# HaydenFaulkner/Tennis

Measured on AMD Instinct MI355X. Metric: frames/sec DenseNet-121 224x224 feature-extract, higher is better.
Workload: dtype f16

## Files before the change

### include/tennis_hip_debug.h

```cpp
#ifndef TENNIS_HIP_DEBUG_H
#define TENNIS_HIP_DEBUG_H
#include "tennis_hip.h"
#ifdef __cplusplus
extern "C" {
#endif

typedef struct {
  char name[32];
  int launches;
  double ms;
  double flops;
  double bytes;
} tn_kernel_stat;


int tn_densenet121_profile(tn_encoder *enc, const void *x, tn_layout layout, int batch, float *feat,
                           tn_kernel_stat *stats, int max_stats, int *n_stats);

int tn_dbg_profile_class_maps(tn_encoder *enc, const void *x, tn_layout layout, int batch, float *feat, const tn_dense *classes,
                              float *maps, tn_kernel_stat *stats, int max_stats, int *n_stats);
int tn_dbg_class_maps(tn_ctx *ctx, const void *x_f16, const float *x32, int B, int H, int W, int C, const float *scale, const float *shift,
                      const float *wd, int PH, int PW, int classes, float *maps, int *n_seq, int *depth);

int tn_densenet121_read_tap(tn_encoder *enc, const char *tap, int batch, float *out_host,
                            size_t capacity, size_t *numel);

int tn_jpeg_sync_passes(const tn_jpeg *j);

int tn_dbg_conv1x1(tn_ctx *ctx, const void *x_f16, int ldx, int K, const float *scale_host,
                   const float *shift_host, const float *w_host, int N, void *y_f16, int ldy, int yoff,
                   int M, int pool, int H, int W);
int tn_dbg_conv3x3(tn_ctx *ctx, const void *x_f16, const float *scale_host, const float *shift_host,
                   const float *w_host, void *y_f16, int ldy, int yoff, int B, int H, int W);
int tn_dbg_pack_conv3x3(const float *w_host, uint16_t *out_host);
int tn_dbg_conv1x1_dev(tn_ctx *ctx, const void *x_f16, int ldx, int K, const float *scale, const float *shift,
                       const void *w_f16, int N, void *y_f16, int ldy, int yoff, int M, int pool, int H, int W,
                       int variant);
int tn_dbg_conv3x3_dev(tn_ctx *ctx, const void *x_f16, const float *scale, const float *shift,
                       const void *wp_f16, void *y_f16, int ldy, int yoff, int B, int H, int W, int variant);
int tn_dbg_conv1x1_ex(tn_ctx *ctx, const void *x_f16, int ldx, int K, const float *scale, const float *shift, const void *w_f16, int N,
                      void *y_f16, int ldy, int yoff, int M, int pool, int H, int W, int variant, const float *bias, int clamp,
                      float *y32, int ld32, const void *wfrag);
int tn_dbg_pack_trans_frags(const uint16_t *w_f16_host, int N, int K, uint16_t *out_host);
int tn_dbg_pack_trans_frags_dev(tn_ctx *ctx, const void *w_f16, int N, int K, void *out_f16);
int tn_dbg_dense_layer_dev(tn_ctx *ctx, void *buf_f16, int ldc, int K, const float *s1, const float *t1,
                           const void *w1_f16, const float *s2, const float *t2, const void *w3p_f16, int B,
                           int H, int W, unsigned long long *ts , int variant );
int tn_dbg_dense_chain_dev(tn_ctx *ctx, void *buf_f16, int ldc, int K0, int nchain, const float *const *s1, const float *const *t1,
                           const void *const *w1_f16, const float *const *s2, const float *const *t2, const void *const *w3p_f16,
                           int B, int H, int W, int variant);
int tn_dbg_linear(tn_ctx *ctx, const float *x, const float *w, const float *bias, float *y, int M, int N,
                  int K);
int tn_dbg_channel_mean(tn_ctx *ctx, const void *x_f16, int ld, int K, const float *scale, const float *shift, int64_t rows,
                        void *scratch, size_t scratch_bytes, float *out, int clamp);
int tn_dbg_stem(tn_ctx *ctx, const float *w0_host, const float *gamma_host, const float *beta_host, const float *mean_host,
                const float *var_host, const float *centre_host, int exact, int fused, int layout, int B, int H, int W,
                const void *x, void *y_f16, int ldy);
int tn_dbg_maxpool(tn_ctx *ctx, const void *x_f16, int B, int H, int W, int C, void *y_f16, int ldy, int Ho, int Wo);
int tn_dbg_head(tn_ctx *ctx, const void *x_f16, const float *x32, int B, int H, int W, int C, const float *scale, const float *shift,
                float *feat, int PH, int PW);
int tn_dbg_pack_strip(const float *w1_host, int K, const float *s2_host, const float *t2_host, uint16_t *w1s_out,
                      const float *w3_host, uint16_t *w3s_out);
int tn_dbg_dense_strip_dev(tn_ctx *ctx, void *buf_f16, int ldc, int K, const float *s1, const float *t1,
                           const void *w1s_f16, const void *w3s_f16, int B, int H, int W,
                           unsigned long long *ts );
int tn_dbg_dense_strip_pair_dev(tn_ctx *ctx, void *buf_f16, int ldc, int K, const float *s1, const float *t1,
                                const void *w1s_f16, const void *w3s_f16, int B, int H, int W, unsigned long long *ts);
int tn_dbg_dense_strip_pair_chain_dev(tn_ctx *ctx, void *buf_f16, int ldc, int K0, int nl, const float *const *s1,
                                      const float *const *t1, const void *const *w1s_f16, const void *const *w3s_f16, int B, int H,
                                      int W);
int tn_dbg_strip_pair_launches(int64_t *count);

int tn_dbg_block7_create(tn_ctx *ctx, int K0, int nl, const float *w1_all, const float *s1_all, const float *t1_all,
                         const float *s2_all, const float *t2_all, const float *w3_all, void **out);
int tn_dbg_block7_run(void *handle, void *buf_f16, int ldc, int B);
int tn_dbg_block7_run_ts(void *handle, void *buf_f16, int ldc, int B,
                         unsigned long long *ts );
void tn_dbg_block7_destroy(void *handle);

int tn_dbg_block14_create(tn_ctx *ctx, int K0, int nl, const float *w1_all, const float *s1_all, const float *t1_all,
                          const float *s2_all, const float *t2_all, const float *w3_all, void **out);
int tn_dbg_block14_run(void *handle, void *buf_f16, int ldc, int B);
int tn_dbg_block14_run_ts(void *handle, void *buf_f16, int ldc, int B,
                          unsigned long long *ts );
void tn_dbg_block14_destroy(void *handle);
int tn_dbg_block28_create(tn_ctx *ctx, int K0, int nl, const float *w1_all, const float *s1_all, const float *t1_all,
                          const float *s2_all, const float *t2_all, const float *w3_all, void **out);
int tn_dbg_block28_run(void *handle, void *buf_f16, int ldc, int B);
int tn_dbg_block28_run_ts(void *handle, void *buf_f16, int ldc, int B, unsigned long long *ts);
void tn_dbg_block28_destroy(void *handle);

int tn_dbg_gemm_tn(tn_ctx *ctx, const float *A, int lda, const float *B, int ldb, const float *bsc, const float *bsh, float *Cm, int ldc,
                   int M, int N, int K, float *workspace, int64_t workspace_floats);
int tn_dbg_linear_bnrelu(tn_ctx *ctx, const float *X, int ldx, const float *asc, const float *ash, const float *W, int ldw,
                         const float *bias, float *Y, int ldy, int M, int N, int K, int accumulate);
int tn_dbg_linear_fp32x3(tn_ctx *ctx, const float *X, int ldx, const float *asc, const float *ash, const float *W, int ldw,
                         const float *bias, float *Y, int ldy, int M, int N, int K, int accumulate);
int tn_dbg_gemm_tn_fp32x3(tn_ctx *ctx, const float *A, int lda, const float *B, int ldb, const float *bsc, const float *bsh, float *Cm,
                          int ldc, int M, int N, int K, float *workspace, int64_t workspace_floats);
int tn_dbg_gemm_nn(tn_ctx *ctx, const float *A, int lda, const float *B, int ldb, float *Cm, int ldc, int M, int N, int K);
int tn_dbg_bn_train(tn_ctx *ctx, const float *x, int ld, int64_t M, int C, const float *gamma, const float *beta, float *mean, float *var,
                    float *y, const float *dy, float *dgamma, float *dbeta, float *dx, int ldd, int accumulate);
int tn_dbg_gnmt_trainer_src_grad(tn_gnmt_trainer *t, const float *src, const int32_t *src_valid_len, const int32_t *tgt, int ld,
                                 const int32_t *tgt_valid_len, int batch, int steps, int tgt_len, float *loss, float *logits_out,
                                 float *dsrc, int ldd);
int tn_dbg_rows_pad_skip(int on);

int tn_dbg_rnn_route(int gates, int B, int H, int dirs, int *nb, int *kr, int *big);

int tn_dbg_rnn_wide_route(int gates, int B, int H, int dirs, int *threads, int *rows, int *nb, int64_t *lds_fwd, int64_t *lds_bwd);
int tn_dbg_rnn_force_wide(int on);
int tn_dbg_rnn_wide_launches(int64_t *count);

int tn_dbg_encoder_plan(int height, int width, int flags, int batch, int calibrate, tn_kernel_stat *stats, int max_stats, int *n_stats);
int tn_dbg_encoder_plan_shared(int height, int width, int flags, int batch, tn_kernel_stat *stats, int max_stats, int *n_stats,
                               int *paired_out);

enum { TN_TRAINER_HEAD = 0, TN_TRAINER_GNMT = 1, TN_TRAINER_BACKBONE = 2 };
typedef struct tn_param_row {
  char name[96];
  int where;
  int64_t offset, count;
} tn_param_row;
int tn_dbg_trainer_params(int which, const int *dims, int n_dims, const char *prefix_a, const char *prefix_b, tn_param_row *rows,
                          int max_rows, int *n_rows, int64_t *numel, int64_t *state_numel);

int tn_dbg_conv_fp32x3(tn_ctx *ctx, int which, int kind, int tile, int layout, const void *x, int ldx, int K, const float *s, const float *t,
                       const float *w_host, int N, const float *es, const float *et, float *y, int ldy, int yoff, int64_t M, int H, int W,
                       int Ho, int Wo);

int tn_dbg_window_head_rows_per_group(struct tn_window_head *h, int nb);

#define TN_GRAD_SUMSQ_BLOCK 256
#define TN_GRAD_SUMSQ_CHUNK 4096
#define TN_GRAD_SUMSQ_GRID 1024
int tn_dbg_grad_sumsq(tn_ctx *ctx, const float *dev, int64_t n, const float *dev2, int64_t n2, double *sumsq_host);

int tn_dbg_gnmt_attention_fwd(tn_ctx *ctx, const float *g0, const float *hprev, int ldh, const float *cprev, int lstm, const float *keyproj,
                              const float *mem, const int32_t *valid_len, int B, int T, int H, int beam, int split_cap, float *hn, float *cn,
                              float *x1, int ldx1, float *ctx_out, float *w_out);
int tn_dbg_gnmt_attention_bwd(tn_ctx *ctx, const float *aw, const float *mem, const float *keyproj, const float *c0, int lc0, const float *c1,
                              int lc1, const int32_t *valid_len, int B, int T, int H, float *ds, float *dctx, float *dh0);
int tn_dbg_gnmt_attention_outer(tn_ctx *ctx, const float *aw, const float *ds, const float *dctx, const float *h0, int ldh, int steps, int B,
                                int T, int H, float *dmem, float *dkp);
int tn_dbg_gnmt_ce(tn_ctx *ctx, const float *logits, const int32_t *labels, int ld, const int32_t *valid_len, int B, int L, int V,
                   float *dlogits, float *loss_rows, float *loss, float *masked_loss);
int tn_dbg_gnmt_emb_grad(tn_ctx *ctx, const float *dx0, int K0, const int32_t *tgt, int ld, int B, int L, int E, int V, float *demb);

#ifdef __cplusplus
}
#endif
#endif
```

### tennis_amd/_lib.py

```python
from __future__ import annotations

import ctypes as C
import os

import numpy as np
import torch

_HERE = os.path.dirname(os.path.abspath(__file__))
LIB_PATH = os.environ.get("TENNIS_HIP_LIB") or os.path.join(_HERE, "lib", "libtennis_hip.so")

LAYOUT_NCHW_F32, LAYOUT_NHWC_F16, LAYOUT_NHWC_U8 = 0, 1, 2
ENC_EXACT_WEIGHTS = 1
ENC_FP32 = 4
ENC_FP32X3 = 8
RNN_GRU, RNN_LSTM = 0, 1
POOL_MAX, POOL_MEAN = 0, 1
MATMUL_MODES = {"f32": 0, "fp32x3": 1}


def matmul_mode(name) -> int:
    if name not in MATMUL_MODES:
        raise ValueError(f"matmul must be 'f32' or 'fp32x3', got {name!r}")
    return MATMUL_MODES[name]

# ... 15 lines not shown
PARAM_FLAT, PARAM_STATE, PARAM_PTR = 0, 1, 2

_P = C.c_void_p
_SIGS = {
    "tn_version": (C.c_int, []),
    "tn_last_error": (C.c_char_p, []),
    "tn_ctx_create": (C.c_int, [C.c_int, _P, C.c_int, C.POINTER(_P)]),
    "tn_ctx_stream": (_P, [_P]),
    "tn_ctx_sync": (C.c_int, [_P]),
    "tn_ctx_destroy": (C.c_int, [_P]),
    "tn_densenet121_create": (C.c_int, [_P, C.POINTER(TnParam), C.c_int, C.c_char_p, C.c_int, C.c_int, C.c_int,
                                        C.POINTER(_P)]),
    "tn_densenet121_create_ex": (C.c_int, [_P, C.POINTER(TnParam), C.c_int, C.c_char_p, C.c_int, C.c_int, C.c_int, C.c_int,
                                           C.POINTER(_P)]),
    "tn_densenet121_feature_dim": (C.c_int, [_P]),
    "tn_densenet121_workspace_bytes": (C.c_size_t, [_P]),
    "tn_densenet121_forward": (C.c_int, [_P, _P, C.c_int, C.c_int, _P]),
    "tn_densenet121_forward_class_maps": (C.c_int, [_P, _P, C.c_int, C.c_int, _P, _P, _P]),
    "tn_densenet121_class_map_dims": (C.c_int, [_P, C.POINTER(C.c_int), C.POINTER(C.c_int)]),
    "tn_dbg_profile_class_maps": (C.c_int, [_P, _P, C.c_int, C.c_int, _P, _P, _P, C.POINTER(TnKernelStat), C.c_int, C.POINTER(C.c_int)]),
    "tn_dbg_class_maps": (C.c_int, [_P, _P, _P, C.c_int, C.c_int, C.c_int, C.c_int, _P, _P, _P, C.c_int, C.c_int, C.c_int, _P,
                                    C.POINTER(C.c_int), C.POINTER(C.c_int)]),
    "tn_densenet121_set_pipelined": (C.c_int, [_P, C.c_int]),
    "tn_densenet121_join": (C.c_int, [_P, C.c_int]),
    "tn_densenet121_profile": (C.c_int, [_P, _P, C.c_int, C.c_int, _P, C.POINTER(TnKernelStat), C.c_int,
                                         C.POINTER(C.c_int)]),
    "tn_densenet121_read_tap": (C.c_int, [_P, C.c_char_p, C.c_int, _P, C.c_size_t, C.POINTER(C.c_size_t)]),
    "tn_densenet121_destroy": (C.c_int, [_P]),
    "tn_dense_create": (C.c_int, [_P, _P, _P, C.c_int, C.c_int, C.POINTER(_P)]),
    "tn_dense_forward": (C.c_int, [_P, _P, C.c_int, _P]),
    "tn_dense_destroy": (C.c_int, [_P]),
    "tn_birnn_create": (C.c_int, [_P, C.c_int, C.c_int, C.c_int, C.POINTER(TnParam), C.c_int, C.c_char_p, C.c_int,
                                  C.c_int, C.POINTER(_P)]),
    "tn_birnn_forward": (C.c_int, [_P, _P, C.c_int, C.c_int, _P, _P, _P, _P]),
    "tn_birnn_destroy": (C.c_int, [_P]),
    "tn_preproc_create": (C.c_int, [_P, C.c_int, C.c_int, C.c_int, C.c_int, C.POINTER(_P)]),
    "tn_preproc_forward": (C.c_int, [_P, _P, C.c_int, _P]),
    "tn_preproc_destroy": (C.c_int, [_P]),
    "tn_augment_forward": (C.c_int, [_P, _P, C.c_int, C.c_int, C.c_int, _P, _P, C.c_int, _P, _P, _P]),
    "tn_to_tensor_normalize": (C.c_int, [_P, _P, C.c_long, C.POINTER(C.c_float), C.POINTER(C.c_float), _P]),
    "tn_jpeg_create": (C.c_int, [_P, C.POINTER(_P)]),
    "tn_jpeg_info": (C.c_int, [_P, C.c_size_t, C.POINTER(C.c_int), C.POINTER(C.c_int), C.POINTER(C.c_int), C.POINTER(C.c_int),
                               C.POINTER(C.c_int)]),
    "tn_jpeg_decode": (C.c_int, [_P, C.POINTER(_P), C.POINTER(C.c_size_t), C.c_int, _P, C.POINTER(C.c_int), C.POINTER(C.c_int)]),
    "tn_jpeg_sync_passes": (C.c_int, [_P]),
    "tn_jpeg_destroy": (C.c_int, [_P]),
    "tn_temporal_pool": (C.c_int, [_P, _P, C.c_int, C.c_int, C.c_int, C.c_int, _P]),
    "tn_window_head_create": (C.c_int, [_P, C.c_int, C.c_int, C.c_int, C.c_int, C.POINTER(TnParam), C.c_int, C.c_char_p, C.c_char_p,
                                        C.c_int, C.c_int, C.POINTER(_P)]),
    "tn_window_head_project": (C.c_int, [_P, _P, C.c_int]),
    "tn_window_head_forward": (C.c_int, [_P, _P, _P, _P, C.c_int, C.c_int, C.c_int, _P, _P]),
    "tn_window_head_forward_rows": (C.c_int, [_P, _P, C.c_int, C.c_int, _P, _P]),
    "tn_window_head_destroy": (C.c_int, [_P]),
    "tn_temporal_pool_windows": (C.c_int, [_P, _P, C.c_int, C.c_int, _P, _P, _P, C.c_int, C.c_int, C.c_int, C.c_int, _P]),
    "tn_temporal_pool_rows": (C.c_int, [_P, _P, C.c_int, C.c_int, _P, C.c_int, C.c_int, C.c_int, _P]),
    "tn_dbg_window_head_rows_per_group": (C.c_int, [_P, C.c_int]),
    "tn_prf1_update": (C.c_int, [_P, _P, _P, C.c_int, C.c_int, _P]),
    "tn_head_create": (C.c_int, [_P, C.c_int, C.c_int, C.c_int, C.c_int, C.POINTER(TnParam), C.c_int, C.c_char_p, C.c_char_p, C.c_int,
                                 C.c_int, C.POINTER(_P)]),
    "tn_head_forward_backward": (C.c_int, [_P, _P, _P, C.c_int, C.c_int, _P, _P]),
    "tn_head_set_features": (C.c_int, [_P, _P, C.c_int, C.c_int]),
    "tn_head_forward_backward_rows": (C.c_int, [_P, _P, _P, C.c_int, C.c_int, _P, _P]),
    "tn_head_forward_rows": (C.c_int, [_P, _P, C.c_int, C.c_int, _P]),
    "tn_head_buffers": (C.c_int, [_P, C.POINTER(_P), C.POINTER(_P), C.POINTER(C.c_int64)]),
    "tn_head_sgd_step": (C.c_int, [_P, C.c_float, C.c_float, C.c_float, C.c_float]),
    "tn_head_read_param": (C.c_int, [_P, C.c_char_p, C.c_int, C.POINTER(C.c_float), C.c_int64, C.POINTER(C.c_int64)]),
    "tn_head_destroy": (C.c_int, [_P]),
    "tn_finetune_create": (C.c_int, [_P, C.POINTER(TnParam), C.c_int, C.c_char_p, C.c_char_p, C.c_int, C.c_int, C.c_int, C.c_int,
                                     C.POINTER(_P)]),
    "tn_finetune_forward_backward": (C.c_int, [_P, _P, _P, C.c_int, C.c_int, C.c_int, _P, _P]),
    "tn_finetune_buffers": (C.c_int, [_P, C.POINTER(_P), C.POINTER(_P), C.POINTER(C.c_int64)]),
    "tn_finetune_sgd_step": (C.c_int, [_P, C.c_float, C.c_float, C.c_float, C.c_float]),
    "tn_finetune_read_param": (C.c_int, [_P, C.c_char_p, C.c_int, C.POINTER(C.c_float), C.c_int64, C.POINTER(C.c_int64)]),
    "tn_finetune_destroy": (C.c_int, [_P]),
    "tn_finetune_set_matmul": (C.c_int, [_P, C.c_int]),
    "tn_finetune_matmul_stats": (C.c_int, [_P, C.POINTER(C.c_int64), C.POINTER(C.c_int64)]),
    "tn_cnnrnn_trainer_set_matmul": (C.c_int, [_P, C.c_int]),
    "tn_cnnrnn_trainer_matmul_stats": (C.c_int, [_P, C.POINTER(C.c_int64), C.POINTER(C.c_int64)]),
    "tn_gnmt_frames_trainer_set_matmul": (C.c_int, [_P, C.c_int]),
    "tn_gnmt_frames_trainer_matmul_stats": (C.c_int, [_P, C.POINTER(C.c_int64), C.POINTER(C.c_int64)]),
    "tn_cnnrnn_trainer_create": (C.c_int, [_P, C.c_int, C.POINTER(TnParam), C.c_int, C.c_char_p, C.c_char_p, C.c_char_p, C.c_int, C.c_int,
                                           C.c_int, C.c_int, C.c_int, C.c_int, C.POINTER(_P)]),
    "tn_cnnrnn_trainer_forward_backward": (C.c_int, [_P, _P, _P, C.c_int, C.c_int, C.c_int, C.c_int, _P, _P]),
    "tn_cnnrnn_trainer_buffers": (C.c_int, [_P, C.POINTER(_P), C.POINTER(_P), C.POINTER(C.c_int64), C.POINTER(_P), C.POINTER(_P),
                                            C.POINTER(C.c_int64)]),
    "tn_cnnrnn_trainer_sgd_step": (C.c_int, [_P, C.c_float, C.c_float, C.c_float, C.c_float]),
    "tn_cnnrnn_trainer_read_param": (C.c_int, [_P, C.c_char_p, C.c_int, C.POINTER(C.c_float), C.c_int64, C.POINTER(C.c_int64)]),
    "tn_cnnrnn_trainer_destroy": (C.c_int, [_P]),
    "tn_gnmt_frames_trainer_create": (C.c_int, [_P, C.POINTER(TnParam), C.c_int, C.c_char_p, C.c_char_p, C.c_int, C.c_int, C.c_int, C.c_int,
                                                C.c_int, C.c_int, C.c_int, C.c_int, C.c_int, C.c_int, C.c_int, C.c_int, C.c_int,
                                                C.POINTER(_P)]),
    "tn_gnmt_frames_trainer_forward_backward": (C.c_int, [_P, _P, _P, _P, C.c_int, _P, C.c_int, C.c_int, C.c_int, _P, _P]),
    "tn_gnmt_frames_trainer_buffers": (C.c_int, [_P, C.POINTER(_P), C.POINTER(_P), C.POINTER(C.c_int64), C.POINTER(_P), C.POINTER(_P),
                                                 C.POINTER(C.c_int64)]),
    "tn_gnmt_frames_trainer_set_dropout": (C.c_int, [_P, C.c_float, C.c_uint64]),
    "tn_gnmt_frames_trainer_adam_step": (C.c_int, [_P, C.c_float, C.c_float, C.c_float, C.c_float]),
    "tn_gnmt_frames_trainer_read_param": (C.c_int, [_P, C.c_char_p, C.c_int, C.POINTER(C.c_float), C.c_int64, C.POINTER(C.c_int64)]),
    "tn_gnmt_frames_trainer_destroy": (C.c_int, [_P]),
    "tn_head_set_clip": (C.c_int, [_P, C.c_float]),
    "tn_head_clip_stats": (C.c_int, [_P, C.POINTER(C.c_float), C.POINTER(C.c_float), C.POINTER(C.c_int64)]),
    "tn_finetune_set_clip": (C.c_int, [_P, C.c_float]),
    "tn_finetune_clip_stats": (C.c_int, [_P, C.POINTER(C.c_float), C.POINTER(C.c_float), C.POINTER(C.c_int64)]),
    "tn_cnnrnn_trainer_set_clip": (C.c_int, [_P, C.c_float]),
    "tn_cnnrnn_trainer_clip_stats": (C.c_int, [_P, C.POINTER(C.c_float), C.POINTER(C.c_float), C.POINTER(C.c_int64)]),
    "tn_gnmt_trainer_set_clip": (C.c_int, [_P, C.c_float]),
    "tn_gnmt_trainer_clip_stats": (C.c_int, [_P, C.POINTER(C.c_float), C.POINTER(C.c_float), C.POINTER(C.c_int64)]),
    "tn_gnmt_frames_trainer_set_clip": (C.c_int, [_P, C.c_float]),
    "tn_gnmt_frames_trainer_clip_stats": (C.c_int, [_P, C.POINTER(C.c_float), C.POINTER(C.c_float), C.POINTER(C.c_int64)]),
    "tn_dbg_grad_sumsq": (C.c_int, [_P, _P, C.c_int64, _P, C.c_int64, C.POINTER(C.c_double)]),
    "tn_dbg_rows_pad_skip": (C.c_int, [C.c_int]),
    "tn_dbg_gnmt_trainer_src_grad": (C.c_int, [_P, _P, _P, _P, C.c_int, _P, C.c_int, C.c_int, C.c_int, _P, _P, _P, C.c_int]),
    "tn_dbg_gnmt_attention_fwd": (C.c_int, [_P, _P, _P, C.c_int, _P, C.c_int, _P, _P, _P, C.c_int, C.c_int, C.c_int, C.c_int, C.c_int,
                                            _P, _P, _P, C.c_int, _P, _P]),
    "tn_dbg_gnmt_attention_bwd": (C.c_int, [_P, _P, _P, _P, _P, C.c_int, _P, C.c_int, _P, C.c_int, C.c_int, C.c_int, _P, _P, _P]),
    "tn_dbg_gnmt_attention_outer": (C.c_int, [_P, _P, _P, _P, _P, C.c_int, C.c_int, C.c_int, C.c_int, C.c_int, _P, _P]),
    "tn_dbg_gnmt_ce": (C.c_int, [_P, _P, _P, C.c_int, _P, C.c_int, C.c_int, C.c_int, _P, _P, _P, _P]),
    "tn_dbg_gnmt_emb_grad": (C.c_int, [_P, _P, C.c_int, _P, C.c_int, C.c_int, C.c_int, C.c_int, C.c_int, _P]),
    "tn_gnmt_trainer_create": (C.c_int, [_P, C.POINTER(TnParam), C.c_int, C.c_char_p, C.c_int, C.c_int, C.c_int, C.c_int, C.c_int,
                                         C.c_int, C.c_int, C.c_int, C.POINTER(_P)]),
    "tn_gnmt_trainer_create_ex": (C.c_int, [_P, C.POINTER(TnParam), C.c_int, C.c_char_p, C.c_int, C.c_int, C.c_int, C.c_int, C.c_int,
                                            C.c_int, C.c_int, C.c_int, C.c_int, C.c_int, C.c_int, C.POINTER(_P)]),
    "tn_gnmt_trainer_dropout_mask": (C.c_int, [_P, C.c_int, C.POINTER(_P)]),
    "tn_gnmt_trainer_forward_backward": (C.c_int, [_P, _P, _P, _P, C.c_int, _P, C.c_int, C.c_int, C.c_int, _P, _P]),
    "tn_gnmt_trainer_forward_backward_rows": (C.c_int, [_P, _P, C.c_int, C.c_int, _P, _P, _P, C.c_int, _P, C.c_int, C.c_int, C.c_int, _P, _P]),
    "tn_gnmt_trainer_buffers": (C.c_int, [_P, C.POINTER(_P), C.POINTER(_P), C.POINTER(C.c_int64)]),
    "tn_gnmt_trainer_set_dropout": (C.c_int, [_P, C.c_float, C.c_uint64]),
    "tn_gnmt_trainer_dropout_masks": (C.c_int, [_P, C.POINTER(_P), C.POINTER(_P), C.POINTER(_P)]),
    "tn_gnmt_trainer_adam_step": (C.c_int, [_P, C.c_float, C.c_float, C.c_float, C.c_float]),
    "tn_gnmt_trainer_read_param": (C.c_int, [_P, C.c_char_p, C.c_int, C.POINTER(C.c_float), C.c_int64, C.POINTER(C.c_int64)]),
    "tn_gnmt_trainer_destroy": (C.c_int, [_P]),
    "tn_gnmt_create": (C.c_int, [_P, C.POINTER(TnParam), C.c_int, C.c_char_p, C.c_int, C.c_int, C.c_int, C.c_int, C.c_int,
                                 C.c_int, C.c_int, C.c_int, C.c_int, C.c_int, C.c_int, C.POINTER(_P)]),
    "tn_gnmt_create_ex": (C.c_int, [_P, C.POINTER(TnParam), C.c_int, C.c_char_p, C.c_int, C.c_int, C.c_int, C.c_int, C.c_int,
                                    C.c_int, C.c_int, C.c_int, C.c_int, C.c_int, C.c_int, C.c_int, C.POINTER(_P)]),
    "tn_gnmt_encode": (C.c_int, [_P, _P, _P, C.c_int, C.c_int, _P]),
    "tn_gnmt_encode_rows": (C.c_int, [_P, _P, C.c_int, C.c_int, _P, _P, C.c_int, C.c_int, _P]),
    "tn_gnmt_beam_search": (C.c_int, [_P, C.c_int, C.c_int, C.c_float, C.c_float, C.c_int, _P, _P, _P,
                                      C.POINTER(C.c_int)]),
    "tn_gnmt_decode_seq": (C.c_int, [_P, _P, C.c_int, C.c_int, _P]),
    "tn_gnmt_decode_seq_attention": (C.c_int, [_P, _P, C.c_int, C.c_int, _P, _P]),
    "tn_gnmt_beam_search_attention": (C.c_int, [_P, C.c_int, C.c_int, C.c_float, C.c_float, C.c_int, _P, _P, _P,
                                                C.POINTER(C.c_int), _P]),
    "tn_masked_softmax_ce": (C.c_int, [_P, _P, _P, C.c_int, _P, C.c_int, C.c_int, C.c_int, _P]),
    "tn_gnmt_destroy": (C.c_int, [_P]),
    "tn_dbg_conv1x1": (C.c_int, [_P, _P, C.c_int, C.c_int, _P, _P, _P, C.c_int, _P, C.c_int, C.c_int, C.c_int,
                                 C.c_int, C.c_int, C.c_int]),
    "tn_dbg_conv3x3": (C.c_int, [_P, _P, _P, _P, _P, _P, C.c_int, C.c_int, C.c_int, C.c_int, C.c_int]),
    "tn_dbg_pack_conv3x3": (C.c_int, [_P, _P]),
    "tn_dbg_conv1x1_dev": (C.c_int, [_P, _P, C.c_int, C.c_int, _P, _P, _P, C.c_int, _P, C.c_int, C.c_int, C.c_int,
                                     C.c_int, C.c_int, C.c_int, C.c_int]),
    "tn_dbg_conv3x3_dev": (C.c_int, [_P, _P, _P, _P, _P, _P, C.c_int, C.c_int, C.c_int, C.c_int, C.c_int, C.c_int]),
    "tn_dbg_conv1x1_ex": (C.c_int, [_P, _P, C.c_int, C.c_int, _P, _P, _P, C.c_int, _P, C.c_int, C.c_int, C.c_int,
                                    C.c_int, C.c_int, C.c_int, C.c_int, _P, C.c_int, _P, C.c_int, _P]),
    "tn_dbg_pack_trans_frags": (C.c_int, [_P, C.c_int, C.c_int, _P]),
    "tn_dbg_pack_trans_frags_dev": (C.c_int, [_P, _P, C.c_int, C.c_int, _P]),
    "tn_dbg_dense_layer_dev": (C.c_int, [_P, _P, C.c_int, C.c_int, _P, _P, _P, _P, _P, _P, C.c_int, C.c_int, C.c_int,
                                         _P, C.c_int]),
    "tn_dbg_dense_chain_dev": (C.c_int, [_P, _P, C.c_int, C.c_int, C.c_int, _P, _P, _P, _P, _P, _P, C.c_int, C.c_int, C.c_int, C.c_int]),
    "tn_dbg_linear": (C.c_int, [_P, _P, _P, _P, _P, C.c_int, C.c_int, C.c_int]),
    "tn_dbg_channel_mean": (C.c_int, [_P, _P, C.c_int, C.c_int, _P, _P, C.c_int64, _P, C.c_size_t, _P, C.c_int]),
    "tn_dbg_stem": (C.c_int, [_P, _P, _P, _P, _P, _P, _P, C.c_int, C.c_int, C.c_int, C.c_int, C.c_int, C.c_int, _P, _P, C.c_int]),
    "tn_dbg_maxpool": (C.c_int, [_P, _P, C.c_int, C.c_int, C.c_int, C.c_int, _P, C.c_int, C.c_int, C.c_int]),
    "tn_dbg_head": (C.c_int, [_P, _P, _P, C.c_int, C.c_int, C.c_int, C.c_int, _P, _P, _P, C.c_int, C.c_int]),
    "tn_dbg_conv_fp32x3": (C.c_int, [_P, C.c_int, C.c_int, C.c_int, C.c_int, _P, C.c_int, C.c_int, _P, _P, _P, C.c_int, _P, _P, _P, C.c_int,
                                     C.c_int, C.c_int64, C.c_int, C.c_int, C.c_int, C.c_int]),
    "tn_dbg_gemm_tn": (C.c_int, [_P, _P, C.c_int, _P, C.c_int, _P, _P, _P, C.c_int, C.c_int, C.c_int, C.c_int, _P, C.c_int64]),
    "tn_dbg_gemm_nn": (C.c_int, [_P, _P, C.c_int, _P, C.c_int, _P, C.c_int, C.c_int, C.c_int, C.c_int]),
    "tn_dbg_rnn_wide_route": (C.c_int, [C.c_int, C.c_int, C.c_int, C.c_int, C.POINTER(C.c_int), C.POINTER(C.c_int), C.POINTER(C.c_int),
                                        C.POINTER(C.c_int64), C.POINTER(C.c_int64)]),
    "tn_dbg_rnn_force_wide": (C.c_int, [C.c_int]),
    "tn_dbg_rnn_wide_launches": (C.c_int, [C.POINTER(C.c_int64)]),
    "tn_dbg_rnn_route": (C.c_int, [C.c_int, C.c_int, C.c_int, C.c_int, C.POINTER(C.c_int), C.POINTER(C.c_int), C.POINTER(C.c_int)]),
    "tn_dbg_encoder_plan": (C.c_int, [C.c_int, C.c_int, C.c_int, C.c_int, C.c_int, C.POINTER(TnKernelStat), C.c_int, C.POINTER(C.c_int)]),
    "tn_dbg_encoder_plan_shared": (C.c_int, [C.c_int, C.c_int, C.c_int, C.c_int, C.POINTER(TnKernelStat), C.c_int, C.POINTER(C.c_int),
                                             C.POINTER(C.c_int)]),
    "tn_dbg_trainer_params": (C.c_int, [C.c_int, C.POINTER(C.c_int), C.c_int, C.c_char_p, C.c_char_p, C.POINTER(TnParamRow), C.c_int,
                                        C.POINTER(C.c_int), C.POINTER(C.c_int64), C.POINTER(C.c_int64)]),
    "tn_dbg_linear_bnrelu": (C.c_int, [_P, _P, C.c_int, _P, _P, _P, C.c_int, _P, _P, C.c_int, C.c_int, C.c_int, C.c_int, C.c_int]),
    "tn_dbg_linear_fp32x3": (C.c_int, [_P, _P, C.c_int, _P, _P, _P, C.c_int, _P, _P, C.c_int, C.c_int, C.c_int, C.c_int, C.c_int]),
    "tn_dbg_gemm_tn_fp32x3": (C.c_int, [_P, _P, C.c_int, _P, C.c_int, _P, _P, _P, C.c_int, C.c_int, C.c_int, C.c_int, _P, C.c_int64]),
    "tn_dbg_bn_train": (C.c_int, [_P, _P, C.c_int, C.c_int64, C.c_int, _P, _P, _P, _P, _P, _P, _P, _P, _P, C.c_int, C.c_int]),
    "tn_comm_unique_id": (C.c_int, [_P]),
    "tn_comm_create": (C.c_int, [_P, C.c_int, C.c_int, _P, C.c_int, C.POINTER(_P)]),
    "tn_comm_rank": (C.c_int, [_P]),
    "tn_comm_world": (C.c_int, [_P]),
    "tn_comm_device": (C.c_int, [_P]),
    "tn_comm_uses_rccl": (C.c_int, [_P]),
    "tn_allgather_features": (C.c_int, [_P, _P, C.c_int, C.c_int, _P]),
    "tn_allreduce_f32": (C.c_int, [_P, _P, C.c_size_t, C.c_int]),
    "tn_allreduce_i64": (C.c_int, [_P, _P, C.c_size_t]),
    "tn_comm_destroy": (C.c_int, [_P]),
    "tn_dbg_pack_strip": (C.c_int, [_P, C.c_int, _P, _P, _P, _P, _P]),
    "tn_dbg_dense_strip_dev": (C.c_int, [_P, _P, C.c_int, C.c_int, _P, _P, _P, _P, C.c_int, C.c_int, C.c_int, _P]),
    "tn_dbg_dense_strip_pair_dev": (C.c_int, [_P, _P, C.c_int, C.c_int, _P, _P, _P, _P, C.c_int, C.c_int, C.c_int, _P]),
    "tn_dbg_dense_strip_pair_chain_dev": (C.c_int, [_P, _P, C.c_int, C.c_int, C.c_int, _P, _P, _P, _P, C.c_int, C.c_int, C.c_int]),
    "tn_dbg_strip_pair_launches": (C.c_int, [C.POINTER(C.c_int64)]),
    "tn_densenet121_input_means": (C.c_int, [_P, _P, C.c_int, C.c_int, _P, C.c_int64, C.POINTER(C.c_int64)]),
    "tn_npy_writer_create": (C.c_int, [C.c_int, C.POINTER(_P)]),
    "tn_npy_writer_submit": (C.c_int, [_P, _P, C.c_int, C.c_int, C.POINTER(C.c_char_p), C.c_int]),
    "tn_npy_writer_drain": (C.c_int, [_P, C.POINTER(C.c_int64), C.POINTER(C.c_int64)]),
    "tn_npy_writer_destroy": (C.c_int, [_P]),
    "tn_bn_relu_clamp_fold": (C.c_int, [_P, _P, _P, _P, C.c_int, _P, _P, _P, _P]),
    "tn_fp32x3_split": (C.c_int, [_P, C.c_int64, _P, _P, _P]),
    "tn_round_fp16_calibrated": (C.c_int, [_P, C.c_int, C.c_int, _P, C.c_int, C.c_int, C.c_double, _P]),
    "tn_dbg_block7_create": (C.c_int, [_P, C.c_int, C.c_int, _P, _P, _P, _P, _P, _P, C.POINTER(C.c_void_p)]),
    "tn_dbg_block7_run": (C.c_int, [_P, _P, C.c_int, C.c_int]),
    "tn_dbg_block7_run_ts": (C.c_int, [_P, _P, C.c_int, C.c_int, _P]),
    "tn_dbg_block7_destroy": (None, [_P]),
    "tn_dbg_block14_create": (C.c_int, [_P, C.c_int, C.c_int, _P, _P, _P, _P, _P, _P, C.POINTER(C.c_void_p)]),
    "tn_dbg_block14_run": (C.c_int, [_P, _P, C.c_int, C.c_int]),
    "tn_dbg_block14_run_ts": (C.c_int, [_P, _P, C.c_int, C.c_int, _P]),
    "tn_dbg_block14_destroy": (None, [_P]),
    "tn_dbg_block28_create": (C.c_int, [_P, C.c_int, C.c_int, _P, _P, _P, _P, _P, _P, C.POINTER(C.c_void_p)]),
    "tn_dbg_block28_run": (C.c_int, [_P, _P, C.c_int, C.c_int]),
    "tn_dbg_block28_run_ts": (C.c_int, [_P, _P, C.c_int, C.c_int, _P]),
    "tn_dbg_block28_destroy": (None, [_P]),
}

_lib = None


def declared_symbols():
    return sorted(_SIGS)


def load():
    global _lib
    if _lib is None:
        if not os.path.exists(LIB_PATH):
            raise RuntimeError(
                f"{LIB_PATH} is missing: build it with `make` (or __graft_entry__.build()). "
                "tennis_amd has no CPU fallback.")
        lib = C.CDLL(LIB_PATH)
        for name, (res, args) in _SIGS.items():
            fn = getattr(lib, name)
            fn.restype, fn.argtypes = res, args
        _lib = lib
    return _lib


def check(rc: int, what: str = ""):
    if rc != 0:
        msg = load().tn_last_error().decode("utf-8", "replace")
        raise RuntimeError(f"libtennis_hip {what} failed ({rc}): {msg}")


def trainer_params(which: int, dims, prefix_a: str, prefix_b: str | None = None):
    lib = load()
    d = (C.c_int * len(dims))(*[int(v) for v in dims])
    b = None if prefix_b is None else prefix_b.encode()
    n, numel, ns = C.c_int(), C.c_int64(), C.c_int64()
    check(lib.tn_dbg_trainer_params(which, d, len(dims), prefix_a.encode(), b, None, 0, C.byref(n), None, None), "tn_dbg_trainer_params")
    rows = (TnParamRow * n.value)()
    check(lib.tn_dbg_trainer_params(which, d, len(dims), prefix_a.encode(), b, rows, n.value, C.byref(n), C.byref(numel), C.byref(ns)),
          "tn_dbg_trainer_params")
    return [(r.name.decode(), r.where, r.offset, r.count) for r in rows], numel.value, ns.value


def make_params(params: dict):
    keep = []
    arr = (TnParam * len(params))()
    for i, (k, v) in enumerate(params.items()):
        a = np.ascontiguousarray(v, dtype=np.float32)
        name = k.encode()
        keep += [a, name]
        arr[i].name = name
        arr[i].data_host = a.ctypes.data_as(C.POINTER(C.c_float))
        arr[i].numel = a.size
    return arr, keep


class Context:

    def __init__(self, device: int | None = None, stream=None):
        if not torch.cuda.is_available():
            raise RuntimeError("tennis_amd needs a ROCm GPU: torch.cuda.is_available() is False and there is no "
                               "CPU fallback")
        self.lib = load()
        device = default_device() if device is None else int(device)
        self.device = device
        if stream is None:
            stream = torch.cuda.current_stream(device)
        self.torch_stream = stream
        h = _P()
        check(self.lib.tn_ctx_create(device, _P(stream.cuda_stream), 0, C.byref(h)), "tn_ctx_create")
        self.handle = h

    def sync(self):
        check(self.lib.tn_ctx_sync(self.handle), "tn_ctx_sync")

    def __del__(self):
        try:
            if getattr(self, "handle", None):
                self.lib.tn_ctx_destroy(self.handle)
                self.handle = None
        except Exception:
            pass


_default_ctx = {}


def default_device() -> int:
    if torch.cuda.is_available():
        cur = torch.cuda.current_device()
        if cur != 0 or "LOCAL_RANK" not in os.environ:
            return cur
        lr = int(os.environ["LOCAL_RANK"])
        return lr if lr < torch.cuda.device_count() else cur
    return 0


def default_context(device: int | None = None) -> Context:
    device = default_device() if device is None else int(device)
    if device not in _default_ctx:
        _default_ctx[device] = Context(device)
    return _default_ctx[device]


def ptr(t) -> _P:
    return _P(t.data_ptr()) if t is not None else _P(None)
```

### tennis_amd/csrc/common.h

```cpp
#pragma once
#include <atomic>
#include <hip/hip_runtime.h>
#include <hip/hip_fp16.h>
#include <stdint.h>
#include <string>
#include <vector>

#include "../../include/tennis_hip.h"
#include "../../include/tennis_hip_debug.h"

typedef _Float16 f16;
typedef _Float16 f16x4 __attribute__((ext_vector_type(4)));
typedef _Float16 f16x8 __attribute__((ext_vector_type(8)));
typedef float f32x4 __attribute__((ext_vector_type(4)));
typedef float f32x16 __attribute__((ext_vector_type(16)));

void tn_set_error(const std::string &msg);
#define TN_HIP_CHECK(expr)                                                             \
  do {                                                                                 \
    hipError_t _e = (expr);                                                            \
    if (_e != hipSuccess) {                                                            \
      tn_set_error(std::string(#expr) + ": " + hipGetErrorString(_e));                 \
      return TN_ERR_HIP;                                                               \
    }                                                                                  \
  } while (0)
#define TN_REQUIRE(cond, msg)                                                          \
  do {                                                                                 \
    if (!(cond)) {                                                                     \
      tn_set_error(std::string("invalid argument: ") + (msg));                         \
      return TN_ERR_INVALID;                                                           \
    }                                                                                  \
  } while (0)

struct TnDeviceGuard {
  int prev = -1;
  bool ok = true;
  explicit TnDeviceGuard(int dev) {
    if (hipGetDevice(&prev) != hipSuccess) prev = -1;
    if (prev == dev) prev = -1;
    else ok = hipSetDevice(dev) == hipSuccess;
  }
  ~TnDeviceGuard() {
    if (prev >= 0) (void)hipSetDevice(prev);
  }
  TnDeviceGuard(const TnDeviceGuard &) = delete;
  TnDeviceGuard &operator=(const TnDeviceGuard &) = delete;
};
#define TN_DG_CAT2(a, b) a##b
#define TN_DG_CAT(a, b) TN_DG_CAT2(a, b)
#define TN_ON_DEVICE(dev)                                                              \
  TnDeviceGuard TN_DG_CAT(tn_dg_, __LINE__)(dev);                                      \
  if (!TN_DG_CAT(tn_dg_, __LINE__).ok) {                                               \
    tn_set_error("hipSetDevice failed");                                               \
    return TN_ERR_HIP;                                                                 \
  }

struct tn_ctx {
  int device;
  hipStream_t stream;
  bool own_stream;
};

__device__ __forceinline__ f16x8 bn_relu8(f16x8 v, const float *__restrict__ s, const float *__restrict__ t) {
  f16x8 r;
#pragma unroll
  for (int j = 0; j < 8; ++j) {
    float f = fmaf((float)v[j], s[j], t[j]);
    r[j] = (f16)fmaxf(f, 0.0f);
  }
  return r;
}

__device__ __forceinline__ f16x8 clamp8(f16x8 v, const float *__restrict__ lo, const float *__restrict__ hi) {
  f16x8 r;
#pragma unroll
  for (int j = 0; j < 8; ++j) r[j] = (f16)fminf(fmaxf((float)v[j], lo[j]), hi[j]);
  return r;
}
__device__ __forceinline__ unsigned clamp2_pk(unsigned in, float lo0, float lo1, float hi0, float hi1) {
  unsigned l, h, o;
  asm("v_cvt_pk_f16_f32 %1, %4, %5\n\tv_cvt_pk_f16_f32 %2, %6, %7\n\tv_pk_max_f16 %0, %3, %1\n\tv_pk_min_f16 %0, %0, %2\n\ts_nop 0"
      : "=&v"(o), "=&v"(l), "=&v"(h) : "v"(in), "v"(lo0), "v"(lo1), "v"(hi0), "v"(hi1));
  return o;
}
__device__ __forceinline__ f16x8 clamp8_pk(f16x8 v, const float *__restrict__ lo, const float *__restrict__ hi) {
  typedef unsigned u32x4 __attribute__((ext_vector_type(4)));
  const u32x4 in = __builtin_bit_cast(u32x4, v);
  u32x4 out;
#pragma unroll
  for (int j = 0; j < 4; ++j) out[j] = clamp2_pk(in[j], lo[2 * j], lo[2 * j + 1], hi[2 * j], hi[2 * j + 1]);
  return __builtin_bit_cast(f16x8, out);
}

__device__ __forceinline__ f16x4 bn_relu4_from_f32(f32x4 v, float4 s, float4 t) {
  typedef unsigned u32x2 __attribute__((ext_vector_type(2)));
  float a0, a1, a2, a3;
  unsigned d0, d1;
  asm("s_nop 11\n\t"
      "v_fma_f32 %2, %6, %10, %14\n\tv_fma_f32 %3, %7, %11, %15\n\tv_fma_f32 %4, %8, %12, %16\n\tv_fma_f32 %5, %9, %13, %17\n\t"
      "v_cvt_pk_f16_f32 %0, %2, %3\n\tv_cvt_pk_f16_f32 %1, %4, %5\n\tv_pk_max_f16 %0, %0, 0\n\tv_pk_max_f16 %1, %1, 0"
      : "=&v"(d0), "=&v"(d1), "=&v"(a0), "=&v"(a1), "=&v"(a2), "=&v"(a3)
      : "v"(v[0]), "v"(v[1]), "v"(v[2]), "v"(v[3]), "v"(s.x), "v"(s.y), "v"(s.z), "v"(s.w), "v"(t.x), "v"(t.y), "v"(t.z), "v"(t.w));
  const u32x2 o = {d0, d1};
  return __builtin_bit_cast(f16x4, o);
}

template <int ROWB>
__device__ __forceinline__ int swz(int row, int chunk) {
  constexpr int NCH = ROWB / 16;
  return row * ROWB + ((chunk ^ (row & (NCH - 1))) << 4);
}

struct Conv1x1Args {
  const f16 *x;
  int ldx;
  int K;
  const float *scale;
  const float *shift;
  const f16 *w;
  int N;
  f16 *y;
  int ldy, yoff;
  int M;
  int pool;
  int H, W;
  int variant = 0;
  int exact = 0;
  const float *bias = nullptr;
  int clamp = 0;
  float *y32 = nullptr;
  int ld32 = 0;
  const f16 *wfrag = nullptr;
};
int launch_conv1x1(const Conv1x1Args &a, hipStream_t s);
bool trans_ws_supported(const Conv1x1Args &a);
int launch_trans_ws(const Conv1x1Args &a, hipStream_t s);
std::vector<f16> pack_trans_frags(const f16 *w, int N, int K);
int launch_pack_trans_frags(const f16 *w, int N, int K, f16 *out, hipStream_t s);

struct Conv3x3Args {
  const f16 *x;
  const float *scale;
  const float *shift;
  const f16 *wp;
  f16 *y;
  int ldy, yoff;
  int M, H, W;
  int variant = 0;
  int exact = 0;
};
int launch_conv3x3(const Conv3x3Args &a, hipStream_t s);
size_t conv3x3_lds_bytes(int W);

struct DenseLayerDev {
  const float *s1, *t1;
  const f16 *w1;
  const float *s2, *t2;
  const f16 *w3p;
};
struct DenseLayerArgs {
  f16 *buf;
  int ldc, K;
  const float *s1, *t1;
  const f16 *w1;
  const float *s2, *t2;
  const f16 *w3p;
  int B, H, W;
  unsigned long long *ts = nullptr;
  int variant = 0;
  const DenseLayerDev *chain = nullptr;
  int nchain = 0;
  int exact = 0;
};
bool dense_layer_supported(int H, int W);
int dense_layer_kmax(int W);
int launch_dense_layer(const DenseLayerArgs &a, hipStream_t s);

struct DenseStripArgs {
  f16 *buf;
  int ldc, K;
  const float *s1, *t1;
  const f16 *w1s;
  const f16 *w3s;
  int B, H, W;
  unsigned long long *ts = nullptr;
};
bool dense_strip_supported(int H, int W, int K);
int launch_dense_strip(const DenseStripArgs &a, hipStream_t s);
struct DenseStripLayerDev {
  const float *s1, *t1;
  const f16 *w1s, *w3s;
};
struct DenseStripChainArgs {
  f16 *buf;
  int ldc, K0, nl;
  const DenseStripLayerDev *layers;
  int B, H, W;
};
bool dense_strip_chain_supported(int H, int W, int K0, int nl);
int dense_strip_chain_layers(int H, int W, int K0);
int launch_dense_strip_chain(const DenseStripChainArgs &a, hipStream_t s);
int launch_dense_strip_pair(const DenseStripArgs &a, hipStream_t s);
int launch_dense_strip_pair_chain(const DenseStripChainArgs &a, hipStream_t s);
long strip_pair_launches();
std::vector<f16> pack_w1_strip(const float *w , int K, const float *shift );
std::vector<f16> pack_w3_strip(const float *w );

struct DenseBlock7Args {
  f16 *buf;
  int ldc, K0, nl, B;
  const f16 *wa, *wb;
  const float *tab;
  unsigned a_off[4], b_off[4];
  unsigned long long *ts = nullptr;
  float *side = nullptr;
};
struct Block7Layer { const float *w1f , *w3 , *s1, *t1 , *t2 ; };
struct Block7Image {
  std::vector<f16> wa, wb;
  std::vector<float> tab;
  unsigned a_off[4], b_off[4];
};
bool dense_block7_supported(int H, int W, int K0, int nl);
inline constexpr const char *kDenseBlock7Range = "7 x 7, K0 = 448 ... 992 in steps of 32, nl >= 1, K0 + 32 nl <= 1024";
Block7Image pack_block7(const std::vector<Block7Layer> &layers, int K0);
int launch_dense_block7(const DenseBlock7Args &a, hipStream_t s);

struct DenseStreamArgs {
  f16 *buf;
  int ldc, K0, nl, B;
  const unsigned char *stream;
  int total_units;
  f16 *scratch = nullptr;
  unsigned long long *ts = nullptr;
};
struct Block14Layer { const float *w1f , *w3 , *s1, *t1 , *t2 ; };
bool dense_block14_supported(int H, int W, int K0, int nl);
int dense_block14_units(int K0, int nl);
size_t dense_block14_scratch_halfs();
std::vector<unsigned char> pack_block14(const std::vector<Block14Layer> &layers, int K0);
int launch_dense_block14(const DenseStreamArgs &a, hipStream_t s);
bool dense_block28_supported(int H, int W, int K0, int nl);
int dense_block28_units(int K0, int nl);
size_t dense_block28_scratch_halfs();
std::vector<unsigned char> pack_block28(const std::vector<Block14Layer> &layers, int K0);
int launch_dense_block28(const DenseStreamArgs &a, hipStream_t s);
inline constexpr const char *kDenseBlock14Range = "14 x 14, K0 = 256 ... 992 in steps of 32, nl >= 1, K0 + 32 nl <= 1024";
inline constexpr const char *kDenseBlock28Range = "28 x 28, K0 = 128 ... 512 in steps of 32, nl >= 1, K0 + 32 (nl - 1) <= 512";
struct DenseStreamKernel {
  int H;
  const char *family;
  bool (*supported)(int H, int W, int K0, int nl);
  int (*units)(int K0, int nl);
  size_t (*scratch_halfs)();
  std::vector<unsigned char> (*pack)(const std::vector<Block14Layer> &layers, int K0);
  int (*launch)(const DenseStreamArgs &a, hipStream_t s);
  const char *range;
};
inline constexpr DenseStreamKernel kDenseStreamKernels[2] = {
    {14, "dense_block_stream_14x14", dense_block14_supported, dense_block14_units, dense_block14_scratch_halfs, pack_block14, launch_dense_block14, kDenseBlock14Range},
    {28, "dense_block_stream_28x28", dense_block28_supported, dense_block28_units, dense_block28_scratch_halfs, pack_block28, launch_dense_block28, kDenseBlock28Range},
};

constexpr double kStemMean[3] = {0.485, 0.456, 0.406}, kStemStd[3] = {0.229, 0.224, 0.225};
constexpr float kStemQ[3] = {124.f, 116.f, 104.f};
constexpr double kStemWScale = 64.0;
constexpr float stem_unscale(int c) { return (float)(255.0 * kStemStd[c]); }
constexpr float stem_wfactor(int c) { return (float)(kStemWScale / (255.0 * kStemStd[c])); }
constexpr double stem_pad(int c) { return 255.0 * kStemMean[c] - (double)kStemQ[c]; }

struct StemArgs {
  const void *x;
  int layout;
  int B, H, W;
  const f16 *wp;
  const f16 *wp_zf;
  const float *scale;
  const float *shift;
  f16 *y;
  int Ho, Wo;
  const float *shift_u8 = nullptr;
  const f16 *wp_zf_lo = nullptr;
  const float *floor = nullptr;
};
struct StemFold {
  std::vector<f16> wp, wp_zf, wp_zf_lo;
  std::vector<float> scale, shift, shift_u8;
  std::vector<float> floor;
};
StemFold fold_stem(const float *w0, const float *bn_scale, const float *bn_shift, const float *centre, bool exact);
StemFold fold_stem_bn(const float *w0, const float *gamma, const float *beta, const float *mean, const float *var, const float *centre, bool exact);
int launch_stem(const StemArgs &a, hipStream_t s);
int launch_stem_pool(const StemArgs &a, f16 *out, int ldy, int Hp, int Wp, hipStream_t s);

int launch_maxpool3x3s2(const f16 *x, int B, int H, int W, int C, f16 *y, int ldy, int Ho, int Wo, hipStream_t s);
struct PerDeviceFlag {
  std::atomic<unsigned long long> done{0};
  bool is_set(int *dev_out) {
    int d = 0;
    (void)hipGetDevice(&d);
    *dev_out = d;
    return (done.load(std::memory_order_acquire) >> (d & 63)) & 1ull;
  }
  void set(int d) { done.fetch_or(1ull << (d & 63), std::memory_order_release); }
};
#define TN_SET_ATTR_ONCE_PER_DEVICE(...)                    \
  do {                                                      \
    static PerDeviceFlag tn_flag_;                          \
    int tn_dev_;                                            \
    if (!tn_flag_.is_set(&tn_dev_)) {                       \
      __VA_ARGS__;                                          \
      tn_flag_.set(tn_dev_);                                \
    }                                                       \
  } while (0)

void bn_scale_shift(const float *gamma, const float *beta, const float *mean, const float *var, int n, float eps, float *scale, float *shift);
void bn_relu_clamp_fold(const float *scale, const float *shift, int n, float *lo, float *hi, float *sw, float *tc);
int launch_channel_mean(const f16 *x, int ld, int K, const float *scale, const float *shift, long rows, double *scratch ,
                        float *out, hipStream_t s, int clamp = 0 );
int launch_head(const f16 *x, int B, int H, int W, int C, const float *scale, const float *shift,
                float *feat, int PH, int PW, hipStream_t s, const float *x32 = nullptr );
int launch_class_maps(const f16 *x, const float *x32, int B, int H, int W, int C, const float *scale, const float *shift, const float *wd,
                      int PH, int PW, int classes, float *out, hipStream_t s);
int class_maps_seq(int C);
int class_maps_depth();

enum { FP32_STEM = 0, FP32_1X1 = 1, FP32_3X3 = 2, FP32_TRANS = 3 };
struct Fp32ConvArgs {
  int kind;
  const void *x;
  int layout;
  int ldx;
  int K;
  const float *s, *t;
  const float *w;
  const uint16_t *wx = nullptr;
  int N;
  const float *es, *et;
  float *y;
  int ldy, yoff;
  long M;
  int H, W;
  int Ho, Wo;
};
int launch_conv_fp32(const Fp32ConvArgs &a, hipStream_t s);
int launch_conv_fp32x3(const Fp32ConvArgs &a, hipStream_t s, int tile = 0);
void fp32x3_split(const float *w, int64_t n, uint16_t *t1, uint16_t *t2, uint16_t *t3);
std::vector<uint16_t> fp32x3_pack_weights(const float *wk, int kp, int N);
int launch_maxpool_fp32(const float *x, int B, int H, int W, float *y, int ldy, int Ho, int Wo, hipStream_t s);
```

### tennis_amd/csrc/conv1x1.hip

```cpp
#include <cstdlib>

#include "common.h"

namespace {

constexpr int BN_TILE = 128;
constexpr int BK = 64;

template <int MI, int NB, bool POOL = false>
constexpr int smem_bytes() {
  constexpr int tiles = (POOL ? 2 : 1) * 32 * MI * 128 + NB * 128;
  constexpr int epi = 32 * MI * (NB * 2 + 16);
  return tiles > epi ? tiles : epi;
}

template <int MI, bool POOL, int NB, bool EX = false, bool ONCE = false>
__global__ __launch_bounds__(256) void conv1x1_kernel(Conv1x1Args a) {
  constexpr int BM = 32 * MI;
  constexpr int NSRC = POOL ? 4 : 1;
  constexpr int NI = NB / 32;
  constexpr int CPITCH = NB * 2 + 16;
  __shared__ __attribute__((aligned(16))) unsigned char smem[smem_bytes<MI, NB, POOL>()];
  unsigned char *Xs = smem;
  unsigned char *Xl = smem + BM * 128;
// ... 42 lines not shown
  const int WLD = EX ? 2 * nkc * BK : K;
  const f16 *wsrc = a.w + (long)(n0 + r0) * WLD;

  f16x8 xr[MI][NSRC];
  f16x8 wr[NI];
  float sc[8], sh[8];

  auto load_tile = [&](int kt) {
    const int kc = ((EX && kt >= nkc) ? kt - nkc : kt) * BK + c * 8;
    const int kw = kt * BK + c * 8;
    if (kc < K) {
      const float4 s0 = *(const float4 *)(a.scale + kc);
      const float4 s1 = *(const float4 *)(a.scale + kc + 4);
      const float4 t0 = *(const float4 *)(a.shift + kc);
      const float4 t1 = *(const float4 *)(a.shift + kc + 4);
      sc[0] = s0.x; sc[1] = s0.y; sc[2] = s0.z; sc[3] = s0.w;
      sc[4] = s1.x; sc[5] = s1.y; sc[6] = s1.z; sc[7] = s1.w;
      sh[0] = t0.x; sh[1] = t0.y; sh[2] = t0.z; sh[3] = t0.w;
      sh[4] = t1.x; sh[5] = t1.y; sh[6] = t1.z; sh[7] = t1.w;
#pragma unroll
      for (int i = 0; i < MI; ++i)
#pragma unroll
        for (int s = 0; s < NSRC; ++s) {
          if constexpr (ONCE) xr[i][s] = __builtin_nontemporal_load((const f16x8 *)(xsrc[i][s] + kc));
          else xr[i][s] = *(const f16x8 *)(xsrc[i][s] + kc);
        }
#pragma unroll
      for (int i = 0; i < NI; ++i) wr[i] = *(const f16x8 *)(wsrc + (long)(32 * i) * WLD + kw);
    }
  };

  auto store_tile = [&](int kt) {
    const int kc = ((EX && kt >= nkc) ? kt - nkc : kt) * BK + c * 8;
    const bool kv = kc < K;
#pragma unroll
    for (int i = 0; i < MI; ++i) {
      f16x8 v;
      [[maybe_unused]] f16x8 vl;
      if (kv) {
        if constexpr (POOL) {
#pragma unroll
          for (int j = 0; j < 8; ++j) {
            float acc = 0.f;
#pragma unroll
            for (int s = 0; s < 4; ++s) acc += fmaxf(fmaf((float)xr[i][s][j], sc[j], sh[j]), 0.f);
            const float m = 0.25f * acc;
            v[j] = (f16)m;
            vl[j] = (f16)(m - (float)v[j]);
          }
        } else {
          v = a.clamp ? clamp8(xr[i][0], sc, sh) : bn_relu8(xr[i][0], sc, sh);
        }
      } else {
#pragma unroll
        for (int j = 0; j < 8; ++j) { v[j] = (f16)0.f; vl[j] = (f16)0.f; }
      }
      *(f16x8 *)(Xs + swz<128>(r0 + 32 * i, c)) = v;
      if constexpr (POOL) *(f16x8 *)(Xl + swz<128>(r0 + 32 * i, c)) = vl;
    }
#pragma unroll
    for (int i = 0; i < NI; ++i) {
      f16x8 v = wr[i];
      if (!kv) {
#pragma unroll
        for (int j = 0; j < 8; ++j) v[j] = (f16)0.f;
      }
      *(f16x8 *)(Ws + swz<128>(r0 + 32 * i, c)) = v;
    }
  };

  f32x4 acc[NI][MI];
#pragma unroll
  for (int ni = 0; ni < NI; ++ni)
#pragma unroll
    for (int mi = 0; mi < MI; ++mi) acc[ni][mi] = (f32x4){0.f, 0.f, 0.f, 0.f};

  const int nk = EX ? 2 * nkc : nkc;
  const int frow = lane & 15;
  const int fch = lane >> 4;

  load_tile(0);
  for (int kt = 0; kt < nk; ++kt) {
    store_tile(kt);
    __syncthreads();
    if (kt + 1 < nk) load_tile(kt + 1);
#pragma unroll
    for (int ks = 0; ks < 2; ++ks) {
      if (((EX && kt >= nkc) ? kt - nkc : kt) * BK + ks * 32 < K) {
        f16x8 xb[MI], wa[NI];
        [[maybe_unused]] f16x8 xl[MI];
#pragma unroll
        for (int mi = 0; mi < MI; ++mi) {
          xb[mi] = *(const f16x8 *)(Xs + swz<128>(wm * 16 * MI + mi * 16 + frow, ks * 4 + fch));
          if constexpr (POOL) xl[mi] = *(const f16x8 *)(Xl + swz<128>(wm * 16 * MI + mi * 16 + frow, ks * 4 + fch));
        }
#pragma unroll
        for (int ni = 0; ni < NI; ++ni)
          wa[ni] = *(const f16x8 *)(Ws + swz<128>(wn * (NB / 2) + ni * 16 + frow, ks * 4 + fch));
#pragma unroll
        for (int ni = 0; ni < NI; ++ni)
#pragma unroll
          for (int mi = 0; mi < MI; ++mi)
            acc[ni][mi] = __builtin_amdgcn_mfma_f32_16x16x32_f16(wa[ni], xb[mi], acc[ni][mi], 0, 0, 0);
        if constexpr (POOL) {
#pragma unroll
          for (int ni = 0; ni < NI; ++ni)
#pragma unroll
            for (int mi = 0; mi < MI; ++mi)
              acc[ni][mi] = __builtin_amdgcn_mfma_f32_16x16x32_f16(wa[ni], xl[mi], acc[ni][mi], 0, 0, 0);
        }
      }
    }
    __syncthreads();
  }

#pragma unroll
  for (int ni = 0; ni < NI; ++ni)
#pragma unroll
    for (int mi = 0; mi < MI; ++mi) {
      const int m = wm * 16 * MI + mi * 16 + frow;
      const int n = wn * (NB / 2) + ni * 16 + fch * 4;
      f16x4 h;
      float4 bv = make_float4(0.f, 0.f, 0.f, 0.f);
      if (a.bias) bv = *(const float4 *)(a.bias + n0 + n);
      const float b4[4] = {bv.x, bv.y, bv.z, bv.w};
#pragma unroll
      for (int r = 0; r < 4; ++r) h[r] = (f16)(acc[ni][mi][r] + b4[r]);
      *(f16x4 *)(smem + m * CPITCH + n * 2) = h;
      if (a.y32 && m0 + m < a.M)
        *(float4 *)(a.y32 + (long)(m0 + m) * a.ld32 + n0 + n) =
            make_float4(acc[ni][mi][0] + b4[0], acc[ni][mi][1] + b4[1], acc[ni][mi][2] + b4[2], acc[ni][mi][3] + b4[3]);
    }
  __syncthreads();
#pragma unroll
  for (int i = 0; i < MI * NB / 64; ++i) {
    const int id = t + 256 * i;
    const int row = id / (NB / 8), ch = id % (NB / 8);
    const int m = m0 + row;
    if (m < a.M) {
      const uint4 v = *(const uint4 *)(smem + row * CPITCH + ch * 16);
      *(uint4 *)(a.y + (long)m * a.ldy + a.yoff + n0 + ch * 8) = v;
    }
  }
}

}

int launch_conv1x1(const Conv1x1Args &a, hipStream_t s) {
  TN_REQUIRE(a.K % 32 == 0 && a.N % BN_TILE == 0, "conv1x1: K%32 or N%128");
  TN_REQUIRE(a.ldx % 8 == 0 && a.ldy % 8 == 0 && a.yoff % 8 == 0, "conv1x1: strides must be multiples of 8");
  const dim3 block(256);
  static const bool no_ws = getenv("TN_NO_TRANS_WS") != nullptr;
  if (a.wfrag && !no_ws && trans_ws_supported(a)) return launch_trans_ws(a, s);
  if (a.pool) {
    static const bool narrow = getenv("TN_TRANS_NARROW") != nullptr;
    const bool wide = a.N % 256 == 0 && !narrow;
    const int mtiles = (a.M + 63) / 64, NT = a.N / (wide ? 256 : BN_TILE);
    const dim3 grid(((mtiles + 7) / 8) * 8 * NT);
    if (a.exact) {
      TN_REQUIRE(a.K % 64 == 0, "conv1x1: the exact-weights mode needs K % 64 == 0");
      if (wide) hipLaunchKernelGGL((conv1x1_kernel<2, true, 256, true>), grid, block, 0, s, a);
      else hipLaunchKernelGGL((conv1x1_kernel<2, true, 128, true>), grid, block, 0, s, a);
    } else {
      static const bool no_nt = getenv("TN_TRANS_NO_NT") != nullptr;
      static const size_t nt_mb = getenv("TN_TRANS_NT_MB") ? (size_t)atoi(getenv("TN_TRANS_NT_MB")) : 128;
      const bool stream = NT == 1 && !no_nt && (size_t)a.M * 4 * a.ldx * sizeof(f16) > (nt_mb << 20);
      if (wide && stream) hipLaunchKernelGGL((conv1x1_kernel<2, true, 256, false, true>), grid, block, 0, s, a);
      else if (wide) hipLaunchKernelGGL((conv1x1_kernel<2, true, 256>), grid, block, 0, s, a);
      else if (stream) hipLaunchKernelGGL((conv1x1_kernel<2, true, 128, false, true>), grid, block, 0, s, a);
      else hipLaunchKernelGGL((conv1x1_kernel<2, true, 128>), grid, block, 0, s, a);
    }
  } else if (a.M >= 128 * 512) {
    const dim3 grid((a.M + 127) / 128, a.N / BN_TILE);
    if (a.exact) hipLaunchKernelGGL((conv1x1_kernel<4, false, 128, true>), grid, block, 0, s, a);
    else hipLaunchKernelGGL((conv1x1_kernel<4, false, 128>), grid, block, 0, s, a);
  } else if (a.M >= 64 * 512) {
    const dim3 grid((a.M + 63) / 64, a.N / BN_TILE);
    if (a.exact) hipLaunchKernelGGL((conv1x1_kernel<2, false, 128, true>), grid, block, 0, s, a);
    else hipLaunchKernelGGL((conv1x1_kernel<2, false, 128>), grid, block, 0, s, a);
  } else {
    const dim3 grid((a.M + 31) / 32, a.N / BN_TILE);
    if (a.exact) hipLaunchKernelGGL((conv1x1_kernel<1, false, 128, true>), grid, block, 0, s, a);
    else hipLaunchKernelGGL((conv1x1_kernel<1, false, 128>), grid, block, 0, s, a);
  }
  TN_HIP_CHECK(hipGetLastError());
  return TN_OK;
}
```

### tennis_amd/csrc/dbg.hip

```cpp
#include <cstring>
#include <vector>

#include "common.h"
#include "encoder_plan.h"
#include "gemm_fp32x3.h"
#include "linear.h"
#include "param_table.h"
#include "rnn.h"
#include "train.h"

namespace {
template <typename T>
T *up(const std::vector<T> &h) {
  T *d = nullptr;
  if (hipMalloc(&d, h.size() * sizeof(T)) != hipSuccess) return nullptr;
  if (hipMemcpy(d, h.data(), h.size() * sizeof(T), hipMemcpyHostToDevice) != hipSuccess) return nullptr;
  return d;
}
}

std::vector<f16> pack_conv3x3(const float *w);

extern "C" int tn_dbg_pack_conv3x3(const float *w_host, uint16_t *out_host) {
  TN_REQUIRE(w_host && out_host, "tn_dbg_pack_conv3x3: null argument");
  const std::vector<f16> p = pack_conv3x3(w_host);
  memcpy(out_host, p.data(), p.size() * sizeof(f16));
  return TN_OK;
}

extern "C" int tn_dbg_conv1x1_dev(tn_ctx *ctx, const void *x_f16, int ldx, int K, const float *scale,
                                  const float *shift, const void *w_f16, int N, void *y_f16, int ldy, int yoff, int M,
                                  int pool, int H, int W, int variant) {
  TN_REQUIRE(ctx && x_f16 && y_f16 && scale && shift && w_f16, "tn_dbg_conv1x1_dev: null argument");
  Conv1x1Args a{(const f16 *)x_f16, ldx, K, scale, shift, (const f16 *)w_f16, N, (f16 *)y_f16, ldy, yoff, M, pool, H, W};
  a.variant = variant & 0xffff;
  a.exact = (variant >> 17) & 1;
  if ((variant >> 18) & 1) {
    TN_REQUIRE(trans_ws_supported(a), "tn_dbg_conv1x1_dev: geometry not supported by trans_ws");
    TN_ON_DEVICE(ctx->device);
    static f16 *frags[64] = {};
    static size_t frag_halves[64] = {};
    TN_REQUIRE(ctx->device >= 0 && ctx->device < 64, "tn_dbg_conv1x1_dev: device index out of range");
    f16 *&frag = frags[ctx->device];
    if (frag_halves[ctx->device] < (size_t)N * K) {
      if (frag) (void)hipFree(frag);
      frag = nullptr; frag_halves[ctx->device] = 0;
      TN_HIP_CHECK(hipMalloc((void **)&frag, (size_t)N * K * sizeof(f16)));
      frag_halves[ctx->device] = (size_t)N * K;
    }
    const int rc = launch_pack_trans_frags(a.w, N, K, frag, ctx->stream);
    if (rc) return rc;
    a.wfrag = frag;
  }
  return launch_conv1x1(a, ctx->stream);
}

extern "C" int tn_dbg_conv1x1_ex(tn_ctx *ctx, const void *x_f16, int ldx, int K, const float *scale, const float *shift, const void *w_f16,
                                 int N, void *y_f16, int ldy, int yoff, int M, int pool, int H, int W, int variant, const float *bias,
                                 int clamp, float *y32, int ld32, const void *wfrag) {
  TN_REQUIRE(ctx && x_f16 && y_f16 && scale && shift && w_f16, "tn_dbg_conv1x1_ex: null argument");
  TN_REQUIRE(M > 0 && K > 0 && N > 0 && ldx >= K && ldy >= yoff + N && yoff >= 0, "tn_dbg_conv1x1_ex: bad shape (M, K, N positive, ldx >= K, ldy >= yoff + N)");
  TN_REQUIRE(!pool || (H >= 2 && W >= 2 && M % ((H / 2) * (W / 2)) == 0), "tn_dbg_conv1x1_ex: pooling needs H, W >= 2 and M = B (H / 2) (W / 2)");
  TN_REQUIRE(!y32 || (ld32 >= N && ld32 % 4 == 0 && ((uintptr_t)y32 & 15) == 0), "tn_dbg_conv1x1_ex: y32 needs ld32 >= N, a multiple of 4, and 16-byte alignment");
  Conv1x1Args a{(const f16 *)x_f16, ldx, K, scale, shift, (const f16 *)w_f16, N, (f16 *)y_f16, ldy, yoff, M, pool, H, W};
  a.variant = variant & 0xffff;
  a.exact = (variant >> 17) & 1;
  a.bias = bias;
  a.clamp = clamp != 0;
  a.y32 = y32;
  a.ld32 = ld32;
  a.wfrag = (const f16 *)wfrag;
  TN_REQUIRE(!wfrag || trans_ws_supported(a), "tn_dbg_conv1x1_ex: wfrag with a geometry trans_ws does not support (pooling, fp16 weights, no bias, N = 512 | 256, K % 128 == 0, even H and W)");
  TN_ON_DEVICE(ctx->device);
  return launch_conv1x1(a, ctx->stream);
}

extern "C" int tn_dbg_pack_trans_frags(const uint16_t *w_f16_host, int N, int K, uint16_t *out_host) {
  TN_REQUIRE(w_f16_host && out_host, "tn_dbg_pack_trans_frags: null argument");
  TN_REQUIRE(N > 0 && K > 0 && N % 32 == 0 && K % 16 == 0, "tn_dbg_pack_trans_frags: N % 32 or K % 16");
  const std::vector<f16> p = pack_trans_frags((const f16 *)w_f16_host, N, K);
  memcpy(out_host, p.data(), p.size() * sizeof(f16));
  return TN_OK;
}
extern "C" int tn_dbg_pack_trans_frags_dev(tn_ctx *ctx, const void *w_f16, int N, int K, void *out_f16) {
  TN_REQUIRE(ctx && w_f16 && out_f16, "tn_dbg_pack_trans_frags_dev: null argument");
  TN_REQUIRE(N > 0 && K > 0, "tn_dbg_pack_trans_frags_dev: N and K must be positive");
  TN_ON_DEVICE(ctx->device);
  return launch_pack_trans_frags((const f16 *)w_f16, N, K, (f16 *)out_f16, ctx->stream);
}

extern "C" int tn_dbg_conv3x3_dev(tn_ctx *ctx, const void *x_f16, const float *scale, const float *shift,
                                  const void *wp_f16, void *y_f16, int ldy, int yoff, int B, int H, int W,
                                  int variant) {
  TN_REQUIRE(ctx && x_f16 && y_f16 && scale && shift && wp_f16, "tn_dbg_conv3x3_dev: null argument");
  Conv3x3Args a{(const f16 *)x_f16, scale, shift, (const f16 *)wp_f16, (f16 *)y_f16, ldy, yoff, B * H * W, H, W};
  a.variant = variant & 0xffff;
  a.exact = (variant >> 17) & 1;
  return launch_conv3x3(a, ctx->stream);
}

extern "C" int tn_dbg_conv1x1(tn_ctx *ctx, const void *x_f16, int ldx, int K, const float *scale_host,
                              const float *shift_host, const float *w_host , int N, void *y_f16, int ldy,
                              int yoff, int M, int pool, int H, int W) {
  TN_REQUIRE(ctx && x_f16 && y_f16 && scale_host && shift_host && w_host, "tn_dbg_conv1x1: null argument");
  TN_ON_DEVICE(ctx->device);
  std::vector<f16> wh((size_t)N * K);
  for (size_t i = 0; i < wh.size(); ++i) wh[i] = (f16)w_host[i];
  f16 *w = up(wh);
  float *s = up(std::vector<float>(scale_host, scale_host + K));
  float *t = up(std::vector<float>(shift_host, shift_host + K));
  TN_REQUIRE(w && s && t, "tn_dbg_conv1x1: device allocation failed");
  const int rc = tn_dbg_conv1x1_dev(ctx, x_f16, ldx, K, s, t, w, N, y_f16, ldy, yoff, M, pool, H, W, 0);
  hipError_t e = hipStreamSynchronize(ctx->stream);
  (void)hipFree(w); (void)hipFree(s); (void)hipFree(t);
  if (rc) return rc;
  TN_HIP_CHECK(e);
  return TN_OK;
}

extern "C" int tn_dbg_conv3x3(tn_ctx *ctx, const void *x_f16, const float *scale_host, const float *shift_host,
                              const float *w_host, void *y_f16, int ldy, int yoff, int B, int H, int W) {
  TN_REQUIRE(ctx && x_f16 && y_f16 && scale_host && shift_host && w_host, "tn_dbg_conv3x3: null argument");
  TN_ON_DEVICE(ctx->device);
  f16 *w = up(pack_conv3x3(w_host));
  float *s = up(std::vector<float>(scale_host, scale_host + 128));
  float *t = up(std::vector<float>(shift_host, shift_host + 128));
  TN_REQUIRE(w && s && t, "tn_dbg_conv3x3: device allocation failed");
  const int rc = tn_dbg_conv3x3_dev(ctx, x_f16, s, t, w, y_f16, ldy, yoff, B, H, W, 0);
  hipError_t e = hipStreamSynchronize(ctx->stream);
  (void)hipFree(w); (void)hipFree(s); (void)hipFree(t);
  if (rc) return rc;
  TN_HIP_CHECK(e);
  return TN_OK;
}

extern "C" int tn_dbg_dense_layer_dev(tn_ctx *ctx, void *buf_f16, int ldc, int K, const float *s1, const float *t1,
                                      const void *w1_f16, const float *s2, const float *t2, const void *w3p_f16,
                                      int B, int H, int W, unsigned long long *ts, int variant) {
  TN_REQUIRE(ctx && buf_f16 && s1 && t1 && w1_f16 && s2 && t2 && w3p_f16, "tn_dbg_dense_layer_dev: null argument");
  DenseLayerArgs a{(f16 *)buf_f16, ldc, K, s1, t1, (const f16 *)w1_f16, s2, t2, (const f16 *)w3p_f16, B, H, W};
  a.ts = ts;
  a.variant = variant & 0xffff;
  a.exact = (variant >> 17) & 1;
  return launch_dense_layer(a, ctx->stream);
}

extern "C" int tn_dbg_dense_chain_dev(tn_ctx *ctx, void *buf_f16, int ldc, int K0, int nchain, const float *const *s1, const float *const *t1,
                                      const void *const *w1_f16, const float *const *s2, const float *const *t2, const void *const *w3p_f16,
                                      int B, int H, int W, int variant) {
  TN_REQUIRE(ctx && buf_f16 && s1 && t1 && w1_f16 && s2 && t2 && w3p_f16, "tn_dbg_dense_chain_dev: null argument");
  TN_REQUIRE(nchain > 0 && nchain <= 64, "tn_dbg_dense_chain_dev: nchain must be 1 ... 64");
  std::vector<DenseLayerDev> cd(nchain);
  for (int l = 0; l < nchain; ++l) {
    TN_REQUIRE(s1[l] && t1[l] && w1_f16[l] && s2[l] && t2[l] && w3p_f16[l], "tn_dbg_dense_chain_dev: null layer operand");
    cd[l] = DenseLayerDev{s1[l], t1[l], (const f16 *)w1_f16[l], s2[l], t2[l], (const f16 *)w3p_f16[l]};
  }
  TN_ON_DEVICE(ctx->device);
  DenseLayerDev *chain = up(cd);
  TN_REQUIRE(chain, "tn_dbg_dense_chain_dev: device allocation failed");
  DenseLayerArgs a{(f16 *)buf_f16, ldc, K0, cd[0].s1, cd[0].t1, cd[0].w1, cd[0].s2, cd[0].t2, cd[0].w3p, B, H, W};
  a.variant = variant & 0xffff;
  a.exact = (variant >> 17) & 1;
  a.chain = ((variant >> 19) & 1) ? nullptr : chain;
  a.nchain = nchain;
  const int rc = launch_dense_layer(a, ctx->stream);
  const hipError_t e = hipStreamSynchronize(ctx->stream);
  (void)hipFree(chain);
  if (rc) return rc;
  TN_HIP_CHECK(e);
  return TN_OK;
}

extern "C" int tn_dbg_channel_mean(tn_ctx *ctx, const void *x_f16, int ld, int K, const float *scale, const float *shift, int64_t rows,
                                   void *scratch, size_t scratch_bytes, float *out, int clamp) {
  TN_REQUIRE(ctx && x_f16 && scale && shift && scratch && out, "tn_dbg_channel_mean: null argument");
  TN_REQUIRE(K > 0 && ld >= K && rows > 0, "tn_dbg_channel_mean: bad shape");
  TN_REQUIRE(scratch_bytes >= (size_t)32 * K * sizeof(double), "tn_dbg_channel_mean: scratch smaller than 32 K doubles");
  TN_ON_DEVICE(ctx->device);
  const int rc = launch_channel_mean((const f16 *)x_f16, ld, K, scale, shift, (long)rows, (double *)scratch, out, ctx->stream, clamp != 0);
  if (rc) return rc;
  TN_HIP_CHECK(hipStreamSynchronize(ctx->stream));
  return TN_OK;
}

extern "C" int tn_dbg_stem(tn_ctx *ctx, const float *w0_host, const float *gamma_host, const float *beta_host, const float *mean_host,
                           const float *var_host, const float *centre_host, int exact, int fused, int layout, int B, int H, int W,
                           const void *x, void *y_f16, int ldy) {
  TN_REQUIRE(ctx && w0_host && gamma_host && beta_host && mean_host && var_host && x && y_f16, "tn_dbg_stem: null argument");
  TN_REQUIRE(layout >= 0 && layout <= 2, "tn_dbg_stem: unknown input layout");
  TN_REQUIRE(B > 0 && H >= 16 && W >= 16 && H <= 1024 && W <= 1024, "tn_dbg_stem: bad shape (frames of 16 .. 1024 pixels a side)");
  TN_REQUIRE(ldy >= 64 && ldy % 8 == 0, "tn_dbg_stem: the output stride must be a multiple of 8, at least 64");
  TN_REQUIRE(((uintptr_t)x & 15) == 0 && ((uintptr_t)y_f16 & 15) == 0, "tn_dbg_stem: x and y must be 16-byte aligned");
  TN_REQUIRE(fused || !exact, "tn_dbg_stem: the exact-weights mode has the fused kernel only");
  TN_ON_DEVICE(ctx->device);
  const StemFold f = fold_stem_bn(w0_host, gamma_host, beta_host, mean_host, var_host, centre_host, exact != 0);
  const int Ho = (H + 6 - 7) / 2 + 1, Wo = (W + 6 - 7) / 2 + 1, Hp = (Ho + 2 - 3) / 2 + 1, Wp = (Wo + 2 - 3) / 2 + 1;
  f16 *wp = up(f.wp), *wp_zf = up(f.wp_zf), *wp_lo = exact ? up(f.wp_zf_lo) : nullptr, *map = nullptr;
  float *sc = up(f.scale), *sh = up(f.shift), *shu = up(f.shift_u8), *fl = centre_host ? up(f.floor) : nullptr;
  bool ok = wp && wp_zf && sc && sh && shu && (!exact || wp_lo) && (!centre_host || fl);
  if (ok && !fused) ok = hipMalloc((void **)&map, (size_t)B * Ho * Wo * 64 * sizeof(f16)) == hipSuccess;
  int rc = TN_OK;
  if (ok) {
    StemArgs a{x, layout, B, H, W, wp, wp_zf, sc, sh, map, Ho, Wo};
    a.shift_u8 = shu;
    a.wp_zf_lo = wp_lo;
    a.floor = fl;
    if (fused) rc = launch_stem_pool(a, (f16 *)y_f16, ldy, Hp, Wp, ctx->stream);
    else {
      rc = launch_stem(a, ctx->stream);
      if (!rc) rc = launch_maxpool3x3s2(map, B, Ho, Wo, 64, (f16 *)y_f16, ldy, Hp, Wp, ctx->stream);
    }
  }
  const hipError_t e = hipStreamSynchronize(ctx->stream);
  (void)hipFree(wp); (void)hipFree(wp_zf); (void)hipFree(wp_lo); (void)hipFree(map);
  (void)hipFree(sc); (void)hipFree(sh); (void)hipFree(shu); (void)hipFree(fl);
  TN_REQUIRE(ok, "tn_dbg_stem: device allocation failed");
  if (rc) return rc;
  TN_HIP_CHECK(e);
  return TN_OK;
}

extern "C" int tn_dbg_maxpool(tn_ctx *ctx, const void *x_f16, int B, int H, int W, int C, void *y_f16, int ldy, int Ho, int Wo) {
  TN_REQUIRE(ctx && x_f16 && y_f16, "tn_dbg_maxpool: null argument");
  TN_REQUIRE(B > 0 && H > 0 && W > 0 && C > 0 && ldy >= C, "tn_dbg_maxpool: bad shape");
  TN_REQUIRE(Ho == (H - 1) / 2 + 1 && Wo == (W - 1) / 2 + 1, "tn_dbg_maxpool: the output is ((H - 1) / 2 + 1) x ((W - 1) / 2 + 1)");
  TN_REQUIRE(((uintptr_t)x_f16 & 15) == 0 && ((uintptr_t)y_f16 & 15) == 0, "tn_dbg_maxpool: x and y must be 16-byte aligned");
  TN_ON_DEVICE(ctx->device);
  const int rc = launch_maxpool3x3s2((const f16 *)x_f16, B, H, W, C, (f16 *)y_f16, ldy, Ho, Wo, ctx->stream);
  if (rc) return rc;
  TN_HIP_CHECK(hipStreamSynchronize(ctx->stream));
  return TN_OK;
}

extern "C" int tn_dbg_head(tn_ctx *ctx, const void *x_f16, const float *x32, int B, int H, int W, int C, const float *scale, const float *shift,
                           float *feat, int PH, int PW) {
  TN_REQUIRE(ctx && (x_f16 || x32) && scale && shift && feat, "tn_dbg_head: null argument");
  TN_REQUIRE(B > 0 && C > 0 && PH > 0 && PW > 0 && 7 * PH <= H && 7 * PW <= W, "tn_dbg_head: bad shape (PH x PW windows of 7 x 7 inside H x W)");
  TN_REQUIRE((((uintptr_t)x_f16 | (uintptr_t)x32) & 15) == 0, "tn_dbg_head: the map must be 16-byte aligned");
  TN_ON_DEVICE(ctx->device);
  const int rc = launch_head((const f16 *)x_f16, B, H, W, C, scale, shift, feat, PH, PW, ctx->stream, x32);
  if (rc) return rc;
  TN_HIP_CHECK(hipStreamSynchronize(ctx->stream));
  return TN_OK;
}

extern "C" int tn_dbg_class_maps(tn_ctx *ctx, const void *x_f16, const float *x32, int B, int H, int W, int C, const float *scale,
                                 const float *shift, const float *wd, int PH, int PW, int classes, float *maps, int *n_seq, int *depth) {
  TN_REQUIRE(ctx && (x_f16 || x32) && scale && shift && wd && maps, "tn_dbg_class_maps: null argument");
  TN_REQUIRE((((uintptr_t)x_f16 | (uintptr_t)x32 | (uintptr_t)wd) & 15) == 0, "tn_dbg_class_maps: the map and the weights must be 16-byte aligned");
  TN_ON_DEVICE(ctx->device);
  const int rc = launch_class_maps((const f16 *)x_f16, x32, B, H, W, C, scale, shift, wd, PH, PW, classes, maps, ctx->stream);
  if (rc) return rc;
  TN_HIP_CHECK(hipStreamSynchronize(ctx->stream));
  if (n_seq) *n_seq = class_maps_seq(C);
  if (depth) *depth = class_maps_depth();
  return TN_OK;
}

extern "C" int tn_dbg_linear(tn_ctx *ctx, const float *x, const float *w, const float *bias, float *y, int M, int N,
                             int K) {
  TN_REQUIRE(ctx && x && w && y, "tn_dbg_linear: null argument");
  TN_ON_DEVICE(ctx->device);
  return launch_linear_f32(x, K, w, K, bias, y, N, M, N, K, 0, ctx->stream);
}

extern "C" int tn_dbg_pack_strip(const float *w1_host, int K, const float *s2_host, const float *t2_host, uint16_t *w1s_out,
                                 const float *w3_host, uint16_t *w3s_out) {
  TN_REQUIRE(K > 0 && K % 32 == 0, "tn_dbg_pack_strip: K must be a multiple of 32");
  if (w1_host && w1s_out) {
    TN_REQUIRE(s2_host && t2_host, "tn_dbg_pack_strip: the 1x1 image needs BN2's scale and shift");
    std::vector<float> wf((size_t)128 * K);
    for (int n = 0; n < 128; ++n)
      for (int k = 0; k < K; ++k) wf[(size_t)n * K + k] = w1_host[(size_t)n * K + k] * s2_host[n];
    const std::vector<f16> p = pack_w1_strip(wf.data(), K, t2_host);
    memcpy(w1s_out, p.data(), p.size() * sizeof(f16));
  }
  if (w3_host && w3s_out) {
    const std::vector<f16> p = pack_w3_strip(w3_host);
    memcpy(w3s_out, p.data(), p.size() * sizeof(f16));
  }
  return TN_OK;
}

extern "C" int tn_dbg_dense_strip_dev(tn_ctx *ctx, void *buf_f16, int ldc, int K, const float *s1, const float *t1,
                                      const void *w1s_f16, const void *w3s_f16, int B, int H, int W, unsigned long long *ts) {
  TN_REQUIRE(ctx && buf_f16 && s1 && t1 && w1s_f16 && w3s_f16, "tn_dbg_dense_strip_dev: null argument");
  DenseStripArgs a{(f16 *)buf_f16, ldc, K, s1, t1, (const f16 *)w1s_f16, (const f16 *)w3s_f16, B, H, W};
  a.ts = ts;
  return launch_dense_strip(a, ctx->stream);
}

extern "C" int tn_dbg_dense_strip_pair_dev(tn_ctx *ctx, void *buf_f16, int ldc, int K, const float *s1, const float *t1,
                                           const void *w1s_f16, const void *w3s_f16, int B, int H, int W, unsigned long long *ts) {
  TN_REQUIRE(ctx && buf_f16 && s1 && t1 && w1s_f16 && w3s_f16, "tn_dbg_dense_strip_pair_dev: null argument");
  DenseStripArgs a{(f16 *)buf_f16, ldc, K, s1, t1, (const f16 *)w1s_f16, (const f16 *)w3s_f16, B, H, W};
  a.ts = ts;
  return launch_dense_strip_pair(a, ctx->stream);
}

extern "C" int tn_dbg_dense_strip_pair_chain_dev(tn_ctx *ctx, void *buf_f16, int ldc, int K0, int nl, const float *const *s1,
                                                 const float *const *t1, const void *const *w1s_f16, const void *const *w3s_f16, int B,
                                                 int H, int W) {
  TN_REQUIRE(ctx && buf_f16 && s1 && t1 && w1s_f16 && w3s_f16, "tn_dbg_dense_strip_pair_chain_dev: null argument");
  TN_REQUIRE(nl > 0 && nl <= 16, "tn_dbg_dense_strip_pair_chain_dev: bad layer count");
  TN_ON_DEVICE(ctx->device);
  std::vector<DenseStripLayerDev> tab(nl);
  for (int l = 0; l < nl; ++l) {
    TN_REQUIRE(s1[l] && t1[l] && w1s_f16[l] && w3s_f16[l], "tn_dbg_dense_strip_pair_chain_dev: null operand");
    tab[l] = DenseStripLayerDev{s1[l], t1[l], (const f16 *)w1s_f16[l], (const f16 *)w3s_f16[l]};
  }
  DenseStripLayerDev *dev = nullptr;
  TN_HIP_CHECK(hipMalloc((void **)&dev, sizeof(DenseStripLayerDev) * nl));
  int rc = TN_OK;
  if (hipMemcpy(dev, tab.data(), sizeof(DenseStripLayerDev) * nl, hipMemcpyHostToDevice) != hipSuccess) {
    tn_set_error("tn_dbg_dense_strip_pair_chain_dev: upload failed");
    rc = TN_ERR_HIP;
  }
  if (rc == TN_OK) {
    const DenseStripChainArgs c{(f16 *)buf_f16, ldc, K0, nl, dev, B, H, W};
    rc = launch_dense_strip_pair_chain(c, ctx->stream);
  }
  const hipError_t he = hipStreamSynchronize(ctx->stream);
  (void)hipFree(dev);
  if (rc == TN_OK && he != hipSuccess) {
    tn_set_error("tn_dbg_dense_strip_pair_chain_dev: the launch failed");
    rc = TN_ERR_HIP;
  }
  return rc;
}


struct tn_dbg_block7 {
  tn_ctx *ctx;
  void *wa = nullptr, *wb = nullptr, *tab = nullptr;
  DenseBlock7Args args;
};

extern "C" int tn_dbg_block7_create(tn_ctx *ctx, int K0, int nl, const float *w1_all, const float *s1_all, const float *t1_all,
                                    const float *s2_all, const float *t2_all, const float *w3_all, void **out) {
  TN_REQUIRE(ctx && w1_all && s1_all && t1_all && s2_all && t2_all && w3_all && out, "tn_dbg_block7_create: null argument");
  TN_REQUIRE(dense_block7_supported(7, 7, K0, nl), std::string("tn_dbg_block7_create: unsupported geometry (dense_block7 runs ") + kDenseBlock7Range + "): 7 x 7, K0 = " + std::to_string(K0) +
                                                       ", nl = " + std::to_string(nl));
  TN_ON_DEVICE(ctx->device);
  std::vector<std::vector<float>> folded(nl);
  std::vector<Block7Layer> layers(nl);
  size_t o1 = 0, ok = 0;
  for (int l = 0; l < nl; ++l) {
    const int K = K0 + 32 * l;
    folded[l].resize((size_t)128 * K);
    for (int n = 0; n < 128; ++n)
      for (int k = 0; k < K; ++k) folded[l][(size_t)n * K + k] = w1_all[o1 + (size_t)n * K + k] * s2_all[(size_t)l * 128 + n];
    layers[l] = Block7Layer{folded[l].data(), w3_all + (size_t)l * 32 * 128 * 9, s1_all + ok, t1_all + ok, t2_all + (size_t)l * 128};
    o1 += (size_t)128 * K;
    ok += K;
  }
  const Block7Image img = pack_block7(layers, K0);
  tn_dbg_block7 *b = new tn_dbg_block7();
  b->ctx = ctx;
  auto up = [&](void **dst, const void *src, size_t bytes) {
    if (hipMalloc(dst, bytes) != hipSuccess) return false;
    return hipMemcpy(*dst, src, bytes, hipMemcpyHostToDevice) == hipSuccess;
  };
  if (!up(&b->wa, img.wa.data(), img.wa.size() * sizeof(f16)) || !up(&b->wb, img.wb.data(), img.wb.size() * sizeof(f16)) ||
      !up(&b->tab, img.tab.data(), img.tab.size() * sizeof(float))) {
    tn_set_error("tn_dbg_block7_create: device allocation failed");
    return TN_ERR_NOMEM;
  }
  b->args = DenseBlock7Args{nullptr, 0, K0, nl, 0, (const f16 *)b->wa, (const f16 *)b->wb, (const float *)b->tab};
  for (int w = 0; w < 4; ++w) { b->args.a_off[w] = img.a_off[w]; b->args.b_off[w] = img.b_off[w]; }
  *out = b;
  return TN_OK;
}

extern "C" int tn_dbg_block7_run_ts(void *handle, void *buf_f16, int ldc, int B, unsigned long long *ts);
extern "C" int tn_dbg_block7_run(void *handle, void *buf_f16, int ldc, int B) { return tn_dbg_block7_run_ts(handle, buf_f16, ldc, B, nullptr); }
extern "C" int tn_dbg_block7_run_ts(void *handle, void *buf_f16, int ldc, int B, unsigned long long *ts) {
  tn_dbg_block7 *b = (tn_dbg_block7 *)handle;
  TN_REQUIRE(b && buf_f16, "tn_dbg_block7_run: null argument");
  TN_ON_DEVICE(b->ctx->device);
  DenseBlock7Args a = b->args;
  a.buf = (f16 *)buf_f16; a.ldc = ldc; a.B = B; a.ts = ts;
  return launch_dense_block7(a, b->ctx->stream);
}

extern "C" void tn_dbg_block7_destroy(void *handle) {
  tn_dbg_block7 *b = (tn_dbg_block7 *)handle;
  if (!b) return;
  (void)hipFree(b->wa); (void)hipFree(b->wb); (void)hipFree(b->tab);
  delete b;
}


struct tn_dbg_stream_block {
  tn_ctx *ctx;
  const DenseStreamKernel *kernel;
  void *stream = nullptr, *scratch = nullptr;
  int scratch_frames = 0;
  DenseStreamArgs args;
};

static_assert(sizeof(kDenseStreamKernels) / sizeof(kDenseStreamKernels[0]) == 2 && kDenseStreamKernels[0].H == 14 && kDenseStreamKernels[1].H == 28,
              "tn_dbg_block14_* / tn_dbg_block28_* index the table");
static int dbg_stream_create(const DenseStreamKernel &sk, tn_ctx *ctx, int K0, int nl, const float *w1_all, const float *s1_all, const float *t1_all,
                             const float *s2_all, const float *t2_all, const float *w3_all, void **out) {
  const std::string who = "tn_dbg_block" + std::to_string(sk.H) + "_create";
  TN_REQUIRE(ctx && w1_all && s1_all && t1_all && s2_all && t2_all && w3_all && out, who + ": null argument");
  TN_REQUIRE(sk.supported(sk.H, sk.H, K0, nl), who + ": unsupported geometry (dense_block" + std::to_string(sk.H) + " runs " + sk.range + "): " + std::to_string(sk.H) + " x " + std::to_string(sk.H) +
                                                   ", K0 = " + std::to_string(K0) + ", nl = " + std::to_string(nl));
  TN_ON_DEVICE(ctx->device);
  std::vector<std::vector<float>> folded(nl);
  std::vector<Block14Layer> layers(nl);
  size_t o1 = 0, ok = 0;
  for (int l = 0; l < nl; ++l) {
    const int K = K0 + 32 * l;
    folded[l].resize((size_t)128 * K);
    for (int n = 0; n < 128; ++n)
      for (int k = 0; k < K; ++k) folded[l][(size_t)n * K + k] = w1_all[o1 + (size_t)n * K + k] * s2_all[(size_t)l * 128 + n];
    layers[l] = Block14Layer{folded[l].data(), w3_all + (size_t)l * 32 * 128 * 9, s1_all + ok, t1_all + ok, t2_all + (size_t)l * 128};
    o1 += (size_t)128 * K;
    ok += K;
  }
  const std::vector<unsigned char> img = sk.pack(layers, K0);
  tn_dbg_stream_block *b = new tn_dbg_stream_block();
  b->ctx = ctx;
  b->kernel = &sk;
  if (hipMalloc(&b->stream, img.size()) != hipSuccess || hipMemcpy(b->stream, img.data(), img.size(), hipMemcpyHostToDevice) != hipSuccess) {
    tn_set_error(who + ": device allocation failed");
    delete b;
    return TN_ERR_NOMEM;
  }
  b->args = DenseStreamArgs{nullptr, 0, K0, nl, 0, (const unsigned char *)b->stream, sk.units(K0, nl)};
  *out = b;
  return TN_OK;
}

static int dbg_stream_run(void *handle, void *buf_f16, int ldc, int B, unsigned long long *ts) {
  tn_dbg_stream_block *b = (tn_dbg_stream_block *)handle;
  TN_REQUIRE(b && buf_f16, "tn_dbg_block14_run / tn_dbg_block28_run: null argument");
  const std::string who = "tn_dbg_block" + std::to_string(b->kernel->H) + "_run";
  TN_REQUIRE(B > 0, who + ": the batch must be positive: " + std::to_string(b->kernel->H) + " x " + std::to_string(b->kernel->H) + ", K0 = " + std::to_string(b->args.K0) +
                        ", nl = " + std::to_string(b->args.nl) + ", ldc = " + std::to_string(ldc) + ", B = " + std::to_string(B));
  TN_ON_DEVICE(b->ctx->device);
  const size_t scratch_bytes = (size_t)B * b->kernel->scratch_halfs() * sizeof(f16);
  if (b->scratch_frames < B) {
    (void)hipFree(b->scratch);
    b->scratch = nullptr; b->scratch_frames = 0;
    if (hipMalloc(&b->scratch, scratch_bytes) != hipSuccess) {
      tn_set_error(who + ": device allocation failed");
      return TN_ERR_NOMEM;
    }
    b->scratch_frames = B;
    TN_HIP_CHECK(hipMemset(b->scratch, 0, scratch_bytes));
  }
  DenseStreamArgs a = b->args;
  a.buf = (f16 *)buf_f16; a.ldc = ldc; a.B = B; a.ts = ts; a.scratch = (f16 *)b->scratch;
  return b->kernel->launch(a, b->ctx->stream);
}

static void dbg_stream_destroy(void *handle) {
  tn_dbg_stream_block *b = (tn_dbg_stream_block *)handle;
  if (!b) return;
  (void)hipFree(b->stream);
  (void)hipFree(b->scratch);
  delete b;
}

extern "C" int tn_dbg_block14_create(tn_ctx *ctx, int K0, int nl, const float *w1_all, const float *s1_all, const float *t1_all,
                                     const float *s2_all, const float *t2_all, const float *w3_all, void **out) {
  return dbg_stream_create(kDenseStreamKernels[0], ctx, K0, nl, w1_all, s1_all, t1_all, s2_all, t2_all, w3_all, out);
}
extern "C" int tn_dbg_block14_run_ts(void *handle, void *buf_f16, int ldc, int B, unsigned long long *ts) { return dbg_stream_run(handle, buf_f16, ldc, B, ts); }
extern "C" int tn_dbg_block14_run(void *handle, void *buf_f16, int ldc, int B) { return dbg_stream_run(handle, buf_f16, ldc, B, nullptr); }
extern "C" void tn_dbg_block14_destroy(void *handle) { dbg_stream_destroy(handle); }

extern "C" int tn_dbg_block28_create(tn_ctx *ctx, int K0, int nl, const float *w1_all, const float *s1_all, const float *t1_all,
                                     const float *s2_all, const float *t2_all, const float *w3_all, void **out) {
  return dbg_stream_create(kDenseStreamKernels[1], ctx, K0, nl, w1_all, s1_all, t1_all, s2_all, t2_all, w3_all, out);
}
extern "C" int tn_dbg_block28_run_ts(void *handle, void *buf_f16, int ldc, int B, unsigned long long *ts) { return dbg_stream_run(handle, buf_f16, ldc, B, ts); }
extern "C" int tn_dbg_block28_run(void *handle, void *buf_f16, int ldc, int B) { return dbg_stream_run(handle, buf_f16, ldc, B, nullptr); }
extern "C" void tn_dbg_block28_destroy(void *handle) { dbg_stream_destroy(handle); }

extern "C" int tn_dbg_gemm_tn(tn_ctx *ctx, const float *A, int lda, const float *B, int ldb, const float *bsc, const float *bsh, float *Cm,
                              int ldc, int M, int N, int K, float *workspace, int64_t workspace_floats) {
  TN_REQUIRE(ctx && A && B && Cm && (bsc == nullptr) == (bsh == nullptr), "tn_dbg_gemm_tn: null argument");
  TN_REQUIRE(M > 0 && N > 0 && K > 0 && lda >= M && ldb >= N && ldc >= N && workspace_floats >= 0, "tn_dbg_gemm_tn: bad shape");
  TN_ON_DEVICE(ctx->device);
  const int rc = bsc ? launch_gemm_tn_f32_bnrelu(A, lda, B, ldb, bsc, bsh, Cm, ldc, M, N, K, ctx->stream, workspace, workspace_floats)
                     : launch_gemm_tn_f32(A, lda, B, ldb, Cm, ldc, M, N, K, ctx->stream, workspace, workspace_floats);
  if (rc) return rc;
  TN_HIP_CHECK(hipStreamSynchronize(ctx->stream));
  return TN_OK;
}

extern "C" int tn_dbg_gemm_nn(tn_ctx *ctx, const float *A, int lda, const float *B, int ldb, float *Cm, int ldc, int M, int N, int K) {
  TN_REQUIRE(ctx && A && B && Cm, "tn_dbg_gemm_nn: null argument");
  TN_REQUIRE(M > 0 && N > 0 && K > 0 && lda >= K && ldb >= N && ldc >= N, "tn_dbg_gemm_nn: bad shape");
  TN_ON_DEVICE(ctx->device);
  const int rc = launch_gemm_nn_f32(A, lda, B, ldb, Cm, ldc, M, N, K, 0, ctx->stream);
  if (rc) return rc;
  TN_HIP_CHECK(hipStreamSynchronize(ctx->stream));
  return TN_OK;
}

extern "C" int tn_dbg_grad_sumsq(tn_ctx *ctx, const float *dev, int64_t n, const float *dev2, int64_t n2, double *sumsq_host) {
  TN_REQUIRE(ctx && sumsq_host, "tn_dbg_grad_sumsq: null argument");
  TN_REQUIRE(n >= 0 && n2 >= 0 && (dev || !n) && (dev2 || !n2), "tn_dbg_grad_sumsq: a non-empty segment needs a pointer, counts >= 0");
  TN_ON_DEVICE(ctx->device);
  void *ws = nullptr;
  const size_t part_bytes = sizeof(float) * TN_GRAD_SUMSQ_GRID;
  TN_HIP_CHECK(hipMalloc(&ws, part_bytes + sizeof(tn_clip_record)));
  tn_clip_record *rec = (tn_clip_record *)((char *)ws + part_bytes), r;
  int rc = launch_grad_sumsq(dev, n, dev2, n2, 1.f, 0.f, (float *)ws, rec, ctx->stream);
  hipError_t e = hipSuccess;
  if (!rc) e = hipMemcpyAsync(&r, rec, sizeof(r), hipMemcpyDeviceToHost, ctx->stream);
  if (!rc && e == hipSuccess) e = hipStreamSynchronize(ctx->stream);
  (void)hipFree(ws);
  if (rc) return rc;
  TN_HIP_CHECK(e);
  *sumsq_host = r.sumsq;
  return TN_OK;
}

extern "C" int tn_dbg_rnn_route(int gates, int B, int H, int dirs, int *nb, int *kr, int *big) {
  TN_REQUIRE(nb && kr && big, "tn_dbg_rnn_route: null argument");
  TN_REQUIRE(gates == 3 || gates == 4, "tn_dbg_rnn_route: gates must be 3 or 4");
  TN_REQUIRE(B > 0 && (dirs == 1 || dirs == 2) && H > 0 && gates * H <= 1024 && H % 4 == 0,
             "tn_dbg_rnn_route: gates*hidden must be <= 1024, hidden % 4 == 0, batch > 0, dirs 1 or 2");
  const tn_rnn_route r = rnn_route(gates, B, H, dirs);
  *nb = r.nb; *kr = r.kr; *big = r.big;
  return TN_OK;
}

extern "C" int tn_dbg_rnn_wide_route(int gates, int B, int H, int dirs, int *threads, int *rows, int *nb, int64_t *lds_fwd, int64_t *lds_bwd) {
  TN_REQUIRE(threads && rows && nb && lds_fwd && lds_bwd, "tn_dbg_rnn_wide_route: null argument");
  TN_REQUIRE(gates == 3 || gates == 4, "tn_dbg_rnn_wide_route: gates must be 3 or 4");
  TN_REQUIRE(B > 0 && (dirs == 1 || dirs == 2) && H > 0 && gates * H > 1024 && gates * H <= 2048 && H % 4 == 0,
             "tn_dbg_rnn_wide_route: gates*hidden must be in (1024, 2048], hidden % 4 == 0, batch > 0, dirs 1 or 2");
  const tn_rnn_wide_route r = rnn_wide_route(gates, B, H, dirs);
  *threads = r.threads; *rows = r.rows; *nb = r.nb; *lds_fwd = (int64_t)r.lds_fwd; *lds_bwd = (int64_t)r.lds_bwd;
  return TN_OK;
}

extern "C" int tn_dbg_rnn_force_wide(int on) {
  rnn_set_force_wide(on != 0);
  return TN_OK;
}

extern "C" int tn_dbg_rnn_wide_launches(int64_t *count) {
  TN_REQUIRE(count, "tn_dbg_rnn_wide_launches: null argument");
  *count = (int64_t)rnn_wide_launches();
  return TN_OK;
}

extern "C" int tn_dbg_trainer_params(int which, const int *dims, int n_dims, const char *prefix_a, const char *prefix_b, tn_param_row *rows,
                                     int max_rows, int *n_rows, int64_t *numel, int64_t *state_numel) {
  TN_REQUIRE(dims && prefix_a && n_rows && (rows || max_rows == 0), "tn_dbg_trainer_params: null argument");
  ParamTable t;
  if (which == TN_TRAINER_HEAD) {
    TN_REQUIRE(n_dims == 4 && prefix_b, "tn_dbg_trainer_params: the head takes (gates, input, hidden, classes) and two prefixes");
    HeadOffsets o;
    t = head_param_table(dims[0], dims[1], dims[2], dims[3], prefix_a, prefix_b, &o);
  } else if (which == TN_TRAINER_GNMT) {
    TN_REQUIRE(n_dims == 7 && dims[5] >= 2 && dims[6] >= 0 && dims[6] < dims[5],
               "tn_dbg_trainer_params: the captioner takes (gates, input, hidden, embed, vocab, num_layers, num_bi_layers < num_layers)");
    GnmtOffsets o;
    t = gnmt_param_table(dims[0], dims[1], dims[2], dims[3], dims[4], dims[5], dims[6], prefix_a, &o);
  } else if (which == TN_TRAINER_BACKBONE) {
    TN_REQUIRE(n_dims == 1 && (dims[0] > 0) == (prefix_b != nullptr),
               "tn_dbg_trainer_params: the backbone takes (classes) and the classifier's prefix, or (0) and none");
    FtNet net;
    t = ft_param_table(prefix_a, prefix_b, dims[0], &net);
  } else {
    TN_REQUIRE(false, "tn_dbg_trainer_params: which must be TN_TRAINER_HEAD, TN_TRAINER_GNMT or TN_TRAINER_BACKBONE");
  }
  for (size_t i = 0; i < t.rows.size() && (int)i < max_rows; ++i) {
    const ParamTable::Row &r = t.rows[i];
    TN_REQUIRE(r.name.size() < sizeof(rows[i].name), "tn_dbg_trainer_params: a name does not fit tn_param_row");
    memset(&rows[i], 0, sizeof(rows[i]));
    memcpy(rows[i].name, r.name.data(), r.name.size());
    rows[i].where = (int)r.where; rows[i].offset = r.off; rows[i].count = r.count;
  }
  *n_rows = (int)t.rows.size();
  if (numel) *numel = t.n;
  if (state_numel) *state_numel = t.ns;
  return TN_OK;
}

static int encoder_plan_stats(int height, int width, int flags, int batch, int calibrate, bool shared_chip, tn_kernel_stat *stats, int max_stats,
                              int *n_stats, int *paired_out) {
  TN_REQUIRE(stats && n_stats && max_stats > 0, "tn_dbg_encoder_plan: null argument");
  TN_REQUIRE((flags & ~TN_ENC_EXACT_WEIGHTS) == 0, "tn_dbg_encoder_plan: unknown flag, or a mode that is not planned (TN_ENC_FP32, TN_ENC_FP32X3)");
  TN_REQUIRE(batch > 0, "tn_dbg_encoder_plan: batch must be positive");
  TN_REQUIRE(height >= 224 && width >= 224 && height <= 1024 && width <= 1024, "tn_dbg_encoder_plan: input size must be in [224,1024]");
  const EncPolicy p = enc_policy(flags);
  const EncGeom g = enc_geom(height, width);
  if (const char *why = enc_refusal(p, g)) { tn_set_error(why); return TN_ERR_INVALID; }
  std::vector<tn_kernel_stat> fams;
  auto add = [&](const std::string &name, const EncCost &c) {
    size_t i = 0;
    while (i < fams.size() && name != fams[i].name) ++i;
    if (i == fams.size()) {
      tn_kernel_stat st;
      memset(&st, 0, sizeof(st));
      strncpy(st.name, name.c_str(), sizeof(st.name) - 1);
      fams.push_back(st);
    }
    fams[i].launches += 1;
    fams[i].flops += c.flops;
    fams[i].bytes += c.bytes;
  };
  const double fB = (double)batch;
  int paired = 0;
  if (p.fuse) {
    add("stem_conv_bn_relu_maxpool", stem_pool_cost(g, fB));
  } else {
    add("stem_conv7x7_bn_relu", stem_cost(g, fB));
    add("maxpool3x3s2", maxpool_cost(g, fB));
  }
  for (int b = 0; b < 4; ++b) {
    const int M = batch * g.Hb[b] * g.Wb[b];
    for (const EncStep &st : enc_block_plan(p, g, b, batch, calibrate != 0, shared_chip)) {
      if (st.paired) ++paired;
      if (st.route == ENC_LAYERWISE) {
        add(family_name(st, g, b), conv1x1_cost(M, enc_layer_cin(g, b, st.l0)));
        add("conv3x3_bnrelu", conv3x3_cost(M));
      } else {
        add(family_name(st, g, b), step_cost(st, g, b, M));
      }
    }
    if (b < 3) add("transition_conv1x1_avgpool", transition_cost(M, batch * g.Hb[b + 1] * g.Wb[b + 1], g.Cb[b], g.Cb[b] / 2));
  }
  add("head_bnrelu_avgpool7", head_cost(g, fB));
  const int n = (int)fams.size() < max_stats ? (int)fams.size() : max_stats;
  for (int i = 0; i < n; ++i) stats[i] = fams[i];
  *n_stats = n;
  if (paired_out) *paired_out = paired;
  return TN_OK;
}

extern "C" int tn_dbg_encoder_plan(int height, int width, int flags, int batch, int calibrate, tn_kernel_stat *stats, int max_stats,
                                   int *n_stats) {
  return encoder_plan_stats(height, width, flags, batch, calibrate, false, stats, max_stats, n_stats, nullptr);
}

extern "C" int tn_dbg_encoder_plan_shared(int height, int width, int flags, int batch, tn_kernel_stat *stats, int max_stats, int *n_stats,
                                          int *paired_out) {
  TN_REQUIRE(paired_out, "tn_dbg_encoder_plan_shared: null argument");
  return encoder_plan_stats(height, width, flags, batch, 0, true, stats, max_stats, n_stats, paired_out);
}

extern "C" int tn_dbg_strip_pair_launches(int64_t *count) {
  TN_REQUIRE(count, "tn_dbg_strip_pair_launches: null argument");
  *count = (int64_t)strip_pair_launches();
  return TN_OK;
}

extern "C" int tn_dbg_gnmt_trainer_src_grad(tn_gnmt_trainer *t, const float *src, const int32_t *src_valid_len, const int32_t *tgt, int ld,
                                            const int32_t *tgt_valid_len, int batch, int steps, int tgt_len, float *loss,
                                            float *logits_out, float *dsrc, int ldd) {
  TN_REQUIRE(t && dsrc, "tn_dbg_gnmt_trainer_src_grad: null argument");
  return gnmt_trainer_step(t, src, src_valid_len, tgt, ld, tgt_valid_len, batch, steps, tgt_len, loss, logits_out, dsrc, ldd);
}

extern "C" int tn_dbg_rows_pad_skip(int on) {
  linear_rows_set_pad_skip(on != 0);
  return TN_OK;
}

extern "C" int tn_dbg_linear_bnrelu(tn_ctx *ctx, const float *X, int ldx, const float *asc, const float *ash, const float *W, int ldw,
                                    const float *bias, float *Y, int ldy, int M, int N, int K, int accumulate) {
  TN_REQUIRE(ctx && X && asc && ash && W && Y, "tn_dbg_linear_bnrelu: null argument");
  TN_REQUIRE(M > 0 && N > 0 && K > 0 && ldx >= K && ldw >= K && ldy >= N, "tn_dbg_linear_bnrelu: bad shape");
  TN_ON_DEVICE(ctx->device);
  const int rc = launch_linear_f32_bnrelu(X, ldx, asc, ash, W, ldw, bias, Y, ldy, M, N, K, accumulate, ctx->stream);
  if (rc) return rc;
  TN_HIP_CHECK(hipStreamSynchronize(ctx->stream));
  return TN_OK;
}

extern "C" int tn_dbg_linear_fp32x3(tn_ctx *ctx, const float *X, int ldx, const float *asc, const float *ash, const float *W, int ldw,
                                    const float *bias, float *Y, int ldy, int M, int N, int K, int accumulate) {
  TN_REQUIRE(ctx && X && W && Y && (asc == nullptr) == (ash == nullptr), "tn_dbg_linear_fp32x3: null argument");
  TN_REQUIRE(M > 0 && N > 0 && K > 0 && ldx >= K && ldw >= K && ldy >= N, "tn_dbg_linear_fp32x3: bad shape");
  TN_ON_DEVICE(ctx->device);
  const int rc = launch_linear_fp32x3(X, ldx, asc, ash, W, ldw, bias, Y, ldy, M, N, K, accumulate, ctx->stream);
  if (rc) return rc;
  TN_HIP_CHECK(hipStreamSynchronize(ctx->stream));
  return TN_OK;
}
extern "C" int tn_dbg_gemm_tn_fp32x3(tn_ctx *ctx, const float *A, int lda, const float *B, int ldb, const float *bsc, const float *bsh,
                                     float *Cm, int ldc, int M, int N, int K, float *workspace, int64_t workspace_floats) {
  TN_REQUIRE(ctx && A && B && Cm && (bsc == nullptr) == (bsh == nullptr), "tn_dbg_gemm_tn_fp32x3: null argument");
  TN_REQUIRE(M > 0 && N > 0 && K > 0 && lda >= M && ldb >= N && ldc >= N && workspace_floats >= 0, "tn_dbg_gemm_tn_fp32x3: bad shape");
  TN_ON_DEVICE(ctx->device);
  const int rc = launch_gemm_tn_fp32x3(A, lda, B, ldb, bsc, bsh, Cm, ldc, M, N, K, ctx->stream, workspace, workspace_floats);
  if (rc) return rc;
  TN_HIP_CHECK(hipStreamSynchronize(ctx->stream));
  return TN_OK;
}

extern "C" int tn_dbg_bn_train(tn_ctx *ctx, const float *x, int ld, int64_t M, int C, const float *gamma, const float *beta, float *mean,
                               float *var, float *y, const float *dy, float *dgamma, float *dbeta, float *dx, int ldd, int accumulate) {
  TN_REQUIRE(ctx && x && gamma && beta && mean && var && y, "tn_dbg_bn_train: null argument");
  TN_REQUIRE(!dy || (dgamma && dbeta && dx), "tn_dbg_bn_train: dy needs dgamma, dbeta and dx");
  TN_REQUIRE(M > 0 && C > 0 && ld >= C && (!dy || ldd >= C), "tn_dbg_bn_train: bad shape");
  TN_ON_DEVICE(ctx->device);
  float *ws = nullptr;
  TN_HIP_CHECK(hipMalloc((void **)&ws, sizeof(float) * ft_bn_ws_floats((long)M, C)));
  int rc = launch_ft_bn_stats(x, ld, (long)M, C, ws, mean, var, ctx->stream);
  if (!rc) rc = launch_ft_bn_relu(x, ld, (long)M, C, mean, var, gamma, beta, y, ctx->stream);
  if (!rc && dy) rc = launch_ft_bn_backward(dy, x, ld, (long)M, C, mean, var, gamma, beta, ws, dgamma, dbeta, dx, ldd, accumulate, ctx->stream);
  const hipError_t e = hipStreamSynchronize(ctx->stream);
  (void)hipFree(ws);
  if (rc) return rc;
  TN_HIP_CHECK(e);
  TN_HIP_CHECK(hipGetLastError());
  return TN_OK;
}

extern "C" int tn_dbg_conv_fp32x3(tn_ctx *ctx, int which, int kind, int tile, int layout, const void *x, int ldx, int K, const float *s,
                                  const float *t, const float *w_host, int N, const float *es, const float *et, float *y, int ldy, int yoff,
                                  int64_t M, int H, int W, int Ho, int Wo) {
  TN_REQUIRE(ctx && x && w_host && y, "tn_dbg_conv_fp32x3: null argument");
  TN_REQUIRE(which == 0 || which == 1, "tn_dbg_conv_fp32x3: which must be 0 (fp32x3) or 1 (fp32)");
  TN_REQUIRE(which == 0 || tile == 0, "tn_dbg_conv_fp32x3: the fp32 kernel takes its launcher's tile");
  TN_REQUIRE(kind >= FP32_STEM && kind <= FP32_TRANS, "tn_dbg_conv_fp32x3: unknown kind");
  TN_REQUIRE(layout >= 0 && layout <= 2, "tn_dbg_conv_fp32x3: unknown input layout");
  TN_REQUIRE(M > 0 && K > 0 && N > 0 && N % 32 == 0 && H > 0 && W > 0 && Ho > 0 && Wo > 0 && M % ((int64_t)Ho * Wo) == 0,
             "tn_dbg_conv_fp32x3: bad shape (M = B Ho Wo, N a multiple of 32)");
  if (kind == FP32_STEM) {
    TN_REQUIRE(K == 147 && es && et && Ho == (H - 1) / 2 + 1 && Wo == (W - 1) / 2 + 1, "tn_dbg_conv_fp32x3: the stem has K = 147, an epilogue and a ((H - 1) / 2 + 1) x ((W - 1) / 2 + 1) output");
  } else {
    TN_REQUIRE(s && t && !es && !et && K % 32 == 0 && ldx % 4 == 0, "tn_dbg_conv_fp32x3: s / t, no epilogue, K a multiple of 32");
    TN_REQUIRE(kind == FP32_3X3 ? (K == 1152 && ldx == 128) : ldx >= K, "tn_dbg_conv_fp32x3: K beyond the channel stride (3x3: K = 1152, ldx = 128)");
    TN_REQUIRE(kind == FP32_TRANS ? (2 * Ho <= H && 2 * Wo <= W) : (Ho == H && Wo == W), "tn_dbg_conv_fp32x3: output map size does not fit the input's");
  }
  TN_ON_DEVICE(ctx->device);
  const int kp = (K + 31) / 32 * 32;
  std::vector<float> wk((size_t)kp * N, 0.f);
  memcpy(wk.data(), w_host, (size_t)K * N * sizeof(float));
  float *wd = nullptr;
  uint16_t *wx = nullptr;
  if (which == 0) wx = up(fp32x3_pack_weights(wk.data(), kp, N));
  else wd = up(wk);
  TN_REQUIRE(wd || wx, "tn_dbg_conv_fp32x3: device allocation failed");
  Fp32ConvArgs a{};
  a.kind = kind; a.x = x; a.layout = layout; a.ldx = ldx; a.K = K; a.s = s; a.t = t; a.w = wd; a.wx = wx; a.N = N; a.es = es; a.et = et;
  a.y = y; a.ldy = ldy; a.yoff = yoff; a.M = (long)M; a.H = H; a.W = W; a.Ho = Ho; a.Wo = Wo;
  const int rc = which == 0 ? launch_conv_fp32x3(a, ctx->stream, tile) : launch_conv_fp32(a, ctx->stream);
  const hipError_t e = hipStreamSynchronize(ctx->stream);
  (void)hipFree(wd); (void)hipFree(wx);
  if (rc) return rc;
  TN_HIP_CHECK(e);
  return TN_OK;
}
```

### tennis_amd/csrc/dense_block7.hip

```cpp
#include <cstring>
#include <type_traits>
#include <utility>

#include "common.h"

#ifndef TN_B7_EXP
#define TN_B7_EXP 0
#endif

namespace {

typedef unsigned u32x4 __attribute__((ext_vector_type(4)));

#define TN_INL __attribute__((always_inline))
template <int N, typename F>
__device__ __forceinline__ void static_for(F &&f) {
  [&]<int... I>(std::integer_sequence<int, I...>) TN_INL { (f(std::integral_constant<int, I>{}), ...); }(std::make_integer_sequence<int, N>{});
}
template <int V>
using ic = std::integral_constant<int, V>;
#define TN_SB() __builtin_amdgcn_sched_barrier(0)

constexpr int kPix = 49;
constexpr int kChunkRow = kPix * 16;
constexpr int kActBytes = 128 * kChunkRow;
constexpr int kSlotPitch = 272;
constexpr int kZeroSlot = 49, kDumpSlot = 50;
constexpr int kTileOff = kActBytes, kTileBytes = 51 * kSlotPitch;
constexpr int kRedOff = kTileOff + kTileBytes, kRedBytes = 4 * 8192;
constexpr int kTabOff = kRedOff + kRedBytes;
constexpr int kTabFloats = 512 + 512 + 128;
constexpr int kLdsBytes = kTabOff + kTabFloats * 4;
static_assert(kLdsBytes <= 160 * 1024, "LDS");
constexpr int kStepUnits = 256;
constexpr int kW3Units = 18 * 64;

__device__ __forceinline__ f32x16 mfma32(const f16x8 a, const f16x8 b, const f32x16 c) {
  return __builtin_amdgcn_mfma_f32_32x32x16_f16(a, b, c, 0, 0, 0);
}

template <int D>
__global__ void __launch_bounds__(256) __attribute__((amdgpu_waves_per_eu(1, 1))) dense_block7_kernel(DenseBlock7Args a) {
  extern __shared__ __attribute__((aligned(16))) unsigned char smem[];
  const int tid = threadIdx.x, lane = tid & 63, n = lane & 31, h = lane >> 5;
  const int w = __builtin_amdgcn_readfirstlane(tid >> 6);
  f16 *xb = a.buf + (size_t)blockIdx.x * kPix * a.ldc;

  auto lds_h8 = [&](unsigned ad) TN_INL -> f16x8 { return *(const f16x8 *)(smem + ad); };
  auto lds_f4 = [&](unsigned ad) TN_INL -> f32x4 { return *(const f32x4 *)(smem + ad); };

  const f16x8 *wa = (const f16x8 *)a.wa + a.a_off[w];
  const f16x8 *wb = (const f16x8 *)a.wb + a.b_off[w];
  f16x8 ring[D][4];
  static_for<D>([&](auto i_tag) TN_INL {
    static_for<4>([&](auto m_tag) TN_INL { ring[i_tag.value][m_tag.value] = wa[i_tag.value * kStepUnits + m_tag.value * 64 + lane]; });
  });
  wa += D * kStepUnits;

  {
    const int c8 = a.K0 >> 3, total = c8 * kPix;
    for (int idx = tid; idx < total; idx += 256) {
      const int p = idx / c8, c = idx - p * c8;
      *(f16x8 *)(smem + c * kChunkRow + p * 16) = *(const f16x8 *)(xb + (size_t)p * a.ldc + c * 8);
    }
    if (tid < kSlotPitch / 16) *(u32x4 *)(smem + kTileOff + kZeroSlot * kSlotPitch + tid * 16) = (u32x4){0, 0, 0, 0};
    const f32x4 *tb = (const f32x4 *)a.tab;
    f32x4 *tl = (f32x4 *)(smem + kTabOff);
    tl[tid] = tb[tid];
    if (tid < 32) tl[256 + tid] = tb[256 + tid];
  }
  __syncthreads();

  const unsigned aaddr0 = (unsigned)(h * kPix + n) * 16;
  const unsigned caddr0 = kTabOff + h * 16;
  unsigned waddr[2], offb[9][2];
#pragma unroll
  for (int t = 0; t < 2; ++t) {
    const int p = 32 * t + n, y = p / 7, x = p - 7 * y;
    const unsigned cell = (unsigned)(4 * w + h) * 16;
    waddr[t] = kTileOff + (p < kPix ? p : kDumpSlot) * kSlotPitch + cell;
#pragma unroll
    for (int tap = 0; tap < 9; ++tap) {
      const int yy = y + tap / 3 - 1, xx = x + tap % 3 - 1;
      const bool ok = p < kPix && yy >= 0 && yy < 7 && xx >= 0 && xx < 7;
      offb[tap][t] = kTileOff + (ok ? yy * 7 + xx : kZeroSlot) * kSlotPitch + cell;
    }
  }

  f32x16 acc[4][2];

  u32x4 raw[2][2], x[2][2];
  u32x4 cs[2][2];
  auto read_step = [&](unsigned aad, unsigned cad, auto i_tag) TN_INL {
    constexpr int I = decltype(i_tag)::value, Bf = I & 1;
    raw[Bf][0] = __builtin_bit_cast(u32x4, lds_h8(aad + I * 2 * kChunkRow));
    raw[Bf][1] = __builtin_bit_cast(u32x4, lds_h8(aad + I * 2 * kChunkRow + 512));
    cs[Bf][0] = __builtin_bit_cast(u32x4, lds_h8(cad + I * 32));
    cs[Bf][1] = __builtin_bit_cast(u32x4, lds_h8(cad + I * 32 + 2048));
  };
  auto bn_pair = [&](auto u_tag, auto par_tag) TN_INL {
    constexpr int U = decltype(u_tag)::value, T = U >> 1, D0 = 2 * (U & 1), D1 = D0 + 1, PAR = decltype(par_tag)::value;
    const unsigned in0 = raw[PAR][T][D0], in1 = raw[PAR][T][D1];
    const unsigned l0 = cs[PAR][0][D0], l1 = cs[PAR][0][D1], h0 = cs[PAR][1][D0], h1 = cs[PAR][1][D1];
    unsigned o0, o1;
    asm("v_pk_max_f16 %0, %2, %4\n\tv_pk_max_f16 %1, %3, %5\n\tv_pk_min_f16 %0, %0, %6\n\tv_pk_min_f16 %1, %1, %7"
        : "=&v"(o0), "=&v"(o1) : "v"(in0), "v"(in1), "v"(l0), "v"(l1), "v"(h0), "v"(h1));
    x[PAR][T][D0] = o0;
    x[PAR][T][D1] = o1;
  };
  auto step = [&](auto p_tag, auto kind_tag, auto last_tag, unsigned aad, unsigned cad) TN_INL {
    constexpr int P = decltype(p_tag)::value, S = P % D, KIND = decltype(kind_tag)::value, PAR = P & 1;
    constexpr int LAST = decltype(last_tag)::value;
    constexpr bool NEXT = LAST == 0 || P + 1 <= LAST, NEXT2 = LAST == 0 || P + 2 <= LAST;
    static_for<8>([&](auto j_tag) TN_INL {
      constexpr int J = decltype(j_tag)::value, M = J >> 1, T = J & 1;
      if constexpr (J == 0 && NEXT2 && !(TN_B7_EXP & 4)) read_step(aad, cad, ic<P + 2>{});
      if constexpr (P == 0) {
        f32x16 z;
#pragma unroll
        for (int e = 0; e < 16; ++e) z[e] = 0.f;
        acc[M][T] = mfma32(ring[S][M], __builtin_bit_cast(f16x8, x[PAR][T]), z);
      } else {
        acc[M][T] = mfma32(ring[S][M], __builtin_bit_cast(f16x8, x[PAR][T]), acc[M][T]);
      }
      if constexpr (NEXT && !(TN_B7_EXP & 2) && (J & 1) == 0) bn_pair(ic<(J >> 1)>{}, ic<PAR ^ 1>{});
      if constexpr (T == 1 && KIND == 1 && !(TN_B7_EXP & 1)) ring[S][M] = wa[M * 64 + lane];
      if constexpr (T == 1 && KIND == 2 && !(TN_B7_EXP & 1)) ring[S][M] = wa[S * kStepUnits + M * 64 + lane];
      TN_SB();
    });
    if constexpr (KIND == 1) wa += kStepUnits;
  };

  int nstamp = 0;
  auto stamp = [&]() TN_INL {
    if (a.ts) {
      const unsigned long long tnow = __builtin_amdgcn_s_memtime();
      if (w == 0 && lane == 0 && nstamp < 126) a.ts[(size_t)blockIdx.x * 128 + nstamp] = tnow;
      ++nstamp;
    }
  };
  if (a.ts && w == 0 && lane == 0) a.ts[(size_t)blockIdx.x * 128 + 127] = __builtin_amdgcn_s_memrealtime();
  stamp();
  int K = a.K0;
  for (int l = 0; l < a.nl; ++l, K += 32) {
    const int G = K >> 4, gbase = G >> 2, grem = G & 3;
    const int nA = gbase + (w < grem ? 1 : 0);
    const int g0 = w * gbase + (w < grem ? w : grem);

    __builtin_amdgcn_s_waitcnt(0x0F70);

    unsigned aad = aaddr0 + (unsigned)g0 * (2 * kChunkRow), cad = caddr0 + (unsigned)g0 * 32;
    read_step(aad, cad, ic<0>{});
    read_step(aad, cad, ic<1>{});
    static_for<4>([&](auto u_tag) TN_INL { bn_pair(u_tag, ic<0>{}); });
    TN_SB();
    step(ic<0>{}, ic<1>{}, ic<0>{}, aad, cad);
#ifdef TN_B7_STAMPS_A
    stamp();
#endif
    int b = 0;
    while (b + 2 * D + 1 <= nA) {
      static_for<D>([&](auto i_tag) TN_INL { step(ic<decltype(i_tag)::value + 1>{}, ic<1>{}, ic<0>{}, aad, cad); });
      aad += D * 2 * kChunkRow;
      cad += D * 32;
      b += D;
    }
#ifdef TN_B7_STAMPS_A
    stamp();
#endif
    const int r = nA - 1 - b - D;
    static_for<D>([&](auto r_tag) TN_INL {
      constexpr int R = decltype(r_tag)::value;
      if (r == R) {
        static_for<D + R>([&](auto i_tag) TN_INL {
          constexpr int P = decltype(i_tag)::value + 1;
          step(ic<P>{}, ic<(P <= R ? 1 : 2)>{}, ic<D + R>{}, aad, cad);
        });
      }
    });
    wa += D * kStepUnits;
    f16x8 w3f[18];
    static_for<18>([&](auto u_tag) TN_INL { w3f[u_tag.value] = wb[u_tag.value * 64 + lane]; });
    wb += kW3Units;
    stamp();

    const float *tbn = a.tab + (size_t)(l + 1) * kTabFloats;
    f32x4 tv0, tv2;
    static_for<3>([&](auto rd_tag) TN_INL {
      constexpr int RD = decltype(rd_tag)::value + 1;
      {
        const unsigned base = kRedOff + (unsigned)((w + RD) & 3) * 8192 + lane * 16;
        static_for<8>([&](auto i_tag) TN_INL {
          constexpr int T = decltype(i_tag)::value >> 2, Q = decltype(i_tag)::value & 3;
          const f32x16 v = acc[RD][T];
          *(f32x4 *)(smem + base + T * 4096 + Q * 1024) = (f32x4){v[4 * Q], v[4 * Q + 1], v[4 * Q + 2], v[4 * Q + 3]};
        });
      }
      __syncthreads();
      if constexpr (RD == 1) {
        if (l + 1 < a.nl) {
          tv0 = ((const f32x4 *)tbn)[tid];
          if (tid < 32) tv2 = ((const f32x4 *)tbn)[256 + tid];
        }
      }
      {
        const unsigned base = kRedOff + (unsigned)w * 8192 + lane * 16;
        static_for<8>([&](auto i_tag) TN_INL {
          constexpr int T = decltype(i_tag)::value >> 2, Q = decltype(i_tag)::value & 3;
          const f32x4 v = lds_f4(base + T * 4096 + Q * 1024);
          acc[0][T][4 * Q] += v[0];
          acc[0][T][4 * Q + 1] += v[1];
          acc[0][T][4 * Q + 2] += v[2];
          acc[0][T][4 * Q + 3] += v[3];
        });
      }
      if constexpr (RD < 3) __syncthreads();
    });

    stamp();
    {
      const unsigned t2ad = kTabOff + 4096 + (unsigned)(32 * w + 4 * h) * 4;
      f32x4 sh[4];
      static_for<4>([&](auto g_tag) TN_INL { sh[g_tag.value] = lds_f4(t2ad + g_tag.value * 32); });
      static_for<2>([&](auto t_tag) TN_INL {
        constexpr int T = decltype(t_tag)::value;
        f16x8 lo, hi;
        static_for<8>([&](auto j_tag) TN_INL {
          constexpr int J = decltype(j_tag)::value;
          lo[J] = (f16)fmaxf(acc[0][T][J] + sh[J >> 2][J & 3], 0.f);
          hi[J] = (f16)fmaxf(acc[0][T][8 + J] + sh[2 + (J >> 2)][J & 3], 0.f);
        });
        *(f16x8 *)(smem + waddr[T]) = lo;
        *(f16x8 *)(smem + waddr[T] + 32) = hi;
      });
    }

    stamp();
    f32x16 q[2];
    f16x8 bq[2][2];
    bq[0][0] = lds_h8(offb[0][0]);
    bq[0][1] = lds_h8(offb[0][1]);
    static_for<36>([&](auto i_tag) TN_INL {
      constexpr int I = decltype(i_tag)::value, U = I >> 1, T = I & 1, TAP = U >> 1, SS = U & 1;
      if constexpr (U + 1 < 18) bq[(U + 1) & 1][T] = lds_h8(offb[(U + 1) >> 1][T] + ((U + 1) & 1) * 32);
      if constexpr (U == 0) {
        f32x16 z;
#pragma unroll
        for (int j = 0; j < 16; ++j) z[j] = 0.f;
        q[T] = mfma32(w3f[U], bq[U & 1][T], z);
      } else {
        q[T] = mfma32(w3f[U], bq[U & 1][T], q[T]);
      }
      (void)TAP; (void)SS;
      TN_SB();
    });

    stamp();
    {
      const unsigned base = kRedOff + (unsigned)w * 8192 + lane * 16;
      static_for<8>([&](auto i_tag) TN_INL {
        constexpr int T = decltype(i_tag)::value >> 2, Q = decltype(i_tag)::value & 3;
        *(f32x4 *)(smem + base + T * 4096 + Q * 1024) = (f32x4){q[T][4 * Q], q[T][4 * Q + 1], q[T][4 * Q + 2], q[T][4 * Q + 3]};
      });
    }
    __syncthreads();
    {
      const int tf = w & 1, sf = w >> 1;
      f32x4 o0 = {0.f, 0.f, 0.f, 0.f}, o1 = {0.f, 0.f, 0.f, 0.f};
      static_for<4>([&](auto x_tag) TN_INL {
        const unsigned base = kRedOff + decltype(x_tag)::value * 8192 + (unsigned)tf * 4096 + (unsigned)(2 * sf) * 1024 + lane * 16;
        o0 += lds_f4(base);
        o1 += lds_f4(base + 1024);
      });
      f16x8 ov;
#pragma unroll
      for (int j = 0; j < 4; ++j) {
        ov[j] = (f16)o0[j];
        ov[4 + j] = (f16)o1[j];
      }
      const int p = 32 * tf + n;
      if (p < kPix) {
        *(f16x8 *)(smem + (unsigned)((K >> 3) + 2 * sf + h) * kChunkRow + p * 16) = ov;
        *(f16x8 *)(xb + (size_t)p * a.ldc + K + 16 * sf + 8 * h) = ov;
        if (a.side) {
          float *sp = a.side + ((size_t)blockIdx.x * kPix + p) * a.ldc + K + 16 * sf + 8 * h;
          *(f32x4 *)sp = o0;
          *(f32x4 *)(sp + 4) = o1;
        }
      }
      if (l + 1 < a.nl) {
        f32x4 *tl = (f32x4 *)(smem + kTabOff);
        tl[tid] = tv0;
        if (tid < 32) tl[256 + tid] = tv2;
      }
    }
    __syncthreads();
    stamp();
  }
  if (a.ts && w == 0 && lane == 0) a.ts[(size_t)blockIdx.x * 128 + 126] = __builtin_amdgcn_s_memrealtime();
}

constexpr int kRingDepth = 6;

}

bool dense_block7_supported(int H, int W, int K0, int nl) {
  return H == 7 && W == 7 && K0 % 32 == 0 && K0 >= 64 * (kRingDepth + 1) && nl >= 1 && K0 + 32 * nl <= 1024;
}

Block7Image pack_block7(const std::vector<Block7Layer> &layers, int K0) {
  Block7Image img;
  const int nl = (int)layers.size();
  std::vector<f16> wave_a[4], wave_b[4];
  for (int l = 0; l < nl; ++l) {
    const Block7Layer &L = layers[l];
    const int K = K0 + 32 * l, G = K / 16, gbase = G / 4, grem = G % 4;
    for (int w = 0; w < 4; ++w) {
      const int nA = gbase + (w < grem ? 1 : 0), g0 = w * gbase + (w < grem ? w : grem);
      for (int sidx = 0; sidx < nA; ++sidx)
        for (int m = 0; m < 4; ++m) {
          const int M = (w + m) & 3, g = g0 + sidx;
          for (int lane = 0; lane < 64; ++lane)
            for (int i = 0; i < 8; ++i)
              wave_a[w].push_back((f16)L.w1f[(size_t)(32 * M + (lane & 31)) * K + 16 * g + 8 * (lane >> 5) + i]);
        }
      for (int tap = 0; tap < 9; ++tap)
        for (int s = 0; s < 2; ++s)
          for (int lane = 0; lane < 64; ++lane) {
            const int r = lane & 31, h = lane >> 5;
            const int co = 16 * (r >> 4) + 8 * ((r >> 2) & 1) + (r & 3) + 4 * ((r >> 3) & 1);
            for (int i = 0; i < 8; ++i) {
              const int cb = 32 * w + (i & 3) + 8 * (2 * s + (i >> 2)) + 4 * h;
              wave_b[w].push_back((f16)L.w3[((size_t)co * 128 + cb) * 9 + tap]);
            }
          }
    }
    img.tab.resize((size_t)(l + 1) * kTabFloats, 0.f);
    float *tb = img.tab.data() + (size_t)l * kTabFloats;
    f16 *th = (f16 *)tb;
    for (int k = 0; k < K; ++k) {
      th[k] = (f16)L.s1[k];
      th[1024 + k] = (f16)L.t1[k];
    }
    memcpy(tb + 1024, L.t2, sizeof(float) * 128);
  }
  for (int w = 0; w < 4; ++w) {
    wave_a[w].resize(wave_a[w].size() + (size_t)kRingDepth * kStepUnits * 8, (f16)0.f);
    img.a_off[w] = (unsigned)(img.wa.size() / 8);
    img.wa.insert(img.wa.end(), wave_a[w].begin(), wave_a[w].end());
    img.b_off[w] = (unsigned)(img.wb.size() / 8);
    img.wb.insert(img.wb.end(), wave_b[w].begin(), wave_b[w].end());
  }
  return img;
}

int launch_dense_block7(const DenseBlock7Args &a, hipStream_t s) {
  const std::string geom = "7 x 7, K0 = " + std::to_string(a.K0) + ", nl = " + std::to_string(a.nl) + ", ldc = " + std::to_string(a.ldc) + ", B = " + std::to_string(a.B);
  TN_REQUIRE(dense_block7_supported(7, 7, a.K0, a.nl), std::string("dense_block7: unsupported geometry (this kernel runs ") + kDenseBlock7Range + "): " + geom);
  TN_REQUIRE(a.ldc % 8 == 0, "dense_block7: the row pitch must be a multiple of 8: " + geom);
  TN_REQUIRE(a.K0 + 32 * a.nl <= a.ldc, "dense_block7: the row pitch does not hold the last layer's output: " + geom);
  TN_REQUIRE(a.B > 0, "dense_block7: the batch must be positive: " + geom);
  TN_SET_ATTR_ONCE_PER_DEVICE(TN_HIP_CHECK(hipFuncSetAttribute((const void *)dense_block7_kernel<kRingDepth>, hipFuncAttributeMaxDynamicSharedMemorySize, kLdsBytes)));
  hipLaunchKernelGGL((dense_block7_kernel<kRingDepth>), dim3(a.B), dim3(256), kLdsBytes, s, a);
  TN_HIP_CHECK(hipGetLastError());
  return TN_OK;
}
```

### tennis_amd/csrc/encoder.hip

```cpp
#include <cmath>
#include <cstdlib>
#include <cstring>
#include <string>
#include <vector>

#include "api_internal.h"
#include "encoder_plan.h"

namespace {

constexpr float kBnEps = 1e-5f;

bool fold_bn(const ParamMap &pm, const std::string &name, int c, std::vector<float> &scale, std::vector<float> &shift) {
  const float *g = pm.get(name + "_gamma", c), *b = pm.get(name + "_beta", c);
  const float *mu = pm.get(name + "_running_mean", c), *var = pm.get(name + "_running_var", c);
  if (!g || !b || !mu || !var) return false;
  scale.resize(c);
  shift.resize(c);
  bn_scale_shift(g, b, mu, var, c, kBnEps, scale.data(), shift.data());
  return true;
}

std::vector<f16> to_f16(const float *w, size_t n) {
  std::vector<f16> h(n + 64, (f16)0.f);
// ... 457 lines not shown
      L.cin = enc_layer_cin(g, b, l);
      const float *w1 = pm.get(sp + "conv" + std::to_string(2 * l) + "_weight", (int64_t)128 * L.cin);
      const float *w3 = pm.get(sp + "conv" + std::to_string(2 * l + 1) + "_weight", 32 * 128 * 9);
      if (!w1 || !w3) return fail(TN_ERR_MISSING);
      if (!fold_bn(pm, sp + "batchnorm" + std::to_string(2 * l), L.cin, s, t)) return fail(TN_ERR_MISSING);
      if (b == 0) centre_shift(s, t);
      std::vector<float> sw1(L.cin), tc1(L.cin);
      bn_relu_clamp_fold(std::vector<float>(s).data(), std::vector<float>(t).data(), L.cin, s.data(), t.data(), sw1.data(), tc1.data());
      L.s1 = e->pool.upload(s); L.t1 = e->pool.upload(t);
      if (b == 0)
        for (int c = 0; c < 64; ++c) e->calib_centre.push_back(s[c] != t[c] ? e->stem_centre[c] : 0.f);
      std::vector<float> x0(L.cin);
      for (int k = 0; k < L.cin; ++k) x0[k] = std::fmin(std::fmax(0.f, s[k]), t[k]);
      if (sk || block7) hl.push_back(BlockLayerHost{{}, s, t, {}, w3});
      if (!fold_bn(pm, sp + "batchnorm" + std::to_string(2 * l + 1), 128, s, t)) return fail(TN_ERR_MISSING);
      std::vector<float> w1f((size_t)128 * L.cin);
      bool in_range = true;
      for (int n = 0; n < 128; ++n) {
        double bias = 0.0, corr = 0.0;
        for (int k = 0; k < L.cin; ++k) {
          const float wf = s[n] * sw1[k] * w1[(size_t)n * L.cin + k];
          w1f[(size_t)n * L.cin + k] = wf;
          in_range = in_range && std::fabs(wf) <= 65504.0f;
          bias += (double)w1[(size_t)n * L.cin + k] * ((double)tc1[k] + (double)sw1[k] * (double)x0[k]);
          if (x0[k] != 0.f) {
            const float hi = (float)(f16)wf;
            const double weff = p.exact ? (double)hi + (double)(float)(f16)(wf - hi) : (double)hi;
            corr += weff * (double)x0[k];
          }
        }
        t[n] = (float)((double)t[n] + (double)s[n] * bias - corr);
      }
      if (!in_range) { tn_set_error("a 1x1 weight leaves the fp16 range once its BatchNorm scales are folded in (" + sp + "conv" + std::to_string(2 * l) + ")"); return fail(TN_ERR_INVALID); }
      if (p.exact) {
        const int bk = enc_exact_ktile(p, g, b, l);
        L.w1 = e->pool.upload(split_hi_lo_rows(w1f.data(), 128, L.cin, (L.cin + bk - 1) / bk * bk));
      } else {
        L.w1 = e->pool.upload(to_f16(w1f.data(), (size_t)128 * L.cin));
      }
      if (sk || block7) { hl.back().w1f = w1f; hl.back().t2 = t; }
      if (enc_layer_strip(p, g, b, l)) L.w1s = e->pool.upload(pack_w1_strip(w1f.data(), L.cin, t.data()));
      L.s2 = e->pool.upload(std::vector<float>(128, 1.0f)); L.t2 = e->pool.upload(t);
      if (p.exact) {
        std::vector<float> hi(32 * 128 * 9), lo(32 * 128 * 9);
        for (size_t i = 0; i < hi.size(); ++i) {
          hi[i] = (float)(f16)w3[i];
          lo[i] = w3[i] - hi[i];
        }
        std::vector<f16> img = pack_conv3x3(hi.data());
        const std::vector<f16> img_lo = pack_conv3x3(lo.data());
        img.insert(img.end(), img_lo.begin(), img_lo.end());
        L.w3p = e->pool.upload(img);
      } else {
        L.w3p = e->pool.upload(pack_conv3x3(w3));
      }
      if (L.w1s) L.w3s = e->pool.upload(pack_w3_strip(w3));
      e->layers[b].push_back(L);
    }
    if (sk) {
      DenseStreamArgs &as = e->b_stream[b];
      as.stream = e->pool.upload(sk->pack(block_layers<Block14Layer>(hl), g.Cin[b]));
      as.total_units = sk->units(g.Cin[b], kBlockCfg[b]);
      as.ldc = g.Cb[b]; as.K0 = g.Cin[b]; as.nl = kBlockCfg[b];
    } else if (block7) {
      const Block7Image img = pack_block7(block_layers<Block7Layer>(hl), g.Cin[b]);
      DenseBlock7Args &a7 = e->b7[b];
      a7.wa = e->pool.upload(img.wa); a7.wb = e->pool.upload(img.wb); a7.tab = e->pool.upload(img.tab);
      for (int w = 0; w < 4; ++w) { a7.a_off[w] = img.a_off[w]; a7.b_off[w] = img.b_off[w]; }
      a7.ldc = g.Cb[b]; a7.K0 = g.Cin[b]; a7.nl = kBlockCfg[b];
    }
    {
      std::vector<DenseLayerDev> cd;
      for (auto &L : e->layers[b]) cd.push_back(DenseLayerDev{L.s1, L.t1, L.w1, L.s2, L.t2, L.w3p});
      e->chain_dev[b] = e->pool.upload(cd);
    }
    if (const int nl = enc_strip_chain_layers(p, g, b)) {
      std::vector<DenseStripLayerDev> sd;
      for (int l = 0; l < nl; ++l) {
        const auto &L = e->layers[b][l];
        sd.push_back(DenseStripLayerDev{L.s1, L.t1, L.w1s, L.w3s});
      }
      e->strip_chain_dev[b] = e->pool.upload(sd);
    }
    if (b < 3) {
      auto &T = e->trans[b];
      T.cin = g.Cb[b]; T.cout = g.Cb[b] / 2;
      const float *wt = pm.get(pre + "conv" + std::to_string(outer) + "_weight", (int64_t)T.cout * T.cin);
      if (!wt || !fold_bn(pm, pre + "batchnorm" + std::to_string(outer), T.cin, s, t)) return fail(TN_ERR_MISSING);
      if (b == 0) centre_shift(s, t);
      T.s = e->pool.upload(s); T.t = e->pool.upload(t);
      T.w = p.exact ? e->pool.upload(split_hi_lo_rows(wt, T.cout, T.cin, T.cin))
                     : e->pool.upload(to_f16(wt, (size_t)T.cout * T.cin));
      if (!p.exact && (T.cout == 512 || T.cout == 256) && T.cin % 128 == 0) {
        const std::vector<f16> wh = to_f16(wt, (size_t)T.cout * T.cin);
        T.wfrag = e->pool.upload(pack_trans_frags(wh.data(), T.cout, T.cin));
      }
      ++outer;
    }
  }
  if (!fold_bn(pm, pre + "batchnorm" + std::to_string(outer), g.Cb[3], s, t)) return fail(TN_ERR_MISSING);
  e->head_s = e->pool.upload(s); e->head_t = e->pool.upload(t);

  const size_t weights_bytes = e->pool.bytes;
  e->interleave = getenv("TN_NO_INTERLEAVE") == nullptr && e->split && max_batch >= 64;
  const size_t B = (size_t)max_batch * (e->interleave ? 2 : 1);
  e->stem_out = (f16 *)e->pool.alloc(B * g.Hs * g.Ws * 64 * sizeof(f16));
  e->bott = (f16 *)e->pool.alloc(B * g.Hb[0] * g.Wb[0] * 128 * sizeof(f16));
  for (int b = 0; b < 4; ++b)
    e->blockbuf[b] = (f16 *)e->pool.alloc(B * g.Hb[b] * g.Wb[b] * g.Cb[b] * sizeof(f16));
  if (enc_block7(p, g, 3)) e->head32 = (float *)e->pool.alloc(B * g.Hb[3] * g.Wb[3] * g.Cb[3] * sizeof(float));
  for (int b = 0; b < 4; ++b)
    if (const DenseStreamKernel *sk = enc_stream_kernel(p, g, b)) e->b_stream_scratch[b] = (f16 *)e->pool.alloc(B * sk->scratch_halfs() * sizeof(f16));
  e->workspace_bytes = e->pool.bytes - weights_bytes;
  if (e->pool.failed) { tn_set_error("device allocation failed"); return fail(TN_ERR_NOMEM); }
  for (int b = 0; b < 4; ++b)
    if (const DenseStreamKernel *sk = enc_stream_kernel(p, g, b))
      if (hipMemset(e->blockbuf[b], 0, B * g.Hb[b] * g.Wb[b] * g.Cb[b] * sizeof(f16)) != hipSuccess ||
          hipMemset(e->b_stream_scratch[b], 0, B * sk->scratch_halfs() * sizeof(f16)) != hipSuccess) {
        tn_set_error("hipMemset failed");
        return fail(TN_ERR_HIP);
      }
  *out = e;
  return TN_OK;
}

extern "C" int tn_densenet121_feature_dim(const tn_encoder *enc) { return enc ? enc->geom.feat_dim : 0; }
extern "C" size_t tn_densenet121_workspace_bytes(const tn_encoder *enc) { return enc ? enc->workspace_bytes : 0; }

static int encoder_run_range(tn_encoder *e, const void *x0, tn_layout layout, int b0, int B, float *feat0,
                             hipStream_t s, EventTimer &tm, int ws0 = -1, bool shared_chip = false) {
  int rc;
  const EncGeom &g = e->geom;
  const EncPolicy &p = e->policy;
  const double fB = (double)B;
  const size_t frame_bytes = (size_t)g.H * g.W * 3 * (layout == TN_LAYOUT_NCHW_F32 ? 4 : layout == TN_LAYOUT_NHWC_F16 ? 2 : 1);
  const void *x = (const unsigned char *)x0 + (size_t)b0 * frame_bytes;
  float *feat = feat0 + (size_t)b0 * g.feat_dim;
  const int w0 = ws0 >= 0 ? ws0 : b0;
  float *cam = e->cam_w ? e->cam_out + (size_t)b0 * e->cam_units * 49 * g.PH * g.PW : nullptr;
  if (e->fp32) return encoder_run_range_fp32(e, x, layout, B, feat, s, tm, w0, cam);
  f16 *stem_out = e->stem_out + (size_t)w0 * g.Hs * g.Ws * 64;
  f16 *bott = e->bott + (size_t)w0 * g.Hb[0] * g.Wb[0] * 128;
  f16 *bbuf[4];
  for (int b = 0; b < 4; ++b) bbuf[b] = e->blockbuf[b] + (size_t)w0 * g.Hb[b] * g.Wb[b] * g.Cb[b];
  const bool cal = e->calib_dev != nullptr;
  float *cal_out = e->calib_dev;
  auto cal_mean = [&](const f16 *xin, int ld, int K, const float *sc, const float *sh, long rows, int clamp = 0) {
    const int rc2 = launch_channel_mean(xin, ld, K, sc, sh, rows, e->calib_scratch, cal_out, s, clamp);
    cal_out += K;
    return rc2;
  };
  std::vector<EncStep> plan[4];
  for (int b = 0; b < 4; ++b) plan[b] = enc_block_plan(p, g, b, B, cal, shared_chip);
  float *h32 = plan[3][0].route == ENC_BLOCK7 ? e->head32 + (size_t)w0 * g.Hb[3] * g.Wb[3] * g.Cb[3] : nullptr;
  auto begin = [&](const std::string &family, const EncCost &c) { tm.begin(family.c_str(), c.flops, c.bytes); };
  {
    StemArgs a{x, (int)layout, B, g.H, g.W, e->stem_wp, e->stem_wp_zf, e->stem_scale, e->stem_shift, stem_out, g.Hs, g.Ws};
    a.shift_u8 = e->stem_shift_u8;
    a.wp_zf_lo = e->stem_wp_zf_lo;
    a.floor = e->stem_floor;
    if (p.fuse) {
      begin("stem_conv_bn_relu_maxpool", stem_pool_cost(g, fB));
      rc = launch_stem_pool(a, bbuf[0], g.Cb[0], g.Hb[0], g.Wb[0], s);
      tm.end();
      if (rc) return rc;
    } else {
      begin("stem_conv7x7_bn_relu", stem_cost(g, fB));
      rc = launch_stem(a, s);
      tm.end();
      if (rc) return rc;
      begin("maxpool3x3s2", maxpool_cost(g, fB));
      rc = launch_maxpool3x3s2(stem_out, B, g.Hs, g.Ws, 64, bbuf[0], g.Cb[0], g.Hb[0], g.Wb[0], s);
      tm.end();
      if (rc) return rc;
    }
  }
  for (int b = 0; b < 4; ++b) {
    const int Hh = g.Hb[b], Ww = g.Wb[b];
    const int M = B * Hh * Ww;
    for (const EncStep &st : plan[b]) {
      auto &L = e->layers[b][st.l0];
      if (st.route != ENC_LAYERWISE) begin(family_name(st, g, b), step_cost(st, g, b, M));
      switch (st.route) {
        case ENC_STREAM14:
        case ENC_STREAM28: {
          const DenseStreamKernel &sk = kDenseStreamKernels[st.route];
          DenseStreamArgs as = e->b_stream[b];
          as.buf = bbuf[b]; as.B = B;
          as.scratch = e->b_stream_scratch[b] + (size_t)w0 * sk.scratch_halfs();
          rc = sk.launch(as, s);
          break;
        }
        case ENC_BLOCK7: {
          DenseBlock7Args a7 = e->b7[b];
          a7.buf = bbuf[b]; a7.B = B;
          a7.side = b == 3 ? h32 : nullptr;
          rc = launch_dense_block7(a7, s);
          break;
        }
        case ENC_CHAIN_TILE:
        case ENC_TILE: {
          const bool ch = st.route == ENC_CHAIN_TILE;
          DenseLayerArgs af{bbuf[b], g.Cb[b], L.cin, L.s1, L.t1, L.w1, L.s2, L.t2, L.w3p, B, Hh, Ww, nullptr, p.dl_variant, ch ? e->chain_dev[b] + st.l0 : nullptr, ch ? st.nl : 0};
          af.exact = p.exact;
          rc = launch_dense_layer(af, s);
          break;
        }
        case ENC_STRIP_CHAIN: {
          DenseStripChainArgs ac{bbuf[b], g.Cb[b], g.Cin[b], st.nl, e->strip_chain_dev[b], B, Hh, Ww};
          rc = st.paired ? launch_dense_strip_pair_chain(ac, s) : launch_dense_strip_chain(ac, s);
          break;
        }
        case ENC_STRIP: {
          DenseStripArgs as{bbuf[b], g.Cb[b], L.cin, L.s1, L.t1, L.w1s, L.w3s, B, Hh, Ww};
          rc = st.paired ? launch_dense_strip_pair(as, s) : launch_dense_strip(as, s);
          break;
        }
        default: {
          if (cal && (rc = cal_mean(bbuf[b], g.Cb[b], L.cin, L.s1, L.t1, M, 1))) return rc;
          Conv1x1Args a1{bbuf[b], g.Cb[b], L.cin, L.s1, L.t1, L.w1, 128, bott, 128, 0, M, 0, Hh, Ww};
          a1.bias = L.t2;
          a1.clamp = 1;
          a1.exact = p.exact;
          begin(family_name(st, g, b), conv1x1_cost(M, L.cin));
          rc = launch_conv1x1(a1, s);
          tm.end();
          if (rc) return rc;
          if (cal && (rc = cal_mean(bott, 128, 128, e->ones128, e->zeros128, M))) return rc;
          Conv3x3Args a3{bott, L.s2, e->zeros128, L.w3p, bbuf[b], g.Cb[b], L.cin, M, Hh, Ww};
          a3.exact = p.exact;
          begin("conv3x3_bnrelu", conv3x3_cost(M));
          rc = launch_conv3x3(a3, s);
        }
      }
      tm.end();
      if (rc) return rc;
    }
    if (b < 3) {
      auto &T = e->trans[b];
      const int Mo = B * g.Hb[b + 1] * g.Wb[b + 1];
      if (cal && (rc = cal_mean(bbuf[b], g.Cb[b], T.cin, T.s, T.t, M))) return rc;
      Conv1x1Args at{bbuf[b], g.Cb[b], T.cin, T.s, T.t, T.w, T.cout, bbuf[b + 1], g.Cb[b + 1], 0, Mo, 1, Hh, Ww};
      at.exact = p.exact;
      at.wfrag = cal ? nullptr : T.wfrag;
      if (b == 2 && h32) { at.y32 = h32; at.ld32 = g.Cb[3]; }
      begin("transition_conv1x1_avgpool", transition_cost(M, Mo, T.cin, T.cout));
      rc = launch_conv1x1(at, s);
      tm.end();
      if (rc) return rc;
    }
  }
  begin("head_bnrelu_avgpool7", head_cost(g, fB));
  rc = launch_head(bbuf[3], B, g.Hb[3], g.Wb[3], g.Cb[3], e->head_s, e->head_t, feat, g.PH, g.PW, s, h32);
  tm.end();
  if (rc || !cam) return rc;
  tm.begin("class_maps", 2.0 * fB * 49 * g.feat_dim * e->cam_units, fB * g.Hb[3] * g.Wb[3] * g.Cb[3] * (h32 ? 4 : 2) + fB * e->cam_units * 49 * g.PH * g.PW * 4);
  rc = launch_class_maps(bbuf[3], h32, B, g.Hb[3], g.Wb[3], g.Cb[3], e->head_s, e->head_t, e->cam_w, g.PH, g.PW, e->cam_units, cam, s);
  tm.end();
  return rc;
}

static int encoder_run(tn_encoder *e, const void *x, tn_layout layout, int B, float *feat, EventTimer &tm) {
  TN_REQUIRE(e && x && feat, "tn_densenet121_forward: null argument");
  TN_REQUIRE(B > 0 && B <= e->maxB, "tn_densenet121_forward: batch exceeds max_batch");
  TN_ON_DEVICE(e->ctx->device);
  hipStream_t s = e->ctx->stream;
  e->last_batch = B;
  const int ns = e->nsplit;
  const bool split = e->split && !tm.on && B >= 32 * ns && (B % (8 * ns)) == 0;
  const int par = (int)(e->calls & 1);
  e->calls++;
  e->last_ws0 = 0;
  if (!split) {
    if (e->pipelined) {
      for (int h = 0; h < e->split_of[par ^ 1]; ++h) TN_HIP_CHECK(hipStreamWaitEvent(s, e->ev_done[par ^ 1][h], 0));
      for (int h = 0; h < ns; ++h) TN_HIP_CHECK(hipStreamWaitEvent(s, e->ev_done[par][h], 0));
    }
    e->split_of[par] = 0;
    return encoder_run_range(e, x, layout, 0, B, feat, s, tm);
  }
  if (e->pipelined && e->interleave && B / ns >= e->policy.strip_min_batch) {
    TN_HIP_CHECK(hipEventRecord(e->ev_in, s));
    TN_HIP_CHECK(hipStreamWaitEvent(e->side[par], e->ev_in, 0));
    if (!e->last_interleaved)
      for (int p2 = 0; p2 < 2; ++p2)
        for (int g = 0; g < e->split_of[p2]; ++g) TN_HIP_CHECK(hipStreamWaitEvent(e->side[par], e->ev_done[p2][g], 0));
    e->last_interleaved = true;
    e->last_ws0 = par * e->maxB;
    const int r = encoder_run_range(e, x, layout, 0, B, feat, e->side[par], tm, par * e->maxB, true);
    TN_HIP_CHECK(hipEventRecord(e->ev_done[par][0], e->side[par]));
    e->split_of[par] = 1;
    e->split_batch = 0;
    return r;
  }
  if (e->last_interleaved) {
    for (int h = 0; h < ns; ++h)
      for (int p2 = 0; p2 < 2; ++p2)
        for (int g = 0; g < e->split_of[p2]; ++g) TN_HIP_CHECK(hipStreamWaitEvent(e->side[h], e->ev_done[p2][g], 0));
    e->last_interleaved = false;
  }
  TN_HIP_CHECK(hipEventRecord(e->ev_in, s));
  if (e->pipelined && e->split_batch != 0 && e->split_batch != B) {
    for (int h = 0; h < ns; ++h)
      for (int p2 = 0; p2 < 2; ++p2)
        for (int g = 0; g < e->split_of[p2]; ++g) TN_HIP_CHECK(hipStreamWaitEvent(e->side[h], e->ev_done[p2][g], 0));
  }
  e->split_batch = B;
  int rc = TN_OK;
  for (int h = 0; h < ns; ++h) {
    TN_HIP_CHECK(hipStreamWaitEvent(e->side[h], e->ev_in, 0));
    const int r = encoder_run_range(e, x, layout, h * (B / ns), B / ns, feat, e->side[h], tm);
    if (r) rc = r;
    TN_HIP_CHECK(hipEventRecord(e->ev_done[par][h], e->side[h]));
    if (!e->pipelined) TN_HIP_CHECK(hipStreamWaitEvent(s, e->ev_done[par][h], 0));
  }
  e->split_of[par] = ns;
  return rc;
}

static int encoder_join(tn_encoder *e, int lag) {
  if (e->calls - 1 - lag < 0) return TN_OK;
  const int par = (int)((e->calls - 1 - lag) & 1);
  for (int h = 0; h < e->split_of[par]; ++h) TN_HIP_CHECK(hipStreamWaitEvent(e->ctx->stream, e->ev_done[par][h], 0));
  return TN_OK;
}

extern "C" int tn_densenet121_set_pipelined(tn_encoder *enc, int on) {
  TN_REQUIRE(enc, "tn_densenet121_set_pipelined: null handle");
  TN_ON_DEVICE(enc->ctx->device);
  if (enc->pipelined && !on) {
    int rc = encoder_join(enc, 0);
    if (rc == TN_OK) rc = encoder_join(enc, 1);
    if (rc) return rc;
  }
  enc->pipelined = on != 0;
  return TN_OK;
}

extern "C" int tn_densenet121_join(tn_encoder *enc, int lag) {
  TN_REQUIRE(enc, "tn_densenet121_join: null handle");
  TN_REQUIRE(lag == 0 || lag == 1, "tn_densenet121_join: lag must be 0 (the last forward) or 1 (the one before)");
  TN_ON_DEVICE(enc->ctx->device);
  return encoder_join(enc, lag);
}

extern "C" int tn_densenet121_forward(tn_encoder *enc, const void *x, tn_layout layout, int batch, float *feat) {
  EventTimer tm;
  return encoder_run(enc, x, layout, batch, feat, tm);
}

extern "C" int tn_densenet121_class_map_dims(const tn_encoder *enc, int *h, int *w) {
  TN_REQUIRE(enc && h && w, "tn_densenet121_class_map_dims: null argument");
  *h = 7 * enc->geom.PH;
  *w = 7 * enc->geom.PW;
  return TN_OK;
}

static int class_maps_check(const char *fn, tn_encoder *enc, const void *x, float *feat, const tn_dense *classes, float *maps) {
  const std::string f(fn);
  TN_REQUIRE(enc, f + ": null encoder");
  TN_REQUIRE(x, f + ": x is null");
  TN_REQUIRE(feat, f + ": features is null");
  TN_REQUIRE(classes, f + ": classes is null");
  TN_REQUIRE(maps, f + ": maps is null");
  TN_REQUIRE(classes->ctx == enc->ctx, f + ": classes belongs to another context than the encoder");
  TN_REQUIRE(classes->in_units == enc->geom.feat_dim, f + ": classes has in_units " + std::to_string(classes->in_units) + ", the encoder's feature width is " +
                                                          std::to_string(enc->geom.feat_dim));
  TN_REQUIRE(classes->units <= 64, f + ": classes has " + std::to_string(classes->units) + " units, the maps take at most 64");
  TN_REQUIRE(enc->calib_dev == nullptr, f + ": a calibration pass is in progress");
  return TN_OK;
}

extern "C" int tn_densenet121_forward_class_maps(tn_encoder *enc, const void *x, tn_layout layout, int batch, float *feat,
                                                 const tn_dense *classes, float *maps) {
  if (int rc = class_maps_check("tn_densenet121_forward_class_maps", enc, x, feat, classes, maps)) return rc;
  enc->cam_w = classes->w; enc->cam_out = maps; enc->cam_units = classes->units;
  EventTimer tm;
  const int rc = encoder_run(enc, x, layout, batch, feat, tm);
  enc->cam_w = nullptr; enc->cam_out = nullptr; enc->cam_units = 0;
  return rc;
}

extern "C" int tn_dbg_profile_class_maps(tn_encoder *enc, const void *x, tn_layout layout, int batch, float *feat,
                                                 const tn_dense *classes, float *maps, tn_kernel_stat *stats, int max_stats, int *n_stats) {
  TN_REQUIRE(stats && n_stats, "tn_dbg_profile_class_maps: null argument");
  if (int rc = class_maps_check("tn_dbg_profile_class_maps", enc, x, feat, classes, maps)) return rc;
  enc->cam_w = classes->w; enc->cam_out = maps; enc->cam_units = classes->units;
  EventTimer tm;
  tm.on = true;
  tm.s = enc->ctx->stream;
  const int rc = encoder_run(enc, x, layout, batch, feat, tm);
  tm.finish();
  enc->cam_w = nullptr; enc->cam_out = nullptr; enc->cam_units = 0;
  if (rc) return rc;
  const int n = (int)tm.fams.size() < max_stats ? (int)tm.fams.size() : max_stats;
  for (int i = 0; i < n; ++i) stats[i] = tm.fams[i];
  *n_stats = n;
  return TN_OK;
}

extern "C" int tn_densenet121_profile(tn_encoder *enc, const void *x, tn_layout layout, int batch, float *feat,
                                      tn_kernel_stat *stats, int max_stats, int *n_stats) {
  TN_REQUIRE(enc && stats && n_stats, "tn_densenet121_profile: null argument");
  EventTimer tm;
// ... 107 lines not shown
```

### tennis_amd/csrc/encoder_plan.h

```cpp
#pragma once
#include <cstdlib>
#include <string>
#include <vector>

#include "common.h"

inline constexpr int kBlockCfg[4] = {6, 12, 24, 16};

struct EncPolicy {
  bool fuse = true;
  bool chain = true;
  bool chain28 = true;
  int chain28_min_batch = 128;
  bool exact = false;
  bool strip = true;
  bool strip_chain = true;
  int strip_min_batch = 64;
  bool strip_pair = true;
  int strip_pair_min_batch = 256;
  bool block7 = true;
  bool block_stream[2] = {true, false};
  int dl_variant = 0;
};
static_assert(sizeof(kDenseStreamKernels) / sizeof(kDenseStreamKernels[0]) == 2 && kDenseStreamKernels[0].H == 14 && kDenseStreamKernels[1].H == 28,
              "block_stream[] is indexed like kDenseStreamKernels");

inline EncPolicy enc_policy(int flags) {
  EncPolicy p;
  const bool fp32 = (flags & (TN_ENC_FP32 | TN_ENC_FP32X3)) != 0;
  p.fuse = getenv("TN_NO_FUSE") == nullptr;
  p.chain = getenv("TN_NO_CHAIN") == nullptr;
  p.exact = (flags & TN_ENC_EXACT_WEIGHTS) != 0 && !fp32;
  p.strip = getenv("TN_NO_STRIP") == nullptr && !p.exact && p.fuse;
  p.strip_chain = getenv("TN_NO_STRIP_CHAIN") == nullptr;
  p.chain28 = p.chain && getenv("TN_NO_CHAIN28") == nullptr;
  if (getenv("TN_CHAIN28_MIN_BATCH")) p.chain28_min_batch = atoi(getenv("TN_CHAIN28_MIN_BATCH"));
  if (getenv("TN_STRIP_MIN_BATCH")) p.strip_min_batch = atoi(getenv("TN_STRIP_MIN_BATCH"));
  p.strip_pair = getenv("TN_NO_STRIP_PAIR") == nullptr;
  if (getenv("TN_STRIP_PAIR_MIN_BATCH")) p.strip_pair_min_batch = atoi(getenv("TN_STRIP_PAIR_MIN_BATCH"));
  p.block7 = getenv("TN_NO_BLOCK7") == nullptr;
  p.block_stream[0] = getenv("TN_NO_BLOCK14") == nullptr;
  p.block_stream[1] = getenv("TN_BLOCK28") != nullptr && atoi(getenv("TN_BLOCK28")) != 0;
  p.dl_variant = getenv("TN_DL_VARIANT") ? atoi(getenv("TN_DL_VARIANT")) : 0;
  return p;
}

struct EncGeom {
  int H, W;
  int Hs, Ws;
  int Hb[4], Wb[4];
  int Cin[4], Cb[4];
  int PH, PW, feat_dim;
};
inline EncGeom enc_geom(int height, int width) {
  EncGeom g;
  g.H = height; g.W = width;
  g.Hs = (height + 6 - 7) / 2 + 1; g.Ws = (width + 6 - 7) / 2 + 1;
  int h = (g.Hs + 2 - 3) / 2 + 1, w = (g.Ws + 2 - 3) / 2 + 1, c = 64;
  for (int b = 0; b < 4; ++b) {
    g.Hb[b] = h; g.Wb[b] = w; g.Cin[b] = c; g.Cb[b] = c + 32 * kBlockCfg[b];
    c = g.Cb[b] / 2; h /= 2; w /= 2;
  }
  g.PH = g.Hb[3] / 7; g.PW = g.Wb[3] / 7;
  g.feat_dim = g.Cb[3] * g.PH * g.PW;
  return g;
}
inline const char *enc_refusal(const EncPolicy &p, const EncGeom &g) {
  if (g.PH < 1 || g.PW < 1) return "input too small for AvgPool2D(7)";
  if (g.Wb[0] > 240) return "input too wide for the conv3x3 LDS tile";
  if (p.exact && !(p.fuse && (p.dl_variant & ~256) == 0)) return "TN_ENC_EXACT_WEIGHTS needs the default kernels (no TN_NO_FUSE, no TN_DL_VARIANT)";
  return nullptr;
}

inline int enc_layer_cin(const EncGeom &g, int b, int l) { return g.Cin[b] + 32 * l; }

inline const DenseStreamKernel *enc_stream_kernel(const EncPolicy &p, const EncGeom &g, int b) {
  for (const DenseStreamKernel &k : kDenseStreamKernels)
    if (p.fuse && p.block_stream[&k - kDenseStreamKernels] && !p.exact && k.supported(g.Hb[b], g.Wb[b], g.Cin[b], kBlockCfg[b])) return &k;
  return nullptr;
}
inline bool enc_block7(const EncPolicy &p, const EncGeom &g, int b) {
  return !enc_stream_kernel(p, g, b) && p.fuse && p.block7 && !p.exact && dense_block7_supported(g.Hb[b], g.Wb[b], g.Cin[b], kBlockCfg[b]);
}
inline bool enc_layer_strip(const EncPolicy &p, const EncGeom &g, int b, int l) {
  return p.strip && dense_strip_supported(g.Hb[b], g.Wb[b], enc_layer_cin(g, b, l));
}
inline int enc_strip_chain_layers(const EncPolicy &p, const EncGeom &g, int b) {
  if (!p.strip_chain) return 0;
  const int nl = dense_strip_chain_layers(g.Hb[b], g.Wb[b], g.Cin[b]);
  if (nl <= 0 || nl > kBlockCfg[b]) return 0;
  for (int l = 0; l < nl; ++l)
    if (!enc_layer_strip(p, g, b, l)) return 0;
  return nl;
}
inline bool enc_layer_tile(const EncPolicy &p, const EncGeom &g, int b, int l) {
  return p.fuse && dense_layer_supported(g.Hb[b], g.Wb[b]) && enc_layer_cin(g, b, l) <= dense_layer_kmax(g.Wb[b]);
}
inline int enc_exact_ktile(const EncPolicy &p, const EncGeom &g, int b, int l) {
  return !enc_layer_tile(p, g, b, l) ? 64 : (g.Hb[b] == 14 || g.Hb[b] == 7) ? 64 : 32;
}
inline bool enc_block_chained_tile(const EncPolicy &p, const EncGeom &g, int b) {
  const int Hh = g.Hb[b], Ww = g.Wb[b];
  return p.chain && (p.dl_variant & ~(32 | 64 | 128 | 256 | 512)) == 0 && Hh == Ww && (Hh == 14 || Hh == 7 || Hh == 16) &&
         enc_layer_tile(p, g, b, kBlockCfg[b] - 1);
}
inline bool enc_chain28(const EncPolicy &p, const EncGeom &g, int b, int l0) {
  if (!p.chain28 || p.exact || p.dl_variant != 0 || g.Hb[b] != 28 || g.Wb[b] != 28) return false;
  if (kBlockCfg[b] - l0 < 2 || enc_layer_cin(g, b, l0) < 64) return false;
  for (int l = l0; l < kBlockCfg[b]; ++l)
    if (!enc_layer_tile(p, g, b, l)) return false;
  return true;
}

enum EncRoute { ENC_STREAM14, ENC_STREAM28, ENC_BLOCK7, ENC_CHAIN_TILE, ENC_STRIP_CHAIN, ENC_STRIP, ENC_TILE, ENC_LAYERWISE, ENC_NROUTES };
struct EncRouteName { const char *name; bool geo; };
inline constexpr EncRouteName kEncRouteNames[] = {
    {kDenseStreamKernels[0].family, false}, {kDenseStreamKernels[1].family, false}, {"dense_block_lds_7x7", false},
    {"dense_block_chained_", true}, {"dense_block_strip_", true}, {"dense_layer_strip_", true}, {"dense_layer_fused_", true},
    {"conv1x1_bnrelu", false},
};
static_assert(sizeof(kEncRouteNames) / sizeof(kEncRouteNames[0]) == ENC_NROUTES && ENC_STREAM14 == 0 && ENC_STREAM28 == 1,
              "kEncRouteNames is indexed by EncRoute, whose first two values index kDenseStreamKernels");

struct EncStep { EncRoute route; int l0, nl; bool paired = false; };

inline std::string family_name(const EncStep &st, const EncGeom &g, int b) {
  const EncRouteName &n = kEncRouteNames[st.route];
  return n.geo ? n.name + std::to_string(g.Hb[b]) + "x" + std::to_string(g.Wb[b]) : std::string(n.name);
}

inline bool enc_strip_pair(const EncPolicy &p, const EncGeom &g, int b, int B, bool cal, bool shared_chip) {
  return shared_chip && p.strip_pair && p.strip && !p.exact && p.dl_variant == 0 && !cal && g.Hb[b] == 28 && g.Wb[b] == 28 &&
         B >= p.strip_pair_min_batch && B % 2 == 0;
}

inline std::vector<EncStep> enc_block_plan(const EncPolicy &p, const EncGeom &g, int b, int B, bool cal, bool shared_chip) {
  const int n = kBlockCfg[b], Hh = g.Hb[b];
  std::vector<EncStep> plan;
  if (cal) {
    for (int l = 0; l < n; ++l) plan.push_back({ENC_LAYERWISE, l, 1});
    return plan;
  }
  const bool tuned = p.dl_variant != 0;
  const bool paired = enc_strip_pair(p, g, b, B, cal, shared_chip);
  if (const DenseStreamKernel *sk = tuned ? nullptr : enc_stream_kernel(p, g, b)) return {{(EncRoute)(sk - kDenseStreamKernels), 0, n}};
  if (!tuned && enc_block7(p, g, b)) return {{ENC_BLOCK7, 0, n}};
  if (enc_block_chained_tile(p, g, b)) return {{ENC_CHAIN_TILE, 0, n}};
  int l = !tuned && B >= p.strip_min_batch ? enc_strip_chain_layers(p, g, b) : 0;
  if (l > 0) plan.push_back({ENC_STRIP_CHAIN, 0, l, paired});
  const bool strip_fills = B * (Hh == 128 ? 5 : Hh == 64 ? 3 : 1) >= p.strip_min_batch;
  for (; l < n; ++l) {
    const EncRoute r = !tuned && strip_fills && enc_layer_strip(p, g, b, l) ? ENC_STRIP : enc_layer_tile(p, g, b, l) ? ENC_TILE : ENC_LAYERWISE;
    if (r == ENC_TILE && B >= p.chain28_min_batch && enc_chain28(p, g, b, l)) {
      plan.push_back({ENC_CHAIN_TILE, l, n - l});
      break;
    }
    plan.push_back({r, l, 1, r == ENC_STRIP && paired});
  }
  return plan;
}

struct EncCost { double flops = 0, bytes = 0; };
inline EncCost layer_cost(int M, int cin) { return {2.0 * M * (128.0 * cin + 32.0 * 1152), (double)M * (cin + 32) * 2 + 128.0 * cin * 2 + 32.0 * 1152 * 2}; }
inline EncCost step_cost(const EncStep &st, const EncGeom &g, int b, int M) {
  EncCost c;
  for (int l = st.l0; l < st.l0 + st.nl; ++l) {
    const EncCost one = layer_cost(M, enc_layer_cin(g, b, l));
    c.flops += one.flops; c.bytes += one.bytes;
  }
  return c;
}
inline EncCost conv1x1_cost(int M, int cin) { return {2.0 * M * 128.0 * cin, (double)M * (cin + 128) * 2 + 128.0 * cin * 2}; }
inline EncCost conv3x3_cost(int M) { return {2.0 * M * 32.0 * 1152, (double)M * (128 + 32) * 2 + 32.0 * 1152 * 2}; }
inline EncCost transition_cost(int M, int Mo, int cin, int cout) {
  return {2.0 * M * (double)cout * cin, (double)M * cin * 2 + (double)Mo * cout * 2 + (double)cout * cin * 2};
}
inline EncCost stem_pool_cost(const EncGeom &g, double fB) { return {2.0 * (fB * g.Hs * g.Ws) * 64 * 147, fB * g.H * g.W * 3 * 2 + fB * g.Hb[0] * g.Wb[0] * 64 * 2}; }
inline EncCost stem_cost(const EncGeom &g, double fB) { return {2.0 * (fB * g.Hs * g.Ws) * 64 * 147, fB * g.H * g.W * 3 * 2 + (fB * g.Hs * g.Ws) * 64 * 2}; }
inline EncCost maxpool_cost(const EncGeom &g, double fB) { return {0.0, (fB * g.Hs * g.Ws) * 64 * 2 + fB * g.Hb[0] * g.Wb[0] * 64 * 2}; }
inline EncCost head_cost(const EncGeom &g, double fB) { return {0.0, fB * g.Hb[3] * g.Wb[3] * g.Cb[3] * 2 + fB * g.feat_dim * 4}; }
```

### tennis_amd/csrc/trans_ws.hip

```cpp
#include <type_traits>
#include <utility>
#include <vector>

#include "common.h"

#ifndef TN_TWS_EXP
#define TN_TWS_EXP 0
#endif

namespace {

constexpr int BK = 64;
template <int BM, int NB>
struct TG {
  static constexpr int XT = BM * 128;
  static constexpr int CPITCH = NB * 2 + 16;
  static constexpr int LDS_BYTES = BM * CPITCH > 4 * XT ? BM * CPITCH : 4 * XT;
  static constexpr int SR = BM / 32;
  static constexpr int NCT = NB / 4 / 32, NPT = BM / 32;
  static_assert(NCT * NPT == 8, "128 accumulator registers");
};

__device__ __forceinline__ void lds_barrier() {
  asm volatile("s_waitcnt lgkmcnt(0)" ::: "memory");
  __builtin_amdgcn_s_barrier();
  asm volatile("" ::: "memory");
}

template <int V>
using ic = std::integral_constant<int, V>;

template <int NK, int BM, int NB>
__global__ __launch_bounds__(512) __attribute__((amdgpu_waves_per_eu(2, 2))) void trans_ws_kernel(Conv1x1Args a, int TPF, int PT) {
  using G = TG<BM, NB>;
  constexpr int XT = G::XT, CPITCH = G::CPITCH, SR = G::SR, NCT = G::NCT, NPT = G::NPT;
  extern __shared__ __attribute__((aligned(16))) unsigned char smem[];
  const int t = threadIdx.x, lane = t & 63;
  const int wid = __builtin_amdgcn_readfirstlane(t >> 6);
  const int Wo = a.W >> 1, Ho = a.H >> 1, P = Wo * Ho;
  const int frame = (int)blockIdx.x / TPF, p0 = ((int)blockIdx.x % TPF) * PT;
  const int nrow = P - p0 < PT ? P - p0 : PT;
  const int K = a.K, nk = NK ? NK : K / BK;

  if (wid < 4) {
    const int c = t & 7, r0 = t >> 3;
    const f16 *xsrc[SR][4];
#pragma unroll
    for (int i = 0; i < SR; ++i) {
      int p = r0 + 32 * i;
      p = p0 + (p < nrow ? p : nrow - 1);
      const int py = p / Wo, px = p - py * Wo;
      const long base = ((long)(frame * a.H + 2 * py) * a.W + 2 * px);
      xsrc[i][0] = a.x + base * a.ldx;
      xsrc[i][1] = a.x + (base + 1) * a.ldx;
      xsrc[i][2] = a.x + (base + a.W) * a.ldx;
      xsrc[i][3] = a.x + (base + a.W + 1) * a.ldx;
    }
    f16x8 xr[2][SR][4];
    float scb[2][8], shb[2][8];
    auto load = [&](int kt, auto b_tag) {
      constexpr int PB = decltype(b_tag)::value;
      kt = kt < nk ? kt : nk - 1;
      const int kc = kt * BK + c * 8;
      const float4 s0 = *(const float4 *)(a.scale + kc), s1 = *(const float4 *)(a.scale + kc + 4);
      const float4 t0 = *(const float4 *)(a.shift + kc), t1 = *(const float4 *)(a.shift + kc + 4);
      float (&sc)[8] = scb[PB], (&sh)[8] = shb[PB];
      sc[0] = s0.x; sc[1] = s0.y; sc[2] = s0.z; sc[3] = s0.w; sc[4] = s1.x; sc[5] = s1.y; sc[6] = s1.z; sc[7] = s1.w;
      sh[0] = t0.x; sh[1] = t0.y; sh[2] = t0.z; sh[3] = t0.w; sh[4] = t1.x; sh[5] = t1.y; sh[6] = t1.z; sh[7] = t1.w;
#pragma unroll
      for (int i = 0; i < SR; ++i)
#pragma unroll
        for (int s = 0; s < 4; ++s) xr[PB][i][s] = *(const f16x8 *)(xsrc[i][s] + kc);
    };
    auto stage = [&](auto b_tag) {
      constexpr int PB = decltype(b_tag)::value;
      unsigned char *Xs = smem + PB * 2 * XT, *Xl = Xs + XT;
#pragma unroll
      for (int i = 0; i < SR; ++i) {
        f16x8 v, vl;
        if (TN_TWS_EXP & 1) { v = xr[PB][i][0]; vl = xr[PB][i][1]; } else
#pragma unroll
        for (int j = 0; j < 8; ++j) {
          float acc = 0.f;
#pragma unroll
          for (int s = 0; s < 4; ++s) acc += fmaxf(fmaf((float)xr[PB][i][s][j], scb[PB][j], shb[PB][j]), 0.f);
          const float m = 0.25f * acc;
          v[j] = (f16)m;
          vl[j] = (f16)(m - (float)v[j]);
        }
        *(f16x8 *)(Xs + swz<128>(r0 + 32 * i, c)) = v;
        *(f16x8 *)(Xl + swz<128>(r0 + 32 * i, c)) = vl;
      }
    };
    load(0, ic<0>{});
    load(1, ic<1>{});
#pragma unroll
    for (int i0 = 0; i0 < nk; i0 += 2) {
      stage(ic<0>{});
      load(i0 + 2, ic<0>{});
      lds_barrier();
      stage(ic<1>{});
      load(i0 + 3, ic<1>{});
      lds_barrier();
    }
    lds_barrier();
  } else {
    const int wn = wid - 4;
    const int r32 = lane & 31, h32 = lane >> 5;
    f32x16 acc[NCT][NPT];
#pragma unroll
    for (int ct = 0; ct < NCT; ++ct)
#pragma unroll
      for (int pt = 0; pt < NPT; ++pt)
#pragma unroll
        for (int r = 0; r < 16; ++r) acc[ct][pt][r] = 0.f;
    const f16x8 *wf = (const f16x8 *)a.wfrag + (size_t)(wn * NCT) * 64 + lane;
    f16x8 wa[4][NCT];
    auto load_w = [&](int kt, auto s_tag) {
      constexpr int S = decltype(s_tag)::value;
      kt = kt < nk ? kt : nk - 1;
#pragma unroll
      for (int ct = 0; ct < NCT; ++ct) wa[S][ct] = wf[((size_t)(kt * 4 + S) * (NB / 32) + ct) * 64];
    };
    auto mult = [&](int kt, auto s_tag) {
      constexpr int S = decltype(s_tag)::value;
      const unsigned char *Xs = smem + (kt & 1) * 2 * XT, *Xl = Xs + XT;
      f16x8 xb[NPT], xl[NPT];
#pragma unroll
      for (int pt = 0; pt < NPT; ++pt) {
        xb[pt] = *(const f16x8 *)(Xs + swz<128>(pt * 32 + r32, S * 2 + h32));
        xl[pt] = *(const f16x8 *)(Xl + swz<128>(pt * 32 + r32, S * 2 + h32));
      }
      if (TN_TWS_EXP & 2) {
#pragma unroll
        for (int pt = 0; pt < NPT; ++pt) acc[0][pt][0] += (float)xb[pt][0] + (float)xl[pt][0] + (float)wa[S][pt % NCT][0];
      } else {
#pragma unroll
        for (int ct = 0; ct < NCT; ++ct)
#pragma unroll
          for (int pt = 0; pt < NPT; ++pt) acc[ct][pt] = __builtin_amdgcn_mfma_f32_32x32x16_f16(wa[S][ct], xb[pt], acc[ct][pt], 0, 0, 0);
#pragma unroll
        for (int ct = 0; ct < NCT; ++ct)
#pragma unroll
          for (int pt = 0; pt < NPT; ++pt) acc[ct][pt] = __builtin_amdgcn_mfma_f32_32x32x16_f16(wa[S][ct], xl[pt], acc[ct][pt], 0, 0, 0);
      }
      if (!(TN_TWS_EXP & 4)) load_w(kt + 1, s_tag);
    };
    load_w(0, ic<0>{});
    load_w(0, ic<1>{});
    load_w(0, ic<2>{});
    load_w(0, ic<3>{});
    lds_barrier();
#pragma unroll
    for (int kt = 0; kt < nk; ++kt) {
      mult(kt, ic<0>{});
      mult(kt, ic<1>{});
      mult(kt, ic<2>{});
      mult(kt, ic<3>{});
      lds_barrier();
    }
#pragma unroll
    for (int ct = 0; ct < NCT; ++ct)
#pragma unroll
      for (int pt = 0; pt < NPT; ++pt)
#pragma unroll
        for (int g = 0; g < 4; ++g) {
          const int m = pt * 32 + r32, n = wn * (NB / 4) + ct * 32 + 8 * g + 4 * h32;
          f16x4 h;
#pragma unroll
          for (int r = 0; r < 4; ++r) h[r] = (f16)acc[ct][pt][4 * g + r];
          *(f16x4 *)(smem + m * CPITCH + n * 2) = h;
          if (a.y32 && m < nrow)
            *(float4 *)(a.y32 + ((long)frame * P + p0 + m) * a.ld32 + n) =
                make_float4(acc[ct][pt][4 * g], acc[ct][pt][4 * g + 1], acc[ct][pt][4 * g + 2], acc[ct][pt][4 * g + 3]);
        }
  }
  __syncthreads();
  for (int id = t; id < nrow * (NB / 8); id += 512) {
    const int row = id / (NB / 8), ch = id % (NB / 8);
    const uint4 v = *(const uint4 *)(smem + row * CPITCH + ch * 16);
    *(uint4 *)(a.y + ((long)frame * P + p0 + row) * a.ldy + a.yoff + ch * 8) = v;
  }
}

__global__ void pack_trans_frags_kernel(const f16 *__restrict__ w, int N, int K, f16 *__restrict__ out) {
  const long id = (long)blockIdx.x * blockDim.x + threadIdx.x;
  if (id >= (long)N * K / 8) return;
  const int l = (int)(id & 63);
  const long f = id >> 6;
  const int ct = (int)(f % (N / 32)), g = (int)(f / (N / 32));
  *(f16x8 *)(out + id * 8) = *(const f16x8 *)(w + (long)(ct * 32 + (l & 31)) * K + g * 16 + 8 * (l >> 5));
}

}

std::vector<f16> pack_trans_frags(const f16 *w, int N, int K) {
  std::vector<f16> out((size_t)N * K);
  for (int g = 0; g < K / 16; ++g)
    for (int ct = 0; ct < N / 32; ++ct)
      for (int l = 0; l < 64; ++l)
        for (int j = 0; j < 8; ++j)
          out[(((size_t)g * (N / 32) + ct) * 64 + l) * 8 + j] = w[(size_t)(ct * 32 + (l & 31)) * K + g * 16 + 8 * (l >> 5) + j];
  return out;
}

bool trans_ws_supported(const Conv1x1Args &a) {
  return a.pool && !a.exact && !a.bias && (a.N == 512 || a.N == 256) && a.K % (2 * BK) == 0 && a.H % 2 == 0 && a.W % 2 == 0 && a.H >= 2 && a.W >= 2 &&
         a.M % ((a.H / 2) * (a.W / 2)) == 0;
}

int launch_pack_trans_frags(const f16 *w, int N, int K, f16 *out, hipStream_t s) {
  TN_REQUIRE(N % 32 == 0 && K % 16 == 0, "pack_trans_frags: N % 32 or K % 16");
  const long cells = (long)N * K / 8;
  hipLaunchKernelGGL(pack_trans_frags_kernel, dim3((unsigned)((cells + 255) / 256)), dim3(256), 0, s, w, N, K, out);
  TN_HIP_CHECK(hipGetLastError());
  return TN_OK;
}

template <int NK, int BM, int NB>
static int launch_tws(const Conv1x1Args &a, hipStream_t s) {
  using G = TG<BM, NB>;
  TN_SET_ATTR_ONCE_PER_DEVICE(TN_HIP_CHECK(hipFuncSetAttribute((const void *)trans_ws_kernel<NK, BM, NB>, hipFuncAttributeMaxDynamicSharedMemorySize, G::LDS_BYTES)));
  const int P = (a.H / 2) * (a.W / 2), TPF = (P + BM - 1) / BM, PT = (P + TPF - 1) / TPF;
  hipLaunchKernelGGL((trans_ws_kernel<NK, BM, NB>), dim3(a.M / P * TPF), dim3(512), G::LDS_BYTES, s, a, TPF, PT);
  TN_HIP_CHECK(hipGetLastError());
  return TN_OK;
}

int launch_trans_ws(const Conv1x1Args &a, hipStream_t s) {
  TN_REQUIRE(trans_ws_supported(a) && a.wfrag, "trans_ws: unsupported geometry");
  if (a.N == 512) return a.K == 16 * BK ? launch_tws<16, 64, 512>(a, s) : launch_tws<0, 64, 512>(a, s);
  return a.K == 8 * BK ? launch_tws<8, 128, 256>(a, s) : launch_tws<0, 128, 256>(a, s);
}
```

Baseline: 139,800.

## Fuse final BN-ReLU-avgpool head into transition and block7 epilogues

```diff
diff --git a/include/tennis_hip_debug.h b/include/tennis_hip_debug.h
--- a/include/tennis_hip_debug.h
+++ b/include/tennis_hip_debug.h
@@ -41,6 +41,9 @@
 int tn_dbg_conv1x1_ex(tn_ctx *ctx, const void *x_f16, int ldx, int K, const float *scale, const float *shift, const void *w_f16, int N,
                       void *y_f16, int ldy, int yoff, int M, int pool, int H, int W, int variant, const float *bias, int clamp,
                       float *y32, int ld32, const void *wfrag);
+int tn_dbg_conv1x1_head(tn_ctx *ctx, const void *x_f16, int ldx, int K, const float *scale, const float *shift, const void *w_f16, int N,
+                        void *y_f16, int ldy, int yoff, int M, int pool, int H, int W, float *y32, int ld32, const void *wfrag,
+                        float *feat, const float *head_s, const float *head_t, int ldfeat);
 int tn_dbg_pack_trans_frags(const uint16_t *w_f16_host, int N, int K, uint16_t *out_host);
 int tn_dbg_pack_trans_frags_dev(tn_ctx *ctx, const void *w_f16, int N, int K, void *out_f16);
 int tn_dbg_dense_layer_dev(tn_ctx *ctx, void *buf_f16, int ldc, int K, const float *s1, const float *t1,
@@ -70,12 +73,16 @@
                                       const float *const *t1, const void *const *w1s_f16, const void *const *w3s_f16, int B, int H,
                                       int W);
 int tn_dbg_strip_pair_launches(int64_t *count);
+int tn_dbg_head_fused_launches(int64_t *count);
+int tn_dbg_head_fused(int height, int width, int flags, int batch, int calibrate, int class_maps, int *fused);
 
 int tn_dbg_block7_create(tn_ctx *ctx, int K0, int nl, const float *w1_all, const float *s1_all, const float *t1_all,
                          const float *s2_all, const float *t2_all, const float *w3_all, void **out);
 int tn_dbg_block7_run(void *handle, void *buf_f16, int ldc, int B);
 int tn_dbg_block7_run_ts(void *handle, void *buf_f16, int ldc, int B,
                          unsigned long long *ts );
+int tn_dbg_block7_run_head(void *handle, void *buf_f16, int ldc, int B, float *side, float *feat, const float *head_s, const float *head_t,
+                           int ldfeat, unsigned long long *ts);
 void tn_dbg_block7_destroy(void *handle);
 
 int tn_dbg_block14_create(tn_ctx *ctx, int K0, int nl, const float *w1_all, const float *s1_all, const float *t1_all,
diff --git a/tennis_amd/_lib.py b/tennis_amd/_lib.py
--- a/tennis_amd/_lib.py
+++ b/tennis_amd/_lib.py
@@ -191,6 +191,8 @@
     "tn_dbg_conv3x3_dev": (C.c_int, [_P, _P, _P, _P, _P, _P, C.c_int, C.c_int, C.c_int, C.c_int, C.c_int, C.c_int]),
     "tn_dbg_conv1x1_ex": (C.c_int, [_P, _P, C.c_int, C.c_int, _P, _P, _P, C.c_int, _P, C.c_int, C.c_int, C.c_int,
                                     C.c_int, C.c_int, C.c_int, C.c_int, _P, C.c_int, _P, C.c_int, _P]),
+    "tn_dbg_conv1x1_head": (C.c_int, [_P, _P, C.c_int, C.c_int, _P, _P, _P, C.c_int, _P, C.c_int, C.c_int, C.c_int,
+                                      C.c_int, C.c_int, C.c_int, _P, C.c_int, _P, _P, _P, _P, C.c_int]),
     "tn_dbg_pack_trans_frags": (C.c_int, [_P, C.c_int, C.c_int, _P]),
     "tn_dbg_pack_trans_frags_dev": (C.c_int, [_P, _P, C.c_int, C.c_int, _P]),
     "tn_dbg_dense_layer_dev": (C.c_int, [_P, _P, C.c_int, C.c_int, _P, _P, _P, _P, _P, _P, C.c_int, C.c_int, C.c_int,
@@ -234,6 +236,8 @@
     "tn_dbg_dense_strip_pair_dev": (C.c_int, [_P, _P, C.c_int, C.c_int, _P, _P, _P, _P, C.c_int, C.c_int, C.c_int, _P]),
     "tn_dbg_dense_strip_pair_chain_dev": (C.c_int, [_P, _P, C.c_int, C.c_int, C.c_int, _P, _P, _P, _P, C.c_int, C.c_int, C.c_int]),
     "tn_dbg_strip_pair_launches": (C.c_int, [C.POINTER(C.c_int64)]),
+    "tn_dbg_head_fused_launches": (C.c_int, [C.POINTER(C.c_int64)]),
+    "tn_dbg_head_fused": (C.c_int, [C.c_int, C.c_int, C.c_int, C.c_int, C.c_int, C.c_int, C.POINTER(C.c_int)]),
     "tn_densenet121_input_means": (C.c_int, [_P, _P, C.c_int, C.c_int, _P, C.c_int64, C.POINTER(C.c_int64)]),
     "tn_npy_writer_create": (C.c_int, [C.c_int, C.POINTER(_P)]),
     "tn_npy_writer_submit": (C.c_int, [_P, _P, C.c_int, C.c_int, C.POINTER(C.c_char_p), C.c_int]),
@@ -245,6 +249,7 @@
     "tn_dbg_block7_create": (C.c_int, [_P, C.c_int, C.c_int, _P, _P, _P, _P, _P, _P, C.POINTER(C.c_void_p)]),
     "tn_dbg_block7_run": (C.c_int, [_P, _P, C.c_int, C.c_int]),
     "tn_dbg_block7_run_ts": (C.c_int, [_P, _P, C.c_int, C.c_int, _P]),
+    "tn_dbg_block7_run_head": (C.c_int, [_P, _P, C.c_int, C.c_int, _P, _P, _P, _P, C.c_int, _P]),
     "tn_dbg_block7_destroy": (None, [_P]),
     "tn_dbg_block14_create": (C.c_int, [_P, C.c_int, C.c_int, _P, _P, _P, _P, _P, _P, C.POINTER(C.c_void_p)]),
     "tn_dbg_block14_run": (C.c_int, [_P, _P, C.c_int, C.c_int]),
diff --git a/tennis_amd/csrc/common.h b/tennis_amd/csrc/common.h
--- a/tennis_amd/csrc/common.h
+++ b/tennis_amd/csrc/common.h
@@ -131,6 +131,9 @@
   float *y32 = nullptr;
   int ld32 = 0;
   const f16 *wfrag = nullptr;
+  float *feat = nullptr;
+  const float *head_s = nullptr, *head_t = nullptr;
+  int ldfeat = 0;
 };
 int launch_conv1x1(const Conv1x1Args &a, hipStream_t s);
 bool trans_ws_supported(const Conv1x1Args &a);
@@ -203,6 +206,8 @@
 int launch_dense_strip_pair(const DenseStripArgs &a, hipStream_t s);
 int launch_dense_strip_pair_chain(const DenseStripChainArgs &a, hipStream_t s);
 long strip_pair_launches();
+long head_fused_launches();
+void head_fused_launched();
 std::vector<f16> pack_w1_strip(const float *w , int K, const float *shift );
 std::vector<f16> pack_w3_strip(const float *w );
 
@@ -214,6 +219,9 @@
   unsigned a_off[4], b_off[4];
   unsigned long long *ts = nullptr;
   float *side = nullptr;
+  float *feat = nullptr;
+  const float *head_s = nullptr, *head_t = nullptr;
+  int ldfeat = 0;
 };
 struct Block7Layer { const float *w1f , *w3 , *s1, *t1 , *t2 ; };
 struct Block7Image {
diff --git a/tennis_amd/csrc/conv1x1.hip b/tennis_amd/csrc/conv1x1.hip
--- a/tennis_amd/csrc/conv1x1.hip
+++ b/tennis_amd/csrc/conv1x1.hip
@@ -218,6 +218,7 @@
   const dim3 block(256);
   static const bool no_ws = getenv("TN_NO_TRANS_WS") != nullptr;
   if (a.wfrag && !no_ws && trans_ws_supported(a)) return launch_trans_ws(a, s);
+  TN_REQUIRE(!a.feat, "conv1x1: the head epilogue (feat) exists in the warp-specialised transition kernel only (wfrag, a geometry trans_ws supports, no TN_NO_TRANS_WS)");
   if (a.pool) {
     static const bool narrow = getenv("TN_TRANS_NARROW") != nullptr;
     const bool wide = a.N % 256 == 0 && !narrow;
diff --git a/tennis_amd/csrc/dbg.hip b/tennis_amd/csrc/dbg.hip
--- a/tennis_amd/csrc/dbg.hip
+++ b/tennis_amd/csrc/dbg.hip
@@ -75,6 +75,23 @@
   return launch_conv1x1(a, ctx->stream);
 }
 
+extern "C" int tn_dbg_conv1x1_head(tn_ctx *ctx, const void *x_f16, int ldx, int K, const float *scale, const float *shift, const void *w_f16,
+                                   int N, void *y_f16, int ldy, int yoff, int M, int pool, int H, int W, float *y32, int ld32, const void *wfrag,
+                                   float *feat, const float *head_s, const float *head_t, int ldfeat) {
+  TN_REQUIRE(ctx && x_f16 && y_f16 && scale && shift && w_f16 && wfrag && feat && head_s && head_t, "tn_dbg_conv1x1_head: null argument");
+  TN_REQUIRE(M > 0 && K > 0 && N > 0 && ldx >= K && ldy >= yoff + N && yoff >= 0 && ldfeat >= N, "tn_dbg_conv1x1_head: bad shape (M, K, N positive, ldx >= K, ldy >= yoff + N, ldfeat >= N)");
+  TN_REQUIRE(pool && H >= 2 && W >= 2 && M % ((H / 2) * (W / 2)) == 0, "tn_dbg_conv1x1_head: a pooling transition with M = B (H / 2) (W / 2)");
+  TN_REQUIRE(!y32 || (ld32 >= N && ld32 % 4 == 0 && ((uintptr_t)y32 & 15) == 0), "tn_dbg_conv1x1_head: y32 needs ld32 >= N, a multiple of 4, and 16-byte alignment");
+  Conv1x1Args a{(const f16 *)x_f16, ldx, K, scale, shift, (const f16 *)w_f16, N, (f16 *)y_f16, ldy, yoff, M, pool, H, W};
+  a.y32 = y32;
+  a.ld32 = ld32;
+  a.wfrag = (const f16 *)wfrag;
+  a.feat = feat; a.head_s = head_s; a.head_t = head_t; a.ldfeat = ldfeat;
+  TN_REQUIRE(trans_ws_supported(a), "tn_dbg_conv1x1_head: a geometry trans_ws does not support (N = 512 | 256, K % 128 == 0, even H and W)");
+  TN_ON_DEVICE(ctx->device);
+  return launch_conv1x1(a, ctx->stream);
+}
+
 extern "C" int tn_dbg_pack_trans_frags(const uint16_t *w_f16_host, int N, int K, uint16_t *out_host) {
   TN_REQUIRE(w_f16_host && out_host, "tn_dbg_pack_trans_frags: null argument");
   TN_REQUIRE(N > 0 && K > 0 && N % 32 == 0 && K % 16 == 0, "tn_dbg_pack_trans_frags: N % 32 or K % 16");
@@ -380,6 +397,19 @@
   TN_ON_DEVICE(b->ctx->device);
   DenseBlock7Args a = b->args;
   a.buf = (f16 *)buf_f16; a.ldc = ldc; a.B = B; a.ts = ts;
+  return launch_dense_block7(a, b->ctx->stream);
+}
+
+extern "C" int tn_dbg_block7_run_head(void *handle, void *buf_f16, int ldc, int B, float *side, float *feat, const float *head_s,
+                                      const float *head_t, int ldfeat, unsigned long long *ts) {
+  tn_dbg_block7 *b = (tn_dbg_block7 *)handle;
+  TN_REQUIRE(b && buf_f16, "tn_dbg_block7_run_head: null argument");
+  TN_REQUIRE(((uintptr_t)side & 15) == 0, "tn_dbg_block7_run_head: side must be 16-byte aligned");
+  TN_ON_DEVICE(b->ctx->device);
+  DenseBlock7Args a = b->args;
+  a.buf = (f16 *)buf_f16; a.ldc = ldc; a.B = B; a.ts = ts;
+  a.side = side;
+  a.feat = feat; a.head_s = head_s; a.head_t = head_t; a.ldfeat = ldfeat;
   return launch_dense_block7(a, b->ctx->stream);
 }
 
@@ -656,6 +686,25 @@
   return TN_OK;
 }
 
+extern "C" int tn_dbg_head_fused_launches(int64_t *count) {
+  TN_REQUIRE(count, "tn_dbg_head_fused_launches: null argument");
+  *count = (int64_t)head_fused_launches();
+  return TN_OK;
+}
+
+extern "C" int tn_dbg_head_fused(int height, int width, int flags, int batch, int calibrate, int class_maps, int *fused) {
+  TN_REQUIRE(fused, "tn_dbg_head_fused: null argument");
+  TN_REQUIRE((flags & ~(TN_ENC_EXACT_WEIGHTS | TN_ENC_FP32 | TN_ENC_FP32X3)) == 0, "tn_dbg_head_fused: unknown flag");
+  TN_REQUIRE(batch > 0, "tn_dbg_head_fused: batch must be positive");
+  TN_REQUIRE(height >= 224 && width >= 224 && height <= 1024 && width <= 1024, "tn_dbg_head_fused: input size must be in [224,1024]");
+  const EncPolicy p = enc_policy(flags);
+  const EncGeom g = enc_geom(height, width);
+  if (const char *why = enc_refusal(p, g)) { tn_set_error(why); return TN_ERR_INVALID; }
+  const bool fp32 = (flags & (TN_ENC_FP32 | TN_ENC_FP32X3)) != 0;
+  *fused = !fp32 && enc_head_fused(p, g, calibrate != 0, class_maps != 0, false) ? 1 : 0;
+  return TN_OK;
+}
+
 extern "C" int tn_dbg_gnmt_trainer_src_grad(tn_gnmt_trainer *t, const float *src, const int32_t *src_valid_len, const int32_t *tgt, int ld,
                                             const int32_t *tgt_valid_len, int batch, int steps, int tgt_len, float *loss,
                                             float *logits_out, float *dsrc, int ldd) {
diff --git a/tennis_amd/csrc/dense_block7.hip b/tennis_amd/csrc/dense_block7.hip
--- a/tennis_amd/csrc/dense_block7.hip
+++ b/tennis_amd/csrc/dense_block7.hip
@@ -1,4 +1,6 @@
+#include <cstdint>
 #include <cstring>
+#include <string>
 #include <type_traits>
 #include <utility>
 
@@ -32,6 +34,9 @@
 constexpr int kTabFloats = 512 + 512 + 128;
 constexpr int kLdsBytes = kTabOff + kTabFloats * 4;
 static_assert(kLdsBytes <= 160 * 1024, "LDS");
+constexpr int kHeadOff = kLdsBytes, kHeadPitch = 52 * 4;
+constexpr int kLdsBytesHead = kHeadOff + 32 * kHeadPitch;
+static_assert(kHeadOff % 16 == 0 && kLdsBytesHead <= 160 * 1024, "LDS");
 constexpr int kStepUnits = 256;
 constexpr int kW3Units = 18 * 64;
 
@@ -39,7 +44,7 @@
   return __builtin_amdgcn_mfma_f32_32x32x16_f16(a, b, c, 0, 0, 0);
 }
 
-template <int D>
+template <int D, bool HEAD = false>
 __global__ void __launch_bounds__(256) __attribute__((amdgpu_waves_per_eu(1, 1))) dense_block7_kernel(DenseBlock7Args a) {
   extern __shared__ __attribute__((aligned(16))) unsigned char smem[];
   const int tid = threadIdx.x, lane = tid & 63, n = lane & 31, h = lane >> 5;
@@ -236,6 +241,12 @@
     }
 
     stamp();
+    f32x4 hsc[2], hsh[2];
+    if constexpr (HEAD) {
+      const int c0 = K + 16 * (w >> 1) + 8 * h;
+      hsc[0] = *(const f32x4 *)(a.head_s + c0); hsc[1] = *(const f32x4 *)(a.head_s + c0 + 4);
+      hsh[0] = *(const f32x4 *)(a.head_t + c0); hsh[1] = *(const f32x4 *)(a.head_t + c0 + 4);
+    }
     f32x16 q[2];
     f16x8 bq[2][2];
     bq[0][0] = lds_h8(offb[0][0]);
@@ -282,7 +293,14 @@
       if (p < kPix) {
         *(f16x8 *)(smem + (unsigned)((K >> 3) + 2 * sf + h) * kChunkRow + p * 16) = ov;
         *(f16x8 *)(xb + (size_t)p * a.ldc + K + 16 * sf + 8 * h) = ov;
-        if (a.side) {
+        if constexpr (HEAD) {
+          float *hp = (float *)(smem + kHeadOff + (unsigned)(16 * sf + 8 * h) * kHeadPitch) + p;
+#pragma unroll
+          for (int j = 0; j < 4; ++j) {
+            hp[j * (kHeadPitch / 4)] = fmaxf(fmaf(o0[j], hsc[0][j], hsh[0][j]), 0.f);
+            hp[(4 + j) * (kHeadPitch / 4)] = fmaxf(fmaf(o1[j], hsc[1][j], hsh[1][j]), 0.f);
+          }
+        } else if (a.side) {
           float *sp = a.side + ((size_t)blockIdx.x * kPix + p) * a.ldc + K + 16 * sf + 8 * h;
           *(f32x4 *)sp = o0;
           *(f32x4 *)(sp + 4) = o1;
@@ -295,6 +313,19 @@
       }
     }
     __syncthreads();
+    if constexpr (HEAD) {
+      if (w == 3 && lane < 32) {
+        const unsigned row = kHeadOff + (unsigned)lane * kHeadPitch;
+        float sum = 0.f;
+#pragma unroll
+        for (int q = 0; q < 12; ++q) {
+          const f32x4 v = lds_f4(row + q * 16);
+          sum += v[0]; sum += v[1]; sum += v[2]; sum += v[3];
+        }
+        sum += *(const float *)(smem + row + 48 * 4);
+        a.feat[(size_t)blockIdx.x * a.ldfeat + K + lane] = sum * (1.0f / 49.0f);
+      }
+    }
     stamp();
   }
   if (a.ts && w == 0 && lane == 0) a.ts[(size_t)blockIdx.x * 128 + 126] = __builtin_amdgcn_s_memrealtime();
@@ -360,6 +391,15 @@
   TN_REQUIRE(a.ldc % 8 == 0, "dense_block7: the row pitch must be a multiple of 8: " + geom);
   TN_REQUIRE(a.K0 + 32 * a.nl <= a.ldc, "dense_block7: the row pitch does not hold the last layer's output: " + geom);
   TN_REQUIRE(a.B > 0, "dense_block7: the batch must be positive: " + geom);
+  if (a.feat) {
+    TN_REQUIRE(a.head_s && a.head_t && a.ldfeat >= a.K0 + 32 * a.nl, "dense_block7: the head epilogue needs head_s, head_t and ldfeat >= K0 + 32 nl: " + geom);
+    TN_REQUIRE((((uintptr_t)a.head_s | (uintptr_t)a.head_t) & 15) == 0, "dense_block7: head_s and head_t must be 16-byte aligned: " + geom);
+    TN_SET_ATTR_ONCE_PER_DEVICE(TN_HIP_CHECK(hipFuncSetAttribute((const void *)dense_block7_kernel<kRingDepth, true>, hipFuncAttributeMaxDynamicSharedMemorySize, kLdsBytesHead)));
+    hipLaunchKernelGGL((dense_block7_kernel<kRingDepth, true>), dim3(a.B), dim3(256), kLdsBytesHead, s, a);
+    TN_HIP_CHECK(hipGetLastError());
+    head_fused_launched();
+    return TN_OK;
+  }
   TN_SET_ATTR_ONCE_PER_DEVICE(TN_HIP_CHECK(hipFuncSetAttribute((const void *)dense_block7_kernel<kRingDepth>, hipFuncAttributeMaxDynamicSharedMemorySize, kLdsBytes)));
   hipLaunchKernelGGL((dense_block7_kernel<kRingDepth>), dim3(a.B), dim3(256), kLdsBytes, s, a);
   TN_HIP_CHECK(hipGetLastError());
diff --git a/tennis_amd/csrc/encoder.hip b/tennis_amd/csrc/encoder.hip
--- a/tennis_amd/csrc/encoder.hip
+++ b/tennis_amd/csrc/encoder.hip
@@ -633,7 +633,8 @@
   };
   std::vector<EncStep> plan[4];
   for (int b = 0; b < 4; ++b) plan[b] = enc_block_plan(p, g, b, B, cal, shared_chip);
-  float *h32 = plan[3][0].route == ENC_BLOCK7 ? e->head32 + (size_t)w0 * g.Hb[3] * g.Wb[3] * g.Cb[3] : nullptr;
+  const bool head_fused = enc_head_fused(p, g, cal, e->cam_w != nullptr, tm.on) && plan[3][0].route == ENC_BLOCK7;
+  float *h32 = !head_fused && plan[3][0].route == ENC_BLOCK7 ? e->head32 + (size_t)w0 * g.Hb[3] * g.Wb[3] * g.Cb[3] : nullptr;
   auto begin = [&](const std::string &family, const EncCost &c) { tm.begin(family.c_str(), c.flops, c.bytes); };
   {
     StemArgs a{x, (int)layout, B, g.H, g.W, e->stem_wp, e->stem_wp_zf, e->stem_scale, e->stem_shift, stem_out, g.Hs, g.Ws};
@@ -676,6 +677,7 @@
           DenseBlock7Args a7 = e->b7[b];
           a7.buf = bbuf[b]; a7.B = B;
           a7.side = b == 3 ? h32 : nullptr;
+          if (b == 3 && head_fused) { a7.feat = feat; a7.head_s = e->head_s; a7.head_t = e->head_t; a7.ldfeat = g.feat_dim; }
           rc = launch_dense_block7(a7, s);
           break;
         }
@@ -725,12 +727,14 @@
       at.exact = p.exact;
       at.wfrag = cal ? nullptr : T.wfrag;
       if (b == 2 && h32) { at.y32 = h32; at.ld32 = g.Cb[3]; }
+      if (b == 2 && head_fused) { at.feat = feat; at.head_s = e->head_s; at.head_t = e->head_t; at.ldfeat = g.feat_dim; }
       begin("transition_conv1x1_avgpool", transition_cost(M, Mo, T.cin, T.cout));
       rc = launch_conv1x1(at, s);
       tm.end();
       if (rc) return rc;
     }
   }
+  if (head_fused) return TN_OK;
   begin("head_bnrelu_avgpool7", head_cost(g, fB));
   rc = launch_head(bbuf[3], B, g.Hb[3], g.Wb[3], g.Cb[3], e->head_s, e->head_t, feat, g.PH, g.PW, s, h32);
   tm.end();
diff --git a/tennis_amd/csrc/encoder_plan.h b/tennis_amd/csrc/encoder_plan.h
--- a/tennis_amd/csrc/encoder_plan.h
+++ b/tennis_amd/csrc/encoder_plan.h
@@ -19,6 +19,8 @@
   bool strip_pair = true;
   int strip_pair_min_batch = 256;
   bool block7 = true;
+  bool trans_ws = true;
+  bool head_fuse = true;
   bool block_stream[2] = {true, false};
   int dl_variant = 0;
 };
@@ -39,6 +41,8 @@
   p.strip_pair = getenv("TN_NO_STRIP_PAIR") == nullptr;
   if (getenv("TN_STRIP_PAIR_MIN_BATCH")) p.strip_pair_min_batch = atoi(getenv("TN_STRIP_PAIR_MIN_BATCH"));
   p.block7 = getenv("TN_NO_BLOCK7") == nullptr;
+  p.trans_ws = getenv("TN_NO_TRANS_WS") == nullptr;
+  p.head_fuse = getenv("TN_NO_HEAD_FUSE") == nullptr;
   p.block_stream[0] = getenv("TN_NO_BLOCK14") == nullptr;
   p.block_stream[1] = getenv("TN_BLOCK28") != nullptr && atoi(getenv("TN_BLOCK28")) != 0;
   p.dl_variant = getenv("TN_DL_VARIANT") ? atoi(getenv("TN_DL_VARIANT")) : 0;
@@ -134,6 +138,13 @@
          B >= p.strip_pair_min_batch && B % 2 == 0;
 }
 
+inline bool enc_head_fused(const EncPolicy &p, const EncGeom &g, bool cal, bool class_maps, bool timed) {
+  if (!p.head_fuse || cal || class_maps || timed) return false;
+  if (p.dl_variant != 0 || !enc_block7(p, g, 3)) return false;
+  if (g.Hb[3] != 7 || g.Wb[3] != 7 || g.PH != 1 || g.PW != 1) return false;
+  return p.trans_ws && !p.exact && g.Cb[2] / 2 == 512 && g.Cb[2] % 128 == 0 && g.Hb[2] == 14 && g.Wb[2] == 14;
+}
+
 inline std::vector<EncStep> enc_block_plan(const EncPolicy &p, const EncGeom &g, int b, int B, bool cal, bool shared_chip) {
   const int n = kBlockCfg[b], Hh = g.Hb[b];
   std::vector<EncStep> plan;
diff --git a/tennis_amd/csrc/trans_ws.hip b/tennis_amd/csrc/trans_ws.hip
--- a/tennis_amd/csrc/trans_ws.hip
+++ b/tennis_amd/csrc/trans_ws.hip
@@ -1,3 +1,6 @@
+#include <atomic>
+#include <cstdint>
+#include <string>
 #include <type_traits>
 #include <utility>
 #include <vector>
@@ -20,6 +23,11 @@
   static constexpr int NCT = NB / 4 / 32, NPT = BM / 32;
   static_assert(NCT * NPT == 8, "128 accumulator registers");
 };
+constexpr int kHeadRows = 49;
+constexpr int kHeadTermOff = kHeadRows * TG<64, 512>::CPITCH;
+constexpr int kHeadTermPitch = 512 * 4 + 16;
+constexpr int kHeadLdsBytes = kHeadTermOff + kHeadRows * kHeadTermPitch;
+static_assert(kHeadTermOff % 16 == 0 && kHeadLdsBytes <= 160 * 1024, "LDS");
 
 __device__ __forceinline__ void lds_barrier() {
   asm volatile("s_waitcnt lgkmcnt(0)" ::: "memory");
@@ -30,9 +38,10 @@
 template <int V>
 using ic = std::integral_constant<int, V>;
 
-template <int NK, int BM, int NB>
+template <int NK, int BM, int NB, bool HEAD = false>
 __global__ __launch_bounds__(512) __attribute__((amdgpu_waves_per_eu(2, 2))) void trans_ws_kernel(Conv1x1Args a, int TPF, int PT) {
   using G = TG<BM, NB>;
+  static_assert(!HEAD || (BM == 64 && NB == 512), "the head epilogue belongs to the 64 x 512 tile");
   constexpr int XT = G::XT, CPITCH = G::CPITCH, SR = G::SR, NCT = G::NCT, NPT = G::NPT;
   extern __shared__ __attribute__((aligned(16))) unsigned char smem[];
   const int t = threadIdx.x, lane = t & 63;
@@ -169,13 +178,30 @@
           f16x4 h;
 #pragma unroll
           for (int r = 0; r < 4; ++r) h[r] = (f16)acc[ct][pt][4 * g + r];
-          *(f16x4 *)(smem + m * CPITCH + n * 2) = h;
-          if (a.y32 && m < nrow)
-            *(float4 *)(a.y32 + ((long)frame * P + p0 + m) * a.ld32 + n) =
-                make_float4(acc[ct][pt][4 * g], acc[ct][pt][4 * g + 1], acc[ct][pt][4 * g + 2], acc[ct][pt][4 * g + 3]);
+          if constexpr (HEAD) {
+            if (m < kHeadRows) {
+              const float4 hs = *(const float4 *)(a.head_s + n), ht = *(const float4 *)(a.head_t + n);
+              *(f16x4 *)(smem + m * CPITCH + n * 2) = h;
+              *(float4 *)(smem + kHeadTermOff + m * kHeadTermPitch + n * 4) =
+                  make_float4(fmaxf(fmaf(acc[ct][pt][4 * g], hs.x, ht.x), 0.f), fmaxf(fmaf(acc[ct][pt][4 * g + 1], hs.y, ht.y), 0.f),
+                              fmaxf(fmaf(acc[ct][pt][4 * g + 2], hs.z, ht.z), 0.f), fmaxf(fmaf(acc[ct][pt][4 * g + 3], hs.w, ht.w), 0.f));
+            }
+          } else {
+            *(f16x4 *)(smem + m * CPITCH + n * 2) = h;
+            if (a.y32 && m < nrow)
+              *(float4 *)(a.y32 + ((long)frame * P + p0 + m) * a.ld32 + n) =
+                  make_float4(acc[ct][pt][4 * g], acc[ct][pt][4 * g + 1], acc[ct][pt][4 * g + 2], acc[ct][pt][4 * g + 3]);
+          }
         }
   }
   __syncthreads();
+  if constexpr (HEAD) {
+    const unsigned char *col = smem + kHeadTermOff + t * 4;
+    float sum = 0.f;
+#pragma unroll
+    for (int p = 0; p < kHeadRows; ++p) sum += *(const float *)(col + p * kHeadTermPitch);
+    a.feat[(long)frame * a.ldfeat + t] = sum * (1.0f / 49.0f);
+  }
   for (int id = t; id < nrow * (NB / 8); id += 512) {
     const int row = id / (NB / 8), ch = id % (NB / 8);
     const uint4 v = *(const uint4 *)(smem + row * CPITCH + ch * 16);
@@ -227,8 +253,29 @@
   return TN_OK;
 }
 
+static std::atomic<long> g_head_fused_launches{0};
+long head_fused_launches() { return g_head_fused_launches.load(std::memory_order_relaxed); }
+void head_fused_launched() { g_head_fused_launches.fetch_add(1, std::memory_order_relaxed); }
+
+template <int NK>
+static int launch_tws_head(const Conv1x1Args &a, hipStream_t s) {
+  TN_SET_ATTR_ONCE_PER_DEVICE(TN_HIP_CHECK(hipFuncSetAttribute((const void *)trans_ws_kernel<NK, 64, 512, true>, hipFuncAttributeMaxDynamicSharedMemorySize, kHeadLdsBytes)));
+  hipLaunchKernelGGL((trans_ws_kernel<NK, 64, 512, true>), dim3(a.M / kHeadRows), dim3(512), kHeadLdsBytes, s, a, 1, kHeadRows);
+  TN_HIP_CHECK(hipGetLastError());
+  head_fused_launched();
+  return TN_OK;
+}
+
 int launch_trans_ws(const Conv1x1Args &a, hipStream_t s) {
   TN_REQUIRE(trans_ws_supported(a) && a.wfrag, "trans_ws: unsupported geometry");
+  if (a.feat) {
+    const int P = (a.H / 2) * (a.W / 2);
+    TN_REQUIRE(a.N == 512 && P == kHeadRows, "trans_ws: the head epilogue needs N = 512 and a frame of one 49-pixel tile (a 14 x 14 map): N = " +
+                                                 std::to_string(a.N) + ", " + std::to_string(a.H) + " x " + std::to_string(a.W));
+    TN_REQUIRE(a.head_s && a.head_t && a.ldfeat >= a.N, "trans_ws: the head epilogue needs head_s, head_t and ldfeat >= N");
+    TN_REQUIRE((((uintptr_t)a.head_s | (uintptr_t)a.head_t) & 15) == 0, "trans_ws: head_s and head_t must be 16-byte aligned");
+    return a.K == 16 * BK ? launch_tws_head<16>(a, s) : launch_tws_head<0>(a, s);
+  }
   if (a.N == 512) return a.K == 16 * BK ? launch_tws<16, 64, 512>(a, s) : launch_tws<0, 64, 512>(a, s);
   return a.K == 8 * BK ? launch_tws<8, 128, 256>(a, s) : launch_tws<0, 128, 256>(a, s);
 }
```

New measurement: 141,200 (median of 6 runs). 1.01x the previous value.
